# DavidXu-JJ/StreetUnveiler

Hardware: AMD Instinct MI355X
Metric: Msplats/s fwd+bwd @1920x1080, 3M Gaussians (higher is better)
Workload: dtype f32; 1 GPU; C3: 3M Gaussians, 1920x1080, fwd+bwd with depth/normal aux outputs (all 7 aux-map gradients live); gaussians=3000000, width=1920, height=1080, sh_degree=3, frames_per_rank=1, parallelism=single GPU, camera_rig=benchmark

## Files before the change

diff_surfel_rasterization/_C.py:

```python
from __future__ import annotations

import ctypes as C
import os

import torch

from streetunveiler_amd import _lib as L


_roctx = None


def _roctx_lib():
    global _roctx
    if _roctx is None:
        _roctx = False
        import os
        if os.environ.get("SURFEL_ROCTX") == "1":
            for name in ("libroctx64.so", "libroctx64.so.4", "/opt/rocm/lib/libroctx64.so"):
                try:
                    lib = C.CDLL(name)
                    lib.roctxRangePushA.argtypes = [C.c_char_p]; lib.roctxRangePushA.restype = C.c_int
                    lib.roctxRangePop.restype = C.c_int
                    _roctx = lib
                    break
                except OSError:
                    continue
    return _roctx


class _range:
    def __init__(self, name: str):
        self.name = name

    def __enter__(self):
        lib = _roctx_lib()
        self.on = bool(lib)
        if self.on:
            lib.roctxRangePushA(("surfel:" + self.name).encode())
        return self

    def __exit__(self, *exc):
        if self.on:
            _roctx.roctxRangePop()
        return False


def _ptr(t: torch.Tensor):
    return None if t is None or t.numel() == 0 else C.c_void_p(t.data_ptr())


def _f32c(t: torch.Tensor, name: str) -> torch.Tensor:
    if t is None:
        return None
    if not t.is_cuda:
        raise L.SurfelRasterError(f"{name} must be a CUDA (ROCm) tensor; the surfel rasterizer has no CPU path")
    if t.dtype != torch.float32:
        t = t.float()
    return t.contiguous()


def _stream(device):
    return C.c_void_p(torch.cuda.current_stream(device).cuda_stream)


_EXTRA_FLAGS = int(os.environ.get("SURFEL_EXTRA_FLAGS", "0"), 0)


def _frame(bg, scale_modifier, viewmatrix, projmatrix, tan_fovx, tan_fovy, H, W, degree, campos, prefiltered, debug, tile=None,
           quadrant_cull=True, blend_counters=None, ballot_ranking=False, row_mapped=None, forward_only=False, no_precomp_color_grad=False,
           binning_capacity=None, backward_kernel=None):
    keep = [_f32c(bg, "bg"), _f32c(viewmatrix, "viewmatrix"), _f32c(projmatrix, "projmatrix"), _f32c(campos, "campos"), blend_counters]
    if blend_counters is not None and (blend_counters.dtype != torch.int64 or blend_counters.numel() < 16 or not blend_counters.is_cuda):
        raise L.SurfelRasterError("blend_counters must be a CUDA (ROCm) int64 tensor with 16 entries")
    fr = L.SrFrame(int(H), int(W), float(tan_fovx), float(tan_fovy), float(scale_modifier), int(degree),
                   int(bool(prefiltered)), int(bool(debug)), _ptr(keep[0]), _ptr(keep[1]), _ptr(keep[2]), _ptr(keep[3]),
                   int(tile[0]) if tile else 0, int(tile[1]) if tile else 0, (0 if quadrant_cull else L.SR_FLAG_NO_QUADRANT_CULL) | (L.SR_FLAG_BALLOT_RANKING if ballot_ranking else 0) |
                   (0 if row_mapped is None else (L.SR_FLAG_ROW_MAPPED_FORWARD if row_mapped else L.SR_FLAG_QUADRANT_MAPPED_FORWARD)) |
                   (L.SR_FLAG_FORWARD_ONLY if forward_only else 0) | (L.SR_FLAG_NO_PRECOMP_COLOR_GRAD if no_precomp_color_grad else 0) |
                   (L.SR_FLAG_BINNING_CAPACITY if binning_capacity is not None else 0) |
                   ({None: 0, "one_wave": L.SR_FLAG_ONE_WAVE_BACKWARD, "coop": L.SR_FLAG_COOP_BACKWARD, "rows": L.SR_FLAG_ROW_BACKWARD}[backward_kernel]) | _EXTRA_FLAGS,
                   _ptr(blend_counters))
    return fr, keep


def _mask(mask, P, dev):
    if mask is None:
        return None
    if mask.numel() != P or mask.dtype not in (torch.bool, torch.uint8):
        raise L.SurfelRasterError("mask must be a bool tensor with one entry per Gaussian")
    if not mask.is_cuda:
        raise L.SurfelRasterError("mask must be a CUDA (ROCm) tensor")
    return mask.contiguous().view(torch.uint8)


def _channels(colors_precomp):
    if colors_precomp is None or (colors_precomp.numel() == 0 and not (colors_precomp.ndim == 2 and colors_precomp.shape[0] == 0 and colors_precomp.shape[1] in (3, 6))):
        return 3
    nc = int(colors_precomp.shape[-1])
    if colors_precomp.ndim != 2 or nc not in (3, 6):
        raise L.SurfelRasterError("colors_precomp must have dimensions (num_points, 3) or (num_points, 6)")
    return nc


def _gaussians(means3D, opacities, scales, rotations, sh, colors_precomp, transMat_precomp, activations=0, mask=None):
    P = int(means3D.shape[0])
    M = int(sh.shape[1]) if sh is not None and (sh.numel() or (P == 0 and sh.ndim == 3)) else 0
    NC = _channels(colors_precomp)
    if M and NC == 6:
        NC = 9
    elif M and colors_precomp is not None and colors_precomp.numel():
        raise L.SurfelRasterError("Please provide exactly one of either SHs or precomputed colors!")
    g = L.SrGaussians(P, M, NC, int(activations), _ptr(means3D), _ptr(opacities), _ptr(scales), _ptr(rotations), _ptr(sh),
                      _ptr(colors_precomp), _ptr(transMat_precomp), _ptr(mask))
    return g


def rasterize_gaussians(bg, means3D, colors_precomp, opacities, scales, rotations, scale_modifier, transMat_precomp,
                        viewmatrix, projmatrix, tan_fovx, tan_fovy, image_height, image_width, sh, degree, campos,
                        prefiltered, debug, activations=0, tile=None, mask=None, quadrant_cull=True, blend_counters=None,
                        ballot_ranking=False, row_mapped=None, forward_only=False, classes=None, n_classes=0, binning_capacity=None, backward_kernel=None):
    lib = L.load()
    if means3D.ndim != 2 or means3D.shape[1] != 3:
        raise L.SurfelRasterError("means3D must have dimensions (num_points, 3)")
    means3D = _f32c(means3D, "means3D"); opacities = _f32c(opacities, "opacities")
    colors_precomp = _f32c(colors_precomp, "colors_precomp"); scales = _f32c(scales, "scales")
    rotations = _f32c(rotations, "rotations"); transMat_precomp = _f32c(transMat_precomp, "transMat_precomp")
    sh = _f32c(sh, "sh")
    dev = means3D.device
    P, H, W = int(means3D.shape[0]), int(image_height), int(image_width)
    with torch.cuda.device(dev), _range("forward"):
        if binning_capacity is not None and (classes is not None or int(binning_capacity) < 0):
            raise L.SurfelRasterError("binning_capacity: a non-negative number of duplicates; not with the shared-plan class pass")
        fr, keep = _frame(bg, scale_modifier, viewmatrix, projmatrix, tan_fovx, tan_fovy, H, W, degree, campos, prefiltered, debug, tile,
                          quadrant_cull, blend_counters, ballot_ranking, row_mapped, forward_only, binning_capacity=binning_capacity,
                          backward_kernel=backward_kernel)
        mask = _mask(mask, P, dev)
        g = _gaussians(means3D, opacities, scales, rotations, sh, colors_precomp, transMat_precomp, activations, mask)
        if keep[0].numel() != g.color_channels:
            raise L.SurfelRasterError(f"bg must have {g.color_channels} entries, one per colour channel")
        color = torch.empty((g.color_channels, H, W), dtype=torch.float32, device=dev)
        allmap = torch.empty((7, H, W), dtype=torch.float32, device=dev)
        radii = torch.empty((P,), dtype=torch.int32, device=dev)
        geom = torch.empty((lib.sr_geom_bytes(P),), dtype=torch.uint8, device=dev)
        img = torch.empty((0 if forward_only else lib.sr_image_bytes(W, H),), dtype=torch.uint8, device=dev)
        stream = _stream(dev)
        D = C.c_uint32(0)
        L.check(lib.sr_forward_plan(C.byref(fr), C.byref(g), _ptr(geom), geom.numel(), _ptr(radii), C.byref(D), stream),
                "sr_forward_plan")
        num_rendered = int(D.value) if binning_capacity is None else (max(1, int(binning_capacity)) if P else 0)
        binning = torch.empty((lib.sr_binning_bytes(P, num_rendered, W, H),), dtype=torch.uint8, device=dev)
        L.check(lib.sr_forward_render(C.byref(fr), C.byref(g), _ptr(geom), geom.numel(), _ptr(binning), binning.numel(),
                                      _ptr(img), img.numel(), num_rendered, _ptr(color), _ptr(allmap), stream),
                "sr_forward_render")
        if classes is not None and int(n_classes) > 0:
            if classes.numel() != P:
                raise L.SurfelRasterError("classes must have one entry per Gaussian")
            if forward_only:
                raise L.SurfelRasterError("the shared-plan class pass is a training pass: not with forward_only")
            cls = classes.to(device=dev, dtype=torch.int32).contiguous()
            dist = torch.empty((int(n_classes), H, W), dtype=torch.float32, device=dev)
            cstate = torch.empty((lib.sr_class_shared_bytes(P, W, H, int(n_classes), num_rendered),), dtype=torch.uint8, device=dev)
            with _range("class_forward"):
                L.check(lib.sr_class_forward_shared(C.byref(fr), C.byref(g), int(n_classes), _ptr(cls), _ptr(geom), geom.numel(), _ptr(binning), binning.numel(),
                                                    _ptr(cstate), cstate.numel(), num_rendered, _ptr(dist), stream), "sr_class_forward_shared")
            del keep
            return num_rendered, color, allmap, radii, geom, binning, img, dist, cstate
    del keep
    return num_rendered, color, allmap, radii, geom, binning, img


def rasterize_gaussians_backward(bg, means3D, radii, colors_precomp, scales, rotations, scale_modifier, transMat_precomp,
                                 viewmatrix, projmatrix, tan_fovx, tan_fovy, dL_dcolor, dL_dallmap, sh, degree, campos,
                                 geomBuffer, num_rendered, binningBuffer, imgBuffer, debug, opacities=None, defer_sh=False,
                                 activations=0, tile=None, after_blend=None, class_state=None, dL_ddist=None, n_classes=0, want_precomp_color_grad=True,
                                 binning_capacity=None, backward_kernel=None):
    lib = L.load()
    means3D = _f32c(means3D, "means3D")
    colors_precomp = _f32c(colors_precomp, "colors_precomp"); scales = _f32c(scales, "scales")
    rotations = _f32c(rotations, "rotations"); transMat_precomp = _f32c(transMat_precomp, "transMat_precomp")
    sh = _f32c(sh, "sh")
    dL_dcolor = _f32c(dL_dcolor, "dL_dcolor"); dL_dallmap = _f32c(dL_dallmap, "dL_dallmap")
    dev = means3D.device
    P = int(means3D.shape[0])
    H, W = int(dL_dcolor.shape[1]), int(dL_dcolor.shape[2])
    M = int(sh.shape[1]) if sh is not None and sh.numel() else 0
    with torch.cuda.device(dev), _range("backward"):
        skip_cg = (not want_precomp_color_grad) and _channels(colors_precomp) == 6
        fr, keep = _frame(bg, scale_modifier, viewmatrix, projmatrix, tan_fovx, tan_fovy, H, W, degree, campos, False, debug, tile,
                          no_precomp_color_grad=skip_cg, binning_capacity=binning_capacity, backward_kernel=backward_kernel)
        g = _gaussians(means3D, means3D, scales, rotations, sh, colors_precomp, transMat_precomp, activations)
        e = lambda *shape: torch.empty(shape, dtype=torch.float32, device=dev)
        has = lambda t: t is not None and t.numel() > 0
        defer_sh = bool(defer_sh) and has(sh) and not has(colors_precomp)
        sizes = [("means3D", (P, 3)), ("sh", (P, M, 3) if has(sh) and not defer_sh else (0, 0, 3)), ("opacity", (P, 1)),
                 ("scales", (P, 2) if has(scales) else (0, 2)), ("rotations", (P, 4) if has(rotations) else (0, 4))]
        numel = lambda shp: int(torch.Size(shp).numel())
        flat = torch.empty(sum(numel(shp) for _, shp in sizes), dtype=torch.float32, device=dev)
        views, off = {}, 0
        for name, shp in sizes:
            n = numel(shp)
            views[name] = flat[off:off + n].view(shp)
            off += n
        dL_dmeans3D, dL_dsh, dL_dopacity, dL_dscales, dL_drotations = (views[k] for k in ("means3D", "sh", "opacity", "scales", "rotations"))
        dL_dmeans2D = e(P, 3)
        NC = g.color_channels
        if int(dL_dcolor.shape[0]) != NC or keep[0].numel() != NC:
            raise L.SurfelRasterError(f"dL_dcolor / bg must have {NC} channels")
        dL_dcolors = e(P, 6 if NC == 9 else NC) if (has(colors_precomp) and not skip_cg) or defer_sh else e(0, 3)
        dL_dtransMat = e(P, 9) if has(transMat_precomp) else e(0, 9)
        ws = torch.empty((lib.sr_backward_workspace_bytes(P, int(num_rendered), NC),), dtype=torch.uint8, device=dev)
        grads = L.SrGradients(_ptr(dL_dmeans2D), _ptr(dL_dcolors), _ptr(dL_dopacity), _ptr(dL_dmeans3D), _ptr(dL_dtransMat),
                              _ptr(dL_dsh), _ptr(dL_dscales), _ptr(dL_drotations))
        if class_state is not None:
            if defer_sh or after_blend is not None:
                raise L.SurfelRasterError("the shared-plan class pass (class_state) does not combine with the factored SH exchange "
                                          "(defer_sh / after_blend): exchange its gradients with the plain all-reduce")
            dL_ddist = _f32c(dL_ddist, "dL_ddist")
            L.check(lib.sr_backward_blend(C.byref(fr), C.byref(g), _ptr(geomBuffer), geomBuffer.numel(), _ptr(binningBuffer),
                                          binningBuffer.numel(), _ptr(imgBuffer), imgBuffer.numel(), int(num_rendered), _ptr(dL_dcolor),
                                          _ptr(dL_dallmap), _ptr(ws), ws.numel(), _stream(dev)), "sr_backward_blend")
            with _range("class_backward"):
                L.check(lib.sr_class_backward_shared(C.byref(fr), C.byref(g), int(n_classes), _ptr(geomBuffer), geomBuffer.numel(), _ptr(binningBuffer),
                                                     binningBuffer.numel(), _ptr(class_state), class_state.numel(), int(num_rendered), _ptr(dL_ddist),
                                                     _ptr(ws), ws.numel(), _stream(dev)), "sr_class_backward_shared")
            L.check(lib.sr_backward_geometry(C.byref(fr), C.byref(g), _ptr(radii), _ptr(geomBuffer), geomBuffer.numel(), _ptr(binningBuffer),
                                             binningBuffer.numel(), _ptr(imgBuffer), imgBuffer.numel(), int(num_rendered), _ptr(ws),
                                             ws.numel(), C.byref(grads), _stream(dev)), "sr_backward_geometry")
        elif after_blend is not None and defer_sh and NC == 3:
            L.check(lib.sr_backward_blend(C.byref(fr), C.byref(g), _ptr(geomBuffer), geomBuffer.numel(), _ptr(binningBuffer),
                                          binningBuffer.numel(), _ptr(imgBuffer), imgBuffer.numel(), int(num_rendered), _ptr(dL_dcolor),
                                          _ptr(dL_dallmap), _ptr(ws), ws.numel(), _stream(dev)), "sr_backward_blend")
            L.check(lib.sr_backward_colors(C.byref(fr), C.byref(g), _ptr(radii), _ptr(geomBuffer), geomBuffer.numel(), int(num_rendered),
                                           _ptr(ws), ws.numel(), _ptr(dL_dcolors), _stream(dev)), "sr_backward_colors")
            after_blend(dL_dcolors)
            grads.dL_dcolors = None
            L.check(lib.sr_backward_geometry(C.byref(fr), C.byref(g), _ptr(radii), _ptr(geomBuffer), geomBuffer.numel(), _ptr(binningBuffer),
                                             binningBuffer.numel(), _ptr(imgBuffer), imgBuffer.numel(), int(num_rendered), _ptr(ws),
                                             ws.numel(), C.byref(grads), _stream(dev)), "sr_backward_geometry")
        else:
            L.check(lib.sr_backward(C.byref(fr), C.byref(g), _ptr(radii), _ptr(geomBuffer), geomBuffer.numel(),
                                    _ptr(binningBuffer), binningBuffer.numel(), _ptr(imgBuffer), imgBuffer.numel(),
                                    int(num_rendered), _ptr(dL_dcolor), _ptr(dL_dallmap), _ptr(ws), ws.numel(),
                                    C.byref(grads), _stream(dev)), "sr_backward")
    del keep
    return dL_dmeans2D, dL_dcolors, dL_dopacity, dL_dmeans3D, dL_dtransMat, dL_dsh, dL_dscales, dL_drotations


def class_distortions(bg, means3D, classes, opacities, scales, rotations, scale_modifier, viewmatrix, projmatrix, tan_fovx, tan_fovy,
                      image_height, image_width, campos, n_classes, debug=False, activations=0, mask=None, tile=None):
    lib = L.load()
    if means3D.ndim != 2 or means3D.shape[1] != 3:
        raise L.SurfelRasterError("means3D must have dimensions (num_points, 3)")
    means3D = _f32c(means3D, "means3D"); opacities = _f32c(opacities, "opacities"); scales = _f32c(scales, "scales"); rotations = _f32c(rotations, "rotations")
    dev = means3D.device
    P, H, W = int(means3D.shape[0]), int(image_height), int(image_width)
    if classes.numel() != P:
        raise L.SurfelRasterError("classes must have one entry per Gaussian")
    cols = torch.zeros((P, 3), dtype=torch.float32, device=dev)
    cols[:, 0] = classes.to(device=dev, dtype=torch.float32).reshape(P)
    with torch.cuda.device(dev), _range("class_forward"):
        fr, keep = _frame(bg, scale_modifier, viewmatrix, projmatrix, tan_fovx, tan_fovy, H, W, 0, campos, False, debug, tile)
        mask = _mask(mask, P, dev)
        g = _gaussians(means3D, opacities, scales, rotations, None, cols, None, activations, mask)
        dist = torch.empty((int(n_classes), H, W), dtype=torch.float32, device=dev)
        radii = torch.empty((P,), dtype=torch.int32, device=dev)
        geom = torch.empty((lib.sr_geom_bytes(P),), dtype=torch.uint8, device=dev)
        cimg = torch.empty((lib.sr_class_image_bytes(W, H, int(n_classes)),), dtype=torch.uint8, device=dev)
        stream = _stream(dev)
        D = C.c_uint32(0)
        L.check(lib.sr_forward_plan(C.byref(fr), C.byref(g), _ptr(geom), geom.numel(), _ptr(radii), C.byref(D), stream), "sr_forward_plan")
        num_rendered = int(D.value)
        binning = torch.empty((lib.sr_binning_bytes(P, num_rendered, W, H),), dtype=torch.uint8, device=dev)
        L.check(lib.sr_class_forward_render(C.byref(fr), C.byref(g), int(n_classes), _ptr(geom), geom.numel(), _ptr(binning), binning.numel(),
                                            _ptr(cimg), cimg.numel(), num_rendered, _ptr(dist), stream), "sr_class_forward_render")
    del keep
    return num_rendered, dist, radii, cols, geom, binning, cimg


def class_distortions_backward(bg, means3D, radii, cols, scales, rotations, scale_modifier, viewmatrix, projmatrix, tan_fovx, tan_fovy,
                               dL_ddist, campos, n_classes, geom, num_rendered, binning, cimg, debug=False, activations=0, tile=None):
    lib = L.load()
    means3D = _f32c(means3D, "means3D"); scales = _f32c(scales, "scales"); rotations = _f32c(rotations, "rotations")
    dL_ddist = _f32c(dL_ddist, "dL_ddist")
    dev = means3D.device
    P = int(means3D.shape[0])
    H, W = int(dL_ddist.shape[1]), int(dL_ddist.shape[2])
    with torch.cuda.device(dev), _range("class_backward"):
        fr, keep = _frame(bg, scale_modifier, viewmatrix, projmatrix, tan_fovx, tan_fovy, H, W, 0, campos, False, debug, tile)
        g = _gaussians(means3D, means3D, scales, rotations, None, cols, None, activations)
        flat = torch.empty(P * 10, dtype=torch.float32, device=dev)
        dL_dmeans3D, dL_dopacity = flat[:3 * P].view(P, 3), flat[3 * P:4 * P].view(P, 1)
        dL_dscales, dL_drotations = flat[4 * P:6 * P].view(P, 2), flat[6 * P:].view(P, 4)
        dL_dmeans2D = torch.empty((P, 3), dtype=torch.float32, device=dev)
        ws = torch.empty((lib.sr_backward_workspace_bytes(P, int(num_rendered), 3),), dtype=torch.uint8, device=dev)
        grads = L.SrGradients(_ptr(dL_dmeans2D), None, _ptr(dL_dopacity), _ptr(dL_dmeans3D), None, None, _ptr(dL_dscales), _ptr(dL_drotations))
        L.check(lib.sr_class_backward(C.byref(fr), C.byref(g), int(n_classes), _ptr(radii), _ptr(geom), geom.numel(), _ptr(binning), binning.numel(),
                                      _ptr(cimg), cimg.numel(), int(num_rendered), _ptr(dL_ddist), _ptr(ws), ws.numel(), C.byref(grads),
                                      _stream(dev)), "sr_class_backward")
    del keep
    return dL_dmeans2D, dL_dopacity, dL_dmeans3D, dL_dscales, dL_drotations


def pair_decisions(bg, means3D, scale_modifier, viewmatrix, projmatrix, tan_fovx, tan_fovy, image_height, image_width, degree, campos,
                   geomBuffer, num_rendered, binningBuffer, tile=None):
    lib = L.load()
    means3D = _f32c(means3D, "means3D")
    dev = means3D.device
    tw, th = tile if tile else (16, 16)
    nq = (tw // 8) * (th // 8)
    valid = torch.zeros((max(int(num_rendered), 1), nq), dtype=torch.int64, device=dev)
    use3d = torch.zeros_like(valid)
    with torch.cuda.device(dev):
        fr, keep = _frame(bg, scale_modifier, viewmatrix, projmatrix, tan_fovx, tan_fovy, image_height, image_width, degree, campos, False, False, tile)
        g = L.SrGaussians(int(means3D.shape[0]), 0, 3, 0, _ptr(means3D), _ptr(means3D), None, None, None, _ptr(means3D), _ptr(means3D), None)
        L.check(lib.sr_debug_pair_decisions(C.byref(fr), C.byref(g), _ptr(geomBuffer), geomBuffer.numel(), _ptr(binningBuffer),
                                            binningBuffer.numel(), int(num_rendered), _ptr(valid), _ptr(use3d), _stream(dev)),
                "sr_debug_pair_decisions")
    del keep
    return valid[:int(num_rendered)], use3d[:int(num_rendered)]


def sh_gradient_expand(means3D, campos, dL_dcolors, sh_coeffs, degree):
    lib = L.load()
    means3D = _f32c(means3D, "means3D"); campos = _f32c(campos, "campos").reshape(-1, 3); dL_dcolors = _f32c(dL_dcolors, "dL_dcolors")
    P, V = int(means3D.shape[0]), int(campos.shape[0])
    if dL_dcolors.numel() != V * P * 3:
        raise L.SurfelRasterError(f"dL_dcolors must have {V} x {P} x 3 elements")
    out = torch.empty((P, int(sh_coeffs), 3), dtype=torch.float32, device=means3D.device)
    with torch.cuda.device(means3D.device):
        L.check(lib.sr_sh_gradient_expand(P, int(sh_coeffs), int(degree), V, _ptr(means3D), _ptr(campos), _ptr(dL_dcolors),
                                          _ptr(out), _stream(means3D.device)), "sr_sh_gradient_expand")
    return out


def mark_visible(means3D, viewmatrix, projmatrix):
    lib = L.load()
    means3D = _f32c(means3D, "means3D"); viewmatrix = _f32c(viewmatrix, "viewmatrix"); projmatrix = _f32c(projmatrix, "projmatrix")
    P = int(means3D.shape[0])
    present = torch.empty((P,), dtype=torch.bool, device=means3D.device)
    with torch.cuda.device(means3D.device):
        L.check(lib.sr_mark_visible(P, _ptr(means3D), _ptr(viewmatrix), _ptr(projmatrix), _ptr(present),
                                    _stream(means3D.device)), "sr_mark_visible")
    return present


def _view(buf: torch.Tensor, ptr, nbytes: int, dtype: torch.dtype) -> torch.Tensor:
    off = int(ptr) - buf.data_ptr()
    return buf[off:off + nbytes].view(dtype)


def forward_status(geom: torch.Tensor, P: int) -> torch.Tensor:
    v = L.SrGeomView()
    L.check(L.load().sr_geom_view(_ptr(geom), geom.numel(), int(P), C.byref(v)), "sr_geom_view")
    return _view(geom, v.frame_counts, 12, torch.int32)


def geom_view(geom: torch.Tensor, P: int):
    v = L.SrGeomView()
    L.check(L.load().sr_geom_view(_ptr(geom), geom.numel(), P, C.byref(v)), "sr_geom_view")
    return dict(splats=_view(geom, v.splats, P * 80, torch.float32).view(P, 20),
                depth_keys=_view(geom, v.depth_keys, P * 4, torch.int32), tiles_touched=_view(geom, v.tiles_touched, P * 4, torch.int32),
                clamped=_view(geom, v.clamped, P, torch.uint8), sorted_gid=_view(geom, v.sorted_gid, P * 4, torch.int32),
                frame_counts=_view(geom, v.frame_counts, 8, torch.int32))


def binning_view(binning: torch.Tensor, P: int, D: int, W: int, H: int, tile=(16, 16)):
    v = L.SrBinningView()
    L.check(L.load().sr_binning_view(_ptr(binning), binning.numel(), P, D, W, H, C.byref(v)), "sr_binning_view")
    tiles = ((W + tile[0] - 1) // tile[0]) * ((H + tile[1] - 1) // tile[1])
    ranges = _view(binning, v.ranges, tiles * 8, torch.int32).view(tiles, 2)
    counts = (ranges[:, 1] - ranges[:, 0]).long()
    tile_keys = torch.repeat_interleave(torch.arange(tiles, device=binning.device, dtype=torch.int32), counts)
    return dict(tile_keys=tile_keys, point_list=_view(binning, v.point_list, D * 4, torch.int32), ranges=ranges,
                tile_order=_view(binning, v.tile_order, tiles * 4, torch.int32))


def image_view(img: torch.Tensor, W: int, H: int):
    v = L.SrImageView()
    L.check(L.load().sr_image_view(_ptr(img), img.numel(), W, H, C.byref(v)), "sr_image_view")
    return dict(final_T=_view(img, v.final_T, 3 * H * W * 4, torch.float32).view(3, H, W),
                n_contrib=_view(img, v.n_contrib, 2 * H * W * 4, torch.int32).view(2, H, W))
```

streetunveiler_amd/csrc/api.hip:

```cpp
#include <cstdarg>
#include <cstdio>
#include <cstring>
#include <cmath>
#include <atomic>
#include <mutex>

#include "common.h"

namespace sr {
hipError_t launch_preprocess_forward(int P, const FrameDev& f, const SrGaussians& g, float4* recs, uint32_t* depth_keys,
                                     uint32_t* tiles_touched, uint2* rect, uint8_t* clamped, int32_t* radii, hipStream_t s);
hipError_t launch_preprocess_backward(int P, const FrameDev& f, const SrGaussians& g, const int32_t* radii,
                                      const uint8_t* clamped, const float4* recs, const float4* inst_grads, const uint8_t* written,
                                      const uint32_t* tiles_touched, const SrGradients& out, hipStream_t s);
hipError_t launch_mark_visible(int P, const float* means3D, const float* view, uint8_t* present, hipStream_t s);
hipError_t launch_sh_gradient_expand(int P, int M, int deg, int V, const float* means3D, const float* campos, const float* gc,
                                     float* dL_dsh, hipStream_t s);
size_t depth_sort_temp_bytes(int P);
size_t tile_scan_temp_bytes(int P);
size_t expand_x_hist_bytes(int P, int tiles_x);
size_t expand_y_hist_bytes(uint32_t D, int tiles_y);
hipError_t run_depth_sort(int P, const uint32_t* depth_keys, const uint2* rect, uint32_t* sorted_keys,
                          uint32_t* sorted_gid, uint2* rect_sorted, void* temp, size_t temp_bytes, int rank_mode, int tiles_x, int tiles_y,
                          const uint32_t* n_visible, hipStream_t s);
hipError_t run_tile_count_scan(int P, const uint32_t* tiles_touched, uint32_t* first, void* block_base, size_t base_bytes, uint32_t* total_host,
                               hipStream_t s);
hipError_t run_expand_columns(int P, int tiles_x, int n_tiles, const uint2* rect_sorted, const uint32_t* sorted_gid, uint2* columns,
                              uint32_t* n_columns, uint32_t* hist, uint32_t* row_total, uint32_t* tile_counts, int rank_mode, const uint32_t* n_visible,
                              hipStream_t s);
hipError_t run_expand_rows(uint32_t D, int tiles_x, int tiles_y, const uint2* columns, const uint32_t* n_columns, uint32_t* hist, uint32_t* row_total,
                           uint32_t* point_list, uint32_t* tile_counts, int rank_mode, hipStream_t s);
hipError_t run_tile_ranges_order(int n_tiles, const uint32_t* tile_counts, uint2* ranges, uint32_t* order, hipStream_t s);
hipError_t run_capacity_guard(uint32_t* counts, uint32_t capacity, hipStream_t s);
hipError_t launch_zero_bytes(void* p, size_t n, hipStream_t s);
hipError_t launch_render_forward(const FrameDev& f, const uint2* ranges, const uint32_t* tile_order, const uint32_t* point_list, const float4* recs,
                                 const float* extra, float* out_color, float* out_allmap, float* final_T, uint32_t* n_contrib, uint16_t* hit_mask, int flags,
                                 unsigned long long* counters, const uint32_t* frame_counts, hipStream_t s);
hipError_t launch_render_backward(const FrameDev& f, const uint2* ranges, const uint32_t* tile_order, const uint32_t* point_list, const float4* recs,
                                  const float* extra, const float* final_T, const uint32_t* n_contrib, const float* dL_dcolor,
                                  const float* dL_dallmap, const uint16_t* hit_mask, float4* inst_grads, uint8_t* written, bool precomp_color_grads, hipStream_t s, int coop_mode);
hipError_t launch_pair_decisions(const FrameDev& f, const uint2* ranges, const uint32_t* point_list, const float4* recs,
                                 unsigned long long* valid_bits, unsigned long long* use3d_bits, hipStream_t s);
hipError_t launch_class_partition(int P, int n_tiles, int n_classes, const float* class_cols, const int32_t* class_i32, const uint2* ranges,
                                  const uint32_t* point_list, uint8_t* ids, uint32_t* cls_list, uint2* cls_ranges, hipStream_t s);
hipError_t launch_class_forward(const FrameDev& f, int n_classes, const uint2* cls_ranges, const uint32_t* tile_order, const uint32_t* cls_list,
                                const float4* recs, float* out_dist, float* cls_state, uint32_t* cls_last, uint32_t* tile_total, uint16_t* hit_mask,
                                int cull, hipStream_t s);
hipError_t launch_class_backward(const FrameDev& f, int n_classes, const uint2* cls_ranges, const uint32_t* tile_order, const uint32_t* cls_list,
                                 const float4* recs, const float* cls_state, const uint32_t* cls_last, const uint32_t* tile_total,
                                 const float* dL_ddist, const uint16_t* hit_mask, float4* inst_grads, uint8_t* written, int shared_rec_quads, hipStream_t s);
hipError_t launch_color_gradients(int P, const FrameDev& f, const int32_t* radii, const uint8_t* clamped, const float4* recs, const float4* inst_grads,
                                  const uint8_t* written, const uint32_t* tiles_touched, bool mask_clamped, float* dL_dcolors, hipStream_t s);
size_t radix_sort_temp_bytes(uint32_t n);
hipError_t radix_sort_pairs(const uint32_t* keys_in, const uint32_t* vals_in, uint32_t* keys_out, uint32_t* vals_out, uint32_t n,
                            int total_bits, void* temp, size_t temp_bytes, hipStream_t s, const uint2* aux_src, uint2* aux_out, int rank_mode,
                            int rect_bx = 0, int rect_by = 0, const uint32_t* n_live = nullptr);
hipError_t launch_rank_selfcheck(uint32_t* result, hipStream_t s);
hipError_t lds_atomic_ranks(const uint32_t* digits, uint32_t* ranks, uint32_t n, int bins, hipStream_t s);
size_t knn_workspace_bytes(int nq, int nr);
hipError_t knn_mean_dist2(int nq, const float* query, int nr, const float* reference, int K, int take_sqrt, float* out, void* ws,
                          size_t ws_bytes, int rank_mode, hipStream_t s);
struct PostCam { int W, H; float fx, fy, depth_ratio; const float* view; };
hipError_t launch_postprocess_forward(const PostCam& cam, const float* allmap, float* rend_normal, float* surf_depth,
                                      float* surf_normal, float* surf_point, hipStream_t s);
hipError_t launch_postprocess_backward(const PostCam& cam, const float* allmap, const float* g_rend_normal, const float* g_surf_depth,
                                       const float* g_surf_normal, const float* g_surf_point, float* scratch6, float* g_allmap,
                                       hipStream_t s);
struct LossImages { int W, H, C; float lambda; const float* image; const float* gt; const float* sky; const float* alpha; };
bool image_loss_supported(int W, int H, int C);
size_t image_loss_partial_bytes();
hipError_t launch_image_loss_forward(const LossImages& a, void* workspace, float* out3, hipStream_t s);
hipError_t launch_image_loss_backward(const LossImages& a, const void* workspace, const float* g_loss, float* g_image, float* g_sky,
                                      float* g_alpha, hipStream_t s);
}

using namespace sr;

namespace {

thread_local char g_err[512] = "";
std::atomic<int> g_timing{0};
std::mutex g_ring_mu;

int fail(int code, const char* fmt, ...) {
    va_list ap;
    va_start(ap, fmt);
    vsnprintf(g_err, sizeof(g_err), fmt, ap);
    va_end(ap);
    return code;
}

#define SR_HIP(expr)                                                                                         \
    do {                                                                                                     \
        hipError_t _e = (expr);                                                                              \
        if (_e != hipSuccess) return fail(SR_ERR_HIP, "%s failed: %s (%s:%d)", #expr, hipGetErrorString(_e), \
                                          __FILE__, __LINE__);                                               \
    } while (0)

constexpr int kEvRing = 512;
struct EvRing {
    hipEvent_t ev[kEvRing][2];
    bool closed[kEvRing];
    int created = 0, used = 0;
};
EvRing g_ring[SR_STAGE_COUNT];

struct StageTimer {
    int stage; hipStream_t s; int slot = -1;
    StageTimer(int st, hipStream_t stream) : stage(st), s(stream) {
        const int mode = g_timing.load();
        if (!mode || (mode != 1 && !((mode >> 1) & (1 << stage)))) return;
        std::lock_guard<std::mutex> lk(g_ring_mu);
        EvRing& r = g_ring[stage];
        if (r.used >= kEvRing) return;
        if (r.used >= r.created) {
            if (hipEventCreate(&r.ev[r.created][0]) != hipSuccess || hipEventCreate(&r.ev[r.created][1]) != hipSuccess) return;
            ++r.created;
        }
        slot = r.used++;
        r.closed[slot] = false;
        (void)hipEventRecord(r.ev[slot][0], s);
    }
    ~StageTimer() {
        if (slot < 0) return;
        std::lock_guard<std::mutex> lk(g_ring_mu);
        if (hipEventRecord(g_ring[stage].ev[slot][1], s) == hipSuccess) g_ring[stage].closed[slot] = true;
    }
};

int debug_sync(const SrFrame* frame, hipStream_t s, const char* what) {
    if (!frame->debug) return SR_OK;
    hipError_t e = hipStreamSynchronize(s);
    if (e == hipSuccess) e = hipGetLastError();
    if (e != hipSuccess) return fail(SR_ERR_HIP, "[debug] after %s: %s", what, hipGetErrorString(e));
    return SR_OK;
}

uint32_t* pinned_words() {
    static thread_local uint32_t* pinned = nullptr;
    if (!pinned && hipHostMalloc(reinterpret_cast<void**>(&pinned), 64, hipHostMallocPortable | hipHostMallocMapped) != hipSuccess) { pinned = nullptr; (void)hipGetLastError(); }
    return pinned;
}

int stream_device(hipStream_t s, int* dev) {
    hipDevice_t d = 0;
    if (s && hipStreamGetDevice(s, &d) == hipSuccess) { *dev = (int)d; return SR_OK; }
    (void)hipGetLastError();
    SR_HIP(hipGetDevice(dev));
    return SR_OK;
}

constexpr int kMaxDevices = 64;
std::atomic<int> g_rank_mode[kMaxDevices];
int rank_mode(hipStream_t s, bool force_ballot, int* mode) {
    int dev = 0;
    { const int rc = stream_device(s, &dev); if (rc != SR_OK) return rc; }
    if (dev < 0 || dev >= kMaxDevices) return fail(SR_ERR_UNSUPPORTED, "device index %d beyond %d", dev, kMaxDevices);
    int m = g_rank_mode[dev].load(std::memory_order_acquire);
    if (m == kRankUnknown) {
        hipStreamCaptureStatus cap = hipStreamCaptureStatusNone;
        if (hipStreamIsCapturing(s, &cap) == hipSuccess && cap != hipStreamCaptureStatusNone)
            return fail(SR_ERR_UNSUPPORTED, "the stream is capturing and device %d has not run the rank self-check yet: call sr_rank_mode(stream) once before the capture", dev);
        (void)hipGetLastError();
        struct Scratch { uint32_t* p = nullptr; ~Scratch() { if (p) (void)hipFree(p); } } scratch;
        uint32_t* host = pinned_words();
        uint32_t* result = nullptr;
        const bool temp = !(host && hipHostGetDevicePointer(reinterpret_cast<void**>(&result), host + 8, 0) == hipSuccess && result);
        if (!temp) host[8] = 0;
        else { (void)hipGetLastError(); SR_HIP(hipMalloc(reinterpret_cast<void**>(&scratch.p), 4)); result = scratch.p; SR_HIP(hipMemsetAsync(result, 0, 4, s)); }
        SR_HIP(launch_rank_selfcheck(result, s));
        uint32_t r = 0;
        if (temp) { SR_HIP(hipMemcpyAsync(&r, result, 4, hipMemcpyDeviceToHost, s)); SR_HIP(hipStreamSynchronize(s)); }
        else { SR_HIP(hipStreamSynchronize(s)); r = *reinterpret_cast<volatile uint32_t*>(host + 8); }
        if (!(r & 0x100u)) return fail(SR_ERR_HIP, "the rank self-check kernel did not report back");
        m = (r & 1u) ? kRankAtomic : ((r & 2u) ? kRankBallot : kRankNone);
        g_rank_mode[dev].store(m, std::memory_order_release);
    }
    if (m == kRankNone) return fail(SR_ERR_UNSUPPORTED, "neither LDS-atomic nor ballot ranking passes the self-check on device %d", dev);
    *mode = force_ballot ? (int)kRankBallot : m;
    return SR_OK;
}

constexpr int kMaxTilesPerAxis = SR_MAX_TILES_PER_AXIS;
struct GeomLayout {
    size_t recs, depth_keys, tiles_touched, rect, clamped, sorted_keys, sorted_gid, rect_sorted, first, sh_jac, block_base, base_bytes,
        n_scan_blocks, temp, temp_bytes, total;
};
GeomLayout geom_layout(int P) {
    GeomLayout L{};
    const size_t n = (size_t)(P > 0 ? P : 1);
    size_t off = 0;
    auto take = [&](size_t bytes) { size_t o = off; off = align_up(off + bytes, 256); return o; };
    L.recs = take(n * kRecFloats * 4);
    L.depth_keys = take(n * 4);
    L.tiles_touched = take(n * 4);
    L.rect = take(n * 8);
    L.clamped = take(n);
    L.sorted_keys = take(n * 4);
    L.sorted_gid = take(n * 4);
    L.rect_sorted = take(n * 8);
    L.first = take(n * 4);
    L.sh_jac = take(n * 36);
    L.base_bytes = tile_scan_temp_bytes(P);
    L.block_base = take(L.base_bytes);
    L.n_scan_blocks = (n + 2047) / 2048;
    static thread_local int memo_P = -1;
    static thread_local size_t memo_bytes = 0;
    if (memo_P != P) {
        memo_bytes = depth_sort_temp_bytes(P);
        const size_t hx = align_up(expand_x_hist_bytes(P, kMaxTilesPerAxis), 256);
        if (hx > memo_bytes) memo_bytes = hx;
        memo_P = P;
    }
    L.temp_bytes = memo_bytes;
    L.temp = take(L.temp_bytes);
    L.total = off;
    return L;
}

struct BinLayout {
    size_t columns, point_list, hit_mask, ranges, order, tile_counts, row_total, n_columns, hist, hist_bytes, total;
};
BinLayout bin_layout(uint32_t D, int W, int H) {
    BinLayout L{};
    const size_t n = (size_t)(D > 0 ? D : 1);
    const int tiles = ((W + 7) / 8) * ((H + 7) / 8);
    size_t off = 0;
    auto take = [&](size_t bytes) { size_t o = off; off = align_up(off + bytes, 256); return o; };
    L.columns = take(n * 8);
    L.point_list = take(n * 4);
    L.hit_mask = take(n * 2);
    L.ranges = take((size_t)(tiles > 0 ? tiles : 1) * 8);
    L.order = take((size_t)(tiles > 0 ? tiles : 1) * 4);
    L.tile_counts = take((size_t)(tiles > 0 ? tiles : 1) * 4);
    L.row_total = take((size_t)kMaxTilesPerAxis * 4);
    L.n_columns = take(4);
    L.hist_bytes = expand_y_hist_bytes(D, (H + 7) / 8);
    L.hist = take(L.hist_bytes);
    L.total = off;
    return L;
}

struct ImgLayout { size_t final_T, n_contrib, total; };
ImgLayout img_layout(int W, int H) {
    ImgLayout L{};
    const size_t hw = (size_t)(W > 0 ? W : 1) * (size_t)(H > 0 ? H : 1);
    L.final_T = 0;
    L.n_contrib = align_up(hw * 3 * 4, 256);
    L.total = align_up(L.n_contrib + hw * 2 * 4, 256);
    return L;
}

int check_common(const SrFrame* frame, const SrGaussians* g) {
    if (!frame || !g) return fail(SR_ERR_INVALID_ARGUMENT, "frame / gaussians is NULL");
    if (frame->image_width <= 0 || frame->image_height <= 0) return fail(SR_ERR_INVALID_ARGUMENT, "bad image size %dx%d", frame->image_width, frame->image_height);
    if (g->P < 0) return fail(SR_ERR_INVALID_ARGUMENT, "P < 0");
    {
        const int tw = frame->tile_width > 0 ? frame->tile_width : kTile, th = frame->tile_height > 0 ? frame->tile_height : kTile;
        const bool known = (tw == 16 && th == 16) || (tw == 8 && th == 8) || (tw == 16 && th == 8) || (tw == 32 && th == 8) || (tw == 32 && th == 16);
        if (!known) return fail(SR_ERR_UNSUPPORTED, "tile shape %dx%d not in {8x8, 16x8, 16x16, 32x8, 32x16}", tw, th);
    }
    if (!frame->bg || !frame->viewmatrix || !frame->projmatrix || !frame->campos) return fail(SR_ERR_INVALID_ARGUMENT, "bg / viewmatrix / projmatrix / campos must be non-NULL device pointers");
    if (g->P > 0) {
        if (!g->means3D || !g->opacities) return fail(SR_ERR_INVALID_ARGUMENT, "means3D / opacities is NULL");
        if (g->color_channels == 9) {
            if (!g->shs || !g->colors_precomp) return fail(SR_ERR_INVALID_ARGUMENT, "9 colour channels need SHs AND a [P,6] precomputed colour array");
        } else if ((g->shs != nullptr) == (g->colors_precomp != nullptr)) return fail(SR_ERR_INVALID_ARGUMENT, "Please provide exactly one of either SHs or precomputed colors!");
        if (g->color_channels != 0 && g->color_channels != 3 && g->color_channels != 6 && g->color_channels != 9) return fail(SR_ERR_UNSUPPORTED, "color_channels %d not in {3, 6, 9}", g->color_channels);
        if (g->activations & ~(SR_ACT_EXP_SCALES | SR_ACT_SIGMOID_OPACITY | SR_ACT_NORMALIZE_ROTATIONS)) return fail(SR_ERR_UNSUPPORTED, "unknown activation bits 0x%x", g->activations);
        if (g->color_channels == 6 && g->shs) return fail(SR_ERR_INVALID_ARGUMENT, "6 colour channels need precomputed colors, not SHs");
        const bool sr_pair = g->scales != nullptr && g->rotations != nullptr;
        if ((g->scales != nullptr) != (g->rotations != nullptr) || sr_pair == (g->transMat_precomp != nullptr))
            return fail(SR_ERR_INVALID_ARGUMENT, "Please provide exactly one of either scale/rotation pair or precomputed transMat!");
        if (g->shs) {
            if (frame->sh_degree < 0 || frame->sh_degree > 3) return fail(SR_ERR_UNSUPPORTED, "sh_degree %d not in 0..3", frame->sh_degree);
            if (g->sh_coeffs < (frame->sh_degree + 1) * (frame->sh_degree + 1)) return fail(SR_ERR_INVALID_ARGUMENT, "shs has %d coefficients, degree %d needs %d", g->sh_coeffs, frame->sh_degree, (frame->sh_degree + 1) * (frame->sh_degree + 1));
        }
    }
    return SR_OK;
}

int check_backward_frame(const SrFrame* frame) {
#if SR_BACKWARD_WH_FROM_FOCAL
    if (!(frame->tanfovx > 0.f) || !(frame->tanfovy > 0.f) || !std::isfinite(frame->tanfovx) || !std::isfinite(frame->tanfovy))
        return fail(SR_ERR_INVALID_ARGUMENT, "tanfovx / tanfovy must be finite and > 0 for a backward call (got %g, %g)", (double)frame->tanfovx, (double)frame->tanfovy);
#else
    (void)frame;
#endif
    return SR_OK;
}

int check_blend_pair_flags(const SrFrame* frame) {
    const uint32_t pair = frame->flags & (SR_FLAG_ONE_WAVE_BACKWARD | SR_FLAG_COOP_BACKWARD | SR_FLAG_ROW_BACKWARD);
    if (pair & (pair - 1))
        return fail(SR_ERR_INVALID_ARGUMENT, "SR_FLAG_ONE_WAVE_BACKWARD, SR_FLAG_COOP_BACKWARD and SR_FLAG_ROW_BACKWARD exclude each other (flags 0x%x)", pair);
    return SR_OK;
}

FrameDev make_frame(const SrFrame* frame, const SrGaussians* g) {
    FrameDev f{};
    f.W = frame->image_width; f.H = frame->image_height;
    f.bw_W = f.W; f.bw_H = f.H;
#if SR_BACKWARD_WH_FROM_FOCAL
    if (frame->tanfovx > 0.f && frame->tanfovy > 0.f && std::isfinite(frame->tanfovx) && std::isfinite(frame->tanfovy)) {
        const float focal_x = (float)f.W / (2.0f * frame->tanfovx), focal_y = (float)f.H / (2.0f * frame->tanfovy);
        f.bw_W = (int)(focal_x * frame->tanfovx * 2); f.bw_H = (int)(focal_y * frame->tanfovy * 2);
    }
#endif
    f.tile_w = frame->tile_width > 0 ? frame->tile_width : kTile; f.tile_h = frame->tile_height > 0 ? frame->tile_height : kTile;
    f.inv_tile_w = 1.f / (float)f.tile_w; f.inv_tile_h = 1.f / (float)f.tile_h;
    f.tiles_x = (f.W + f.tile_w - 1) / f.tile_w; f.tiles_y = (f.H + f.tile_h - 1) / f.tile_h;
    f.sh_degree = frame->sh_degree; f.sh_coeffs = g->sh_coeffs;
    f.colors = g->color_channels == 6 ? 6 : (g->color_channels == 9 ? 9 : 3);
    f.activations = g->activations;
    f.scale_modifier = frame->scale_modifier;
    f.bg = frame->bg; f.view = frame->viewmatrix; f.proj = frame->projmatrix; f.campos = frame->campos;
    f.overflow = nullptr;
    return f;
}

template <class T> T* at(void* base, size_t off) { return reinterpret_cast<T*>(static_cast<char*>(base) + off); }

}

extern "C" {

int sr_abi_version(void) { return SR_ABI_VERSION; }
uint32_t sr_build_switches(void) { return SR_SWITCH_BITS; }
const char* sr_last_error(void) { return g_err; }

size_t sr_geom_bytes(int32_t P) { return geom_layout(P).total; }
size_t sr_binning_bytes(int32_t P, uint32_t num_rendered, int32_t W, int32_t H) { (void)P; return bin_layout(num_rendered, W, H).total; }
size_t sr_image_bytes(int32_t W, int32_t H) { return img_layout(W, H).total; }
static size_t record_bytes(int color_channels) { return (size_t)(color_channels == 9 ? kGradFloats + 4 : kGradFloats) * 4; }

size_t sr_backward_workspace_bytes(int32_t P, uint32_t num_rendered, int32_t color_channels) {
    (void)P;
    const size_t n = (size_t)(num_rendered > 0 ? num_rendered : 1);
    return align_up(n * record_bytes(color_channels), 256) + align_up(n, 256);
}

int sr_geom_view(void* geom, size_t geom_bytes, int32_t P, SrGeomView* out) {
    if (!geom || !out) return fail(SR_ERR_INVALID_ARGUMENT, "NULL argument");
    const GeomLayout L = geom_layout(P);
    if (geom_bytes < L.total) return fail(SR_ERR_BUFFER_TOO_SMALL, "geom buffer %zu < %zu", geom_bytes, L.total);
    out->splats = at<float>(geom, L.recs); out->depth_keys = at<uint32_t>(geom, L.depth_keys);
    out->tiles_touched = at<uint32_t>(geom, L.tiles_touched); out->clamped = at<uint8_t>(geom, L.clamped);
    out->sorted_gid = at<uint32_t>(geom, L.sorted_gid);
    out->frame_counts = at<uint32_t>(geom, L.block_base) + L.n_scan_blocks;
    return SR_OK;
}

int sr_binning_view(void* binning, size_t binning_bytes, int32_t P, uint32_t D, int32_t W, int32_t H, SrBinningView* out) {
    (void)P;
    if (!binning || !out) return fail(SR_ERR_INVALID_ARGUMENT, "NULL argument");
    const BinLayout L = bin_layout(D, W, H);
    if (binning_bytes < L.total) return fail(SR_ERR_BUFFER_TOO_SMALL, "binning buffer %zu < %zu", binning_bytes, L.total);
    out->point_list = at<uint32_t>(binning, L.point_list);
    out->ranges = at<uint32_t>(binning, L.ranges); out->tile_order = at<uint32_t>(binning, L.order);
    return SR_OK;
}

int sr_image_view(void* image, size_t image_bytes, int32_t W, int32_t H, SrImageView* out) {
    if (!image || !out) return fail(SR_ERR_INVALID_ARGUMENT, "NULL argument");
    const ImgLayout L = img_layout(W, H);
    if (image_bytes < L.total) return fail(SR_ERR_BUFFER_TOO_SMALL, "image buffer %zu < %zu", image_bytes, L.total);
    out->final_T = at<float>(image, L.final_T); out->n_contrib = at<uint32_t>(image, L.n_contrib);
    return SR_OK;
}

int sr_forward_plan(const SrFrame* frame, const SrGaussians* g, void* geom, size_t geom_bytes, int32_t* radii,
                    uint32_t* num_rendered_host, void* stream) {
    if (int rc = check_common(frame, g)) return rc;
    if (!num_rendered_host) return fail(SR_ERR_INVALID_ARGUMENT, "num_rendered_host is NULL");
    *num_rendered_host = 0;
    const int P = g->P;
    if (P == 0) return SR_OK;
    if (!geom || !radii) return fail(SR_ERR_INVALID_ARGUMENT, "geom / radii is NULL");
    const GeomLayout L = geom_layout(P);
    if (geom_bytes < L.total) return fail(SR_ERR_BUFFER_TOO_SMALL, "geom buffer %zu < %zu", geom_bytes, L.total);
    hipStream_t s = static_cast<hipStream_t>(stream);
    FrameDev f = make_frame(frame, g);
    f.sh_jac = (frame->flags & SR_FLAG_FORWARD_ONLY) ? nullptr : at<float>(geom, L.sh_jac);
    {
        StageTimer t(SR_STAGE_PREPROCESS, s);
        SR_HIP(launch_preprocess_forward(P, f, *g, at<float4>(geom, L.recs), at<uint32_t>(geom, L.depth_keys),
                                         at<uint32_t>(geom, L.tiles_touched), at<uint2>(geom, L.rect), at<uint8_t>(geom, L.clamped), radii, s));
    }
    if (int rc = debug_sync(frame, s, "preprocess_forward")) return rc;
    int sort_mode = kRankUnknown;
    if (int rc = rank_mode(s, (frame->flags & SR_FLAG_BALLOT_RANKING) != 0, &sort_mode)) return rc;
    const int depth_sort_mode = sort_mode | ((frame->flags & SR_FLAG_ONE_SWEEP_SORT) ? 0x100 : 0);
    if (frame->flags & SR_FLAG_BINNING_CAPACITY) {
        {
            StageTimer t(SR_STAGE_SCAN, s);
            SR_HIP(run_tile_count_scan(P, at<uint32_t>(geom, L.tiles_touched), at<uint32_t>(geom, L.first), at<void>(geom, L.block_base), L.base_bytes, nullptr, s));
        }
        if (int rc = debug_sync(frame, s, "emission_scan")) return rc;
        {
            StageTimer t(SR_STAGE_DEPTH_SORT, s);
            SR_HIP(run_depth_sort(P, at<uint32_t>(geom, L.depth_keys), at<uint2>(geom, L.rect), at<uint32_t>(geom, L.sorted_keys),
                                  at<uint32_t>(geom, L.sorted_gid), at<uint2>(geom, L.rect_sorted), at<void>(geom, L.temp), L.temp_bytes, depth_sort_mode,
                                  f.tiles_x, f.tiles_y, at<uint32_t>(geom, L.block_base) + L.n_scan_blocks + 1, s));
        }
        *num_rendered_host = 0xFFFFFFFFu;
        return debug_sync(frame, s, "depth_sort");
    }
    uint32_t* pinned = pinned_words();
    uint32_t* pinned_dev = nullptr;
    if (pinned && (hipHostGetDevicePointer(reinterpret_cast<void**>(&pinned_dev), pinned, 0) != hipSuccess)) pinned_dev = nullptr;
    {
        StageTimer t(SR_STAGE_SCAN, s);
        SR_HIP(run_tile_count_scan(P, at<uint32_t>(geom, L.tiles_touched), at<uint32_t>(geom, L.first), at<void>(geom, L.block_base),
                                   L.base_bytes, pinned_dev, s));
    }
    if (int rc = debug_sync(frame, s, "emission_scan")) return rc;
    static thread_local hipEvent_t copied_ev[kMaxDevices] = {};
    int dev = 0;
    SR_HIP(hipGetDevice(&dev));
    hipEvent_t copied = nullptr;
    if (dev >= 0 && dev < kMaxDevices) {
        if (!copied_ev[dev] && hipEventCreateWithFlags(&copied_ev[dev], hipEventDisableTiming) != hipSuccess) copied_ev[dev] = nullptr;
        copied = copied_ev[dev];
    }
    if (!pinned_dev) {
        uint32_t* dst = pinned ? pinned : num_rendered_host;
        SR_HIP(hipMemcpyAsync(dst, at<uint32_t>(geom, L.block_base) + L.n_scan_blocks, 4, hipMemcpyDeviceToHost, s));
    }
    if (copied && pinned && hipEventRecord(copied, s) != hipSuccess) copied = nullptr;
    {
        StageTimer t(SR_STAGE_DEPTH_SORT, s);
        SR_HIP(run_depth_sort(P, at<uint32_t>(geom, L.depth_keys), at<uint2>(geom, L.rect), at<uint32_t>(geom, L.sorted_keys),
                              at<uint32_t>(geom, L.sorted_gid), at<uint2>(geom, L.rect_sorted), at<void>(geom, L.temp), L.temp_bytes, depth_sort_mode,
                              f.tiles_x, f.tiles_y, at<uint32_t>(geom, L.block_base) + L.n_scan_blocks + 1, s));
    }
    if (int rc = debug_sync(frame, s, "depth_sort")) return rc;
    if (copied && pinned) SR_HIP(hipEventSynchronize(copied));
    else SR_HIP(hipStreamSynchronize(s));
    if (pinned) *num_rendered_host = *reinterpret_cast<volatile uint32_t*>(pinned);
    return SR_OK;
}

namespace {
int bin_duplicates(const SrFrame* frame, const SrGaussians* g, const FrameDev& f, void* geom, size_t geom_bytes, void* binning, const BinLayout& B,
                   uint32_t D, hipStream_t s, float4** recs_out) {
    const int P = g->P;
    const int n_tiles = f.tiles_x * f.tiles_y;
    *recs_out = nullptr;
    if (P > 0 && D > 0) {
        if (!geom) return fail(SR_ERR_INVALID_ARGUMENT, "geom is NULL");
        const GeomLayout L = geom_layout(P);
        if (geom_bytes < L.total) return fail(SR_ERR_BUFFER_TOO_SMALL, "geom buffer %zu < %zu", geom_bytes, L.total);
        float4* recs = at<float4>(geom, L.recs);
        *recs_out = recs;
        if (f.tiles_x > kMaxTilesPerAxis || f.tiles_y > kMaxTilesPerAxis)
            return fail(SR_ERR_INVALID_ARGUMENT, "%d x %d tiles: at most %d per axis (use a larger tile)", f.tiles_x, f.tiles_y, kMaxTilesPerAxis);
        if (L.temp_bytes < expand_x_hist_bytes(P, f.tiles_x)) return fail(SR_ERR_BUFFER_TOO_SMALL, "geom scratch too small for the column histogram");
        int sort_mode = kRankUnknown;
        if (int rc = rank_mode(s, (frame->flags & SR_FLAG_BALLOT_RANKING) != 0, &sort_mode)) return rc;
        if (frame->flags & SR_FLAG_BINNING_CAPACITY)
            SR_HIP(run_capacity_guard(at<uint32_t>(geom, L.block_base) + L.n_scan_blocks, D, s));
        {
            StageTimer t(SR_STAGE_EXPAND_X, s);
            SR_HIP(run_expand_columns(P, f.tiles_x, n_tiles, at<uint2>(geom, L.rect_sorted), at<uint32_t>(geom, L.sorted_gid), at<uint2>(binning, B.columns),
                                      at<uint32_t>(binning, B.n_columns), at<uint32_t>(geom, L.temp), at<uint32_t>(binning, B.row_total),
                                      at<uint32_t>(binning, B.tile_counts), sort_mode, at<uint32_t>(geom, L.block_base) + L.n_scan_blocks + 1, s));
        }
        if (int rc = debug_sync(frame, s, "expand_columns")) return rc;
        {
            StageTimer t(SR_STAGE_EXPAND_Y, s);
            SR_HIP(run_expand_rows(D, f.tiles_x, f.tiles_y, at<uint2>(binning, B.columns), at<uint32_t>(binning, B.n_columns),
                                   at<uint32_t>(binning, B.hist), at<uint32_t>(binning, B.row_total), at<uint32_t>(binning, B.point_list),
                                   at<uint32_t>(binning, B.tile_counts), sort_mode, s));
        }
        if (int rc = debug_sync(frame, s, "expand_rows")) return rc;
    } else {
        SR_HIP(launch_zero_bytes(at<uint32_t>(binning, B.tile_counts), sizeof(uint32_t) * (size_t)n_tiles, s));
    }
    {
        StageTimer t(SR_STAGE_RANGES, s);
        SR_HIP(run_tile_ranges_order(n_tiles, at<uint32_t>(binning, B.tile_counts), at<uint2>(binning, B.ranges), at<uint32_t>(binning, B.order), s));
    }
    return debug_sync(frame, s, "tile_ranges");
}

struct ClassLayout { size_t state, last, tile_total, ranges, total; };
ClassLayout class_layout(int W, int H, int n_classes) {
    ClassLayout L{};
    const size_t hw = (size_t)(W > 0 ? W : 1) * (size_t)(H > 0 ? H : 1), n = (size_t)(n_classes > 0 ? n_classes : 1);
    const size_t tiles = (size_t)((W + 7) / 8) * (size_t)((H + 7) / 8);
    L.state = 0;
    L.last = align_up(n * 3 * hw * 4, 256);
    L.tile_total = L.last + align_up(n * hw * 4, 256);
    L.ranges = L.tile_total + align_up((tiles > 0 ? tiles : 1) * n * 4, 256);
    L.total = L.ranges + align_up((tiles > 0 ? tiles : 1) * n * 8, 256);
    return L;
}

int check_class_pass(const SrFrame* frame, const SrGaussians* g, int n_classes) {
    if (int rc = check_common(frame, g)) return rc;
    if (frame->flags & SR_FLAG_BINNING_CAPACITY) return fail(SR_ERR_UNSUPPORTED, "SR_FLAG_BINNING_CAPACITY serves the operator (sr_forward_* / sr_backward*), not the per-class pass");
    if (n_classes < 1 || n_classes > 6) return fail(SR_ERR_UNSUPPORTED, "n_classes %d not in 1..6", n_classes);
    const int tw = frame->tile_width > 0 ? frame->tile_width : kTile, th = frame->tile_height > 0 ? frame->tile_height : kTile;
    (void)tw; (void)th;
    if (g->P > 0 && (g->shs || !g->colors_precomp || (g->color_channels != 0 && g->color_channels != 3)))
        return fail(SR_ERR_INVALID_ARGUMENT, "the per-class distortion pass takes the class ids in colors_precomp[P,3] (column 0), no SHs");
    return SR_OK;
}
}

int sr_forward_render(const SrFrame* frame, const SrGaussians* g, void* geom, size_t geom_bytes, void* binning,
                      size_t binning_bytes, void* image, size_t image_bytes, uint32_t D, float* out_color,
                      float* out_allmap, void* stream) {
    if (int rc = check_common(frame, g)) return rc;
    if (int rc = check_blend_pair_flags(frame)) return rc;
    const bool fwd_only = (frame->flags & SR_FLAG_FORWARD_ONLY) != 0;
    if (!binning || (!image && !fwd_only) || !out_color || !out_allmap) return fail(SR_ERR_INVALID_ARGUMENT, "binning / image / out_color / out_allmap is NULL");
    const int W = frame->image_width, H = frame->image_height;
    const BinLayout B = bin_layout(D, W, H);
    const ImgLayout I = img_layout(W, H);
    if (binning_bytes < B.total) return fail(SR_ERR_BUFFER_TOO_SMALL, "binning buffer %zu < %zu", binning_bytes, B.total);
    if (!fwd_only && image_bytes < I.total) return fail(SR_ERR_BUFFER_TOO_SMALL, "image buffer %zu < %zu", image_bytes, I.total);
    if (fwd_only && frame->blend_counters) return fail(SR_ERR_UNSUPPORTED, "SR_FLAG_FORWARD_ONLY and blend_counters exclude each other");
    hipStream_t s = static_cast<hipStream_t>(stream);
    const FrameDev f = make_frame(frame, g);
    if (frame->blend_counters && !(f.tile_w == 16 && f.tile_h == 16 && (f.colors == 3 || f.colors == 6)))
        return fail(SR_ERR_UNSUPPORTED, "blend_counters: the counting variant of the forward blend exists for the 16x16 tile with 3 or 6 colour channels only");
    float4* recs = nullptr;
    if (int rc = bin_duplicates(frame, g, f, geom, geom_bytes, binning, B, D, s, &recs)) return rc;
    {
        StageTimer t(SR_STAGE_BLEND_FWD, s);
        const bool rows = (frame->flags & SR_FLAG_ROW_MAPPED_FORWARD) != 0, quads = (frame->flags & SR_FLAG_QUADRANT_MAPPED_FORWARD) != 0;
        if (rows && quads) return fail(SR_ERR_INVALID_ARGUMENT, "SR_FLAG_ROW_MAPPED_FORWARD and SR_FLAG_QUADRANT_MAPPED_FORWARD exclude each other");
        if (rows && (!(f.tile_w == 16 && f.tile_h == 16 && f.colors == 3) || frame->blend_counters || (frame->flags & SR_FLAG_NO_QUADRANT_CULL)))
            return fail(SR_ERR_UNSUPPORTED, "SR_FLAG_ROW_MAPPED_FORWARD: 16x16 tile, three colour channels, no counters, culling on");
        const bool cells = (frame->flags & SR_FLAG_ROW_BACKWARD) != 0;
        if (cells && (!(f.tile_w == 16 && f.tile_h == 16 && f.colors == 3) || frame->blend_counters || (frame->flags & SR_FLAG_NO_QUADRANT_CULL) || quads || fwd_only))
            return fail(SR_ERR_UNSUPPORTED, "SR_FLAG_ROW_BACKWARD: 16x16 tile, three colour channels, no counters, culling on, the row-mapped forward, a backward to follow");
        const int flags = ((frame->flags & SR_FLAG_NO_QUADRANT_CULL) ? 0 : 1) | (frame->blend_counters ? 2 : 0) | (rows ? 4 : 0) | (quads ? 8 : 0) |
                          ((frame->flags & SR_FLAG_ONE_WAVE_BACKWARD) ? 16 : 0) | ((frame->flags & SR_FLAG_COOP_BACKWARD) ? 32 : 0) |
                          (cells ? 64 : 0);
        const GeomLayout GL = geom_layout(g->P);
        SR_HIP(launch_render_forward(f, at<uint2>(binning, B.ranges), at<uint32_t>(binning, B.order), at<uint32_t>(binning, B.point_list), recs, g->colors_precomp, out_color,
                                     out_allmap, fwd_only ? nullptr : at<float>(image, I.final_T), fwd_only ? nullptr : at<uint32_t>(image, I.n_contrib),
                                     fwd_only ? nullptr : at<uint16_t>(binning, B.hit_mask), flags,
                                     reinterpret_cast<unsigned long long*>(frame->blend_counters), at<uint32_t>(geom, GL.block_base) + GL.n_scan_blocks, s));
    }
    return debug_sync(frame, s, "render_forward");
}

size_t sr_class_image_bytes(int32_t W, int32_t H, int32_t n_classes) { return class_layout(W, H, n_classes).total; }

int sr_class_forward_render(const SrFrame* frame, const SrGaussians* g, int32_t n_classes, void* geom, size_t geom_bytes, void* binning,
                            size_t binning_bytes, void* class_image, size_t class_image_bytes, uint32_t D, float* out_dist, void* stream) {
    if (int rc = check_class_pass(frame, g, n_classes)) return rc;
    if (!binning || !class_image || !out_dist) return fail(SR_ERR_INVALID_ARGUMENT, "binning / class_image / out_dist is NULL");
    if (g->P > 0 && !geom) return fail(SR_ERR_INVALID_ARGUMENT, "geom is NULL (the class ids of the P Gaussians are staged in it, even when no duplicate was emitted)");
    const int W = frame->image_width, H = frame->image_height;
    const BinLayout B = bin_layout(D, W, H);
    const ClassLayout C = class_layout(W, H, n_classes);
    if (binning_bytes < B.total) return fail(SR_ERR_BUFFER_TOO_SMALL, "binning buffer %zu < %zu", binning_bytes, B.total);
    if (class_image_bytes < C.total) return fail(SR_ERR_BUFFER_TOO_SMALL, "class image buffer %zu < %zu", class_image_bytes, C.total);
    hipStream_t s = static_cast<hipStream_t>(stream);
    const FrameDev f = make_frame(frame, g);
    float4* recs = nullptr;
    if (int rc = bin_duplicates(frame, g, f, geom, geom_bytes, binning, B, D, s, &recs)) return rc;
    {
        StageTimer t(SR_STAGE_CLASS_PARTITION, s);
        const GeomLayout GL = geom_layout(g->P);
        SR_HIP(launch_class_partition(g->P, f.tiles_x * f.tiles_y, n_classes, g->colors_precomp, nullptr, at<uint2>(binning, B.ranges), at<uint32_t>(binning, B.point_list),
                                      g->P > 0 && geom ? at<uint8_t>(geom, GL.sh_jac) : nullptr, at<uint32_t>(binning, B.columns), at<uint2>(class_image, C.ranges), s));
    }
    if (int rc = debug_sync(frame, s, "class_partition")) return rc;
    {
        StageTimer t(SR_STAGE_CLASS_FWD, s);
        SR_HIP(launch_class_forward(f, n_classes, at<uint2>(class_image, C.ranges), at<uint32_t>(binning, B.order), at<uint32_t>(binning, B.columns), recs, out_dist,
                                    at<float>(class_image, C.state), at<uint32_t>(class_image, C.last), at<uint32_t>(class_image, C.tile_total),
                                    at<uint16_t>(binning, B.hit_mask), (frame->flags & SR_FLAG_NO_QUADRANT_CULL) ? 0 : 1, s));
    }
    return debug_sync(frame, s, "class_forward");
}

int sr_class_backward(const SrFrame* frame, const SrGaussians* g, int32_t n_classes, const int32_t* radii, void* geom, size_t geom_bytes,
                      void* binning, size_t binning_bytes, void* class_image, size_t class_image_bytes, uint32_t D, const float* dL_ddist,
                      void* workspace, size_t workspace_bytes, const SrGradients* grads, void* stream) {
    if (int rc = check_class_pass(frame, g, n_classes)) return rc;
    if (int rc = check_backward_frame(frame)) return rc;
    if (!grads) return fail(SR_ERR_INVALID_ARGUMENT, "grads is NULL");
    const int P = g->P;
    if (P == 0) return SR_OK;
    if (!radii || !geom || !binning || !class_image || !dL_ddist || !workspace) return fail(SR_ERR_INVALID_ARGUMENT, "NULL buffer argument");
    const int W = frame->image_width, H = frame->image_height;
    const GeomLayout L = geom_layout(P);
    const BinLayout B = bin_layout(D, W, H);
    const ClassLayout C = class_layout(W, H, n_classes);
    if (geom_bytes < L.total || binning_bytes < B.total || class_image_bytes < C.total) return fail(SR_ERR_BUFFER_TOO_SMALL, "state buffer too small");
    if (workspace_bytes < sr_backward_workspace_bytes(P, D, 3)) return fail(SR_ERR_BUFFER_TOO_SMALL, "workspace %zu < %zu", workspace_bytes, sr_backward_workspace_bytes(P, D, 3));
    hipStream_t s = static_cast<hipStream_t>(stream);
    FrameDev f = make_frame(frame, g);
    f.first = at<uint32_t>(geom, L.first); f.first_base = at<uint32_t>(geom, L.block_base); f.sh_jac = at<float>(geom, L.sh_jac);
    float4* inst_grads = static_cast<float4*>(workspace);
    uint8_t* written = static_cast<uint8_t*>(workspace) + align_up((size_t)(D > 0 ? D : 1) * record_bytes(3), 256);
    {
        StageTimer t(SR_STAGE_CLASS_BWD, s);
        if (D > 0) SR_HIP(launch_zero_bytes(written, D, s));
        if (D > 0)
            SR_HIP(launch_class_backward(f, n_classes, at<uint2>(class_image, C.ranges), at<uint32_t>(binning, B.order), at<uint32_t>(binning, B.columns), at<float4>(geom, L.recs),
                                         at<float>(class_image, C.state), at<uint32_t>(class_image, C.last), at<uint32_t>(class_image, C.tile_total), dL_ddist,
                                         at<uint16_t>(binning, B.hit_mask), inst_grads, written, 0, s));
    }
    if (int rc = debug_sync(frame, s, "class_backward")) return rc;
    {
        StageTimer t(SR_STAGE_PREPROCESS_BWD, s);
        SR_HIP(launch_preprocess_backward(P, f, *g, radii, at<uint8_t>(geom, L.clamped), at<float4>(geom, L.recs), inst_grads, written,
                                          at<uint32_t>(geom, L.tiles_touched), *grads, s));
    }
    return debug_sync(frame, s, "preprocess_backward");
}

namespace {
struct ClassSharedLayout { ClassLayout C; size_t ids, hit, total; };
ClassSharedLayout class_shared_layout(int P, int W, int H, int n_classes, uint32_t D) {
    ClassSharedLayout L{};
    L.C = class_layout(W, H, n_classes);
    L.ids = L.C.total;
    L.hit = L.ids + align_up((size_t)(P > 0 ? P : 1), 256);
    L.total = L.hit + align_up((size_t)(D > 0 ? D : 1) * 2, 256);
    return L;
}
}

size_t sr_class_shared_bytes(int32_t P, int32_t W, int32_t H, int32_t n_classes, uint32_t D) { return class_shared_layout(P, W, H, n_classes, D).total; }

int sr_class_forward_shared(const SrFrame* frame, const SrGaussians* g, int32_t n_classes, const int32_t* classes, void* geom, size_t geom_bytes,
                            void* binning, size_t binning_bytes, void* class_state, size_t class_state_bytes, uint32_t D, float* out_dist, void* stream) {
    if (int rc = check_common(frame, g)) return rc;
    if (frame->flags & SR_FLAG_BINNING_CAPACITY) return fail(SR_ERR_UNSUPPORTED, "SR_FLAG_BINNING_CAPACITY serves the operator (sr_forward_* / sr_backward*), not the per-class pass");
    if (n_classes < 1 || n_classes > 6) return fail(SR_ERR_UNSUPPORTED, "n_classes %d not in 1..6", n_classes);
    if (!binning || !class_state || !out_dist || (g->P > 0 && !classes)) return fail(SR_ERR_INVALID_ARGUMENT, "binning / class_state / out_dist / classes is NULL");
    if (g->transMat_precomp) return fail(SR_ERR_UNSUPPORTED, "the per-class pass takes scales and rotations, not a precomputed transMat");
    const int W = frame->image_width, H = frame->image_height, P = g->P;
    const BinLayout B = bin_layout(D, W, H);
    const ClassSharedLayout S = class_shared_layout(P, W, H, n_classes, D);
    if (binning_bytes < B.total) return fail(SR_ERR_BUFFER_TOO_SMALL, "binning buffer %zu < %zu", binning_bytes, B.total);
    if (class_state_bytes < S.total) return fail(SR_ERR_BUFFER_TOO_SMALL, "class state buffer %zu < %zu", class_state_bytes, S.total);
    float4* recs = nullptr;
    if (P > 0 && D > 0) {
        if (!geom) return fail(SR_ERR_INVALID_ARGUMENT, "geom is NULL");
        const GeomLayout L = geom_layout(P);
        if (geom_bytes < L.total) return fail(SR_ERR_BUFFER_TOO_SMALL, "geom buffer %zu < %zu", geom_bytes, L.total);
        recs = at<float4>(geom, L.recs);
    }
    hipStream_t s = static_cast<hipStream_t>(stream);
    const FrameDev f = make_frame(frame, g);
    {
        StageTimer t(SR_STAGE_CLASS_PARTITION, s);
        SR_HIP(launch_class_partition(P, f.tiles_x * f.tiles_y, n_classes, nullptr, classes, at<uint2>(binning, B.ranges), at<uint32_t>(binning, B.point_list),
                                      at<uint8_t>(class_state, S.ids), at<uint32_t>(binning, B.columns), at<uint2>(class_state, S.C.ranges), s));
    }
    if (int rc = debug_sync(frame, s, "class_partition")) return rc;
    {
        StageTimer t(SR_STAGE_CLASS_FWD, s);
        SR_HIP(launch_class_forward(f, n_classes, at<uint2>(class_state, S.C.ranges), at<uint32_t>(binning, B.order), at<uint32_t>(binning, B.columns), recs, out_dist,
                                    at<float>(class_state, S.C.state), at<uint32_t>(class_state, S.C.last), at<uint32_t>(class_state, S.C.tile_total),
                                    at<uint16_t>(class_state, S.hit), (frame->flags & SR_FLAG_NO_QUADRANT_CULL) ? 0 : 1, s));
    }
    return debug_sync(frame, s, "class_forward");
}

int sr_class_backward_shared(const SrFrame* frame, const SrGaussians* g, int32_t n_classes, void* geom, size_t geom_bytes, void* binning,
                             size_t binning_bytes, void* class_state, size_t class_state_bytes, uint32_t D, const float* dL_ddist, void* workspace,
                             size_t workspace_bytes, void* stream) {
    if (int rc = check_common(frame, g)) return rc;
    if (frame->flags & SR_FLAG_BINNING_CAPACITY) return fail(SR_ERR_UNSUPPORTED, "SR_FLAG_BINNING_CAPACITY serves the operator (sr_forward_* / sr_backward*), not the per-class pass");
    if (int rc = check_backward_frame(frame)) return rc;
    if (n_classes < 1 || n_classes > 6) return fail(SR_ERR_UNSUPPORTED, "n_classes %d not in 1..6", n_classes);
    const int P = g->P;
    if (P == 0 || D == 0) return SR_OK;
    if (!geom || !binning || !class_state || !dL_ddist || !workspace) return fail(SR_ERR_INVALID_ARGUMENT, "NULL buffer argument");
    const int W = frame->image_width, H = frame->image_height;
    const GeomLayout L = geom_layout(P);
    const BinLayout B = bin_layout(D, W, H);
    const ClassSharedLayout S = class_shared_layout(P, W, H, n_classes, D);
    if (geom_bytes < L.total || binning_bytes < B.total || class_state_bytes < S.total) return fail(SR_ERR_BUFFER_TOO_SMALL, "state buffer too small");
    if (workspace_bytes < sr_backward_workspace_bytes(P, D, g->color_channels)) return fail(SR_ERR_BUFFER_TOO_SMALL, "workspace %zu < %zu", workspace_bytes, sr_backward_workspace_bytes(P, D, g->color_channels));
    hipStream_t s = static_cast<hipStream_t>(stream);
    FrameDev f = make_frame(frame, g);
    f.first = at<uint32_t>(geom, L.first); f.first_base = at<uint32_t>(geom, L.block_base);
    float4* inst_grads = static_cast<float4*>(workspace);
    uint8_t* written = static_cast<uint8_t*>(workspace) + align_up((size_t)D * record_bytes(g->color_channels), 256);
    {
        StageTimer t(SR_STAGE_CLASS_BWD, s);
        SR_HIP(launch_class_backward(f, n_classes, at<uint2>(class_state, S.C.ranges), at<uint32_t>(binning, B.order), at<uint32_t>(binning, B.columns), at<float4>(geom, L.recs),
                                     at<float>(class_state, S.C.state), at<uint32_t>(class_state, S.C.last), at<uint32_t>(class_state, S.C.tile_total), dL_ddist,
                                     at<uint16_t>(class_state, S.hit), inst_grads, written, (int)(record_bytes(g->color_channels) / 16), s));
    }
    return debug_sync(frame, s, "class_backward_shared");
}

namespace {
struct BackwardCtx {
    int P; GeomLayout L; BinLayout B; ImgLayout I; FrameDev f; float4* inst_grads; uint8_t* written; hipStream_t s;
};
int backward_ctx(const SrFrame* frame, const SrGaussians* g, void* geom, size_t geom_bytes, void* binning, size_t binning_bytes,
                 void* image, size_t image_bytes, uint32_t D, void* workspace, size_t workspace_bytes, void* stream, BackwardCtx* c) {
    if (int rc = check_common(frame, g)) return rc;
    if (int rc = check_backward_frame(frame)) return rc;
    if (int rc = check_blend_pair_flags(frame)) return rc;
    const FrameDev shape = make_frame(frame, g);
    if ((frame->flags & SR_FLAG_ROW_BACKWARD) && (!(shape.tile_w == 16 && shape.tile_h == 16 && shape.colors == 3) || (frame->flags & SR_FLAG_NO_QUADRANT_CULL)))
        return fail(SR_ERR_UNSUPPORTED, "SR_FLAG_ROW_BACKWARD: 16x16 tile, three colour channels, culling on (as in the forward of the frame)");
    c->P = g->P;
    if (c->P == 0) return SR_OK;
    if (!geom || !binning || !image || !workspace) return fail(SR_ERR_INVALID_ARGUMENT, "NULL buffer argument");
    const int W = frame->image_width, H = frame->image_height;
    c->L = geom_layout(c->P); c->B = bin_layout(D, W, H); c->I = img_layout(W, H);
    if (geom_bytes < c->L.total) return fail(SR_ERR_BUFFER_TOO_SMALL, "geom buffer %zu < %zu", geom_bytes, c->L.total);
    if (binning_bytes < c->B.total) return fail(SR_ERR_BUFFER_TOO_SMALL, "binning buffer %zu < %zu", binning_bytes, c->B.total);
    if (image_bytes < c->I.total) return fail(SR_ERR_BUFFER_TOO_SMALL, "image buffer %zu < %zu", image_bytes, c->I.total);
    if (workspace_bytes < sr_backward_workspace_bytes(c->P, D, g->color_channels)) return fail(SR_ERR_BUFFER_TOO_SMALL, "workspace %zu < %zu", workspace_bytes, sr_backward_workspace_bytes(c->P, D, g->color_channels));
    c->s = static_cast<hipStream_t>(stream);
    c->f = make_frame(frame, g);
    c->f.first = at<uint32_t>(geom, c->L.first); c->f.first_base = at<uint32_t>(geom, c->L.block_base); c->f.sh_jac = at<float>(geom, c->L.sh_jac);
    if (frame->flags & SR_FLAG_BINNING_CAPACITY) c->f.overflow = at<uint32_t>(geom, c->L.block_base) + c->L.n_scan_blocks + 2;
    c->inst_grads = static_cast<float4*>(workspace);
    c->written = static_cast<uint8_t*>(workspace) + align_up((size_t)(D > 0 ? D : 1) * record_bytes(g->color_channels), 256);
    return SR_OK;
}
}

int sr_backward_blend(const SrFrame* frame, const SrGaussians* g, void* geom, size_t geom_bytes, void* binning, size_t binning_bytes,
                      void* image, size_t image_bytes, uint32_t D, const float* dL_dcolor, const float* dL_dallmap, void* workspace,
                      size_t workspace_bytes, void* stream) {
    BackwardCtx c;
    if (int rc = backward_ctx(frame, g, geom, geom_bytes, binning, binning_bytes, image, image_bytes, D, workspace, workspace_bytes, stream, &c)) return rc;
    if (c.P == 0) return SR_OK;
    if (!dL_dcolor || !dL_dallmap) return fail(SR_ERR_INVALID_ARGUMENT, "dL_dcolor / dL_dallmap is NULL");
    {
        StageTimer t(SR_STAGE_BLEND_BWD, c.s);
        if (D > 0) SR_HIP(launch_zero_bytes(c.written, D, c.s));
        if (D > 0)
            SR_HIP(launch_render_backward(c.f, at<uint2>(binning, c.B.ranges), at<uint32_t>(binning, c.B.order), at<uint32_t>(binning, c.B.point_list), at<float4>(geom, c.L.recs), g->colors_precomp,
                                          at<float>(image, c.I.final_T), at<uint32_t>(image, c.I.n_contrib), dL_dcolor, dL_dallmap, at<uint16_t>(binning, c.B.hit_mask), c.inst_grads, c.written,
                                          !(frame->flags & SR_FLAG_NO_PRECOMP_COLOR_GRAD), c.s,
                                          (frame->flags & SR_FLAG_ROW_BACKWARD) ? 3
                                          : ((frame->flags & SR_FLAG_ONE_WAVE_BACKWARD) ? 1 : ((frame->flags & SR_FLAG_COOP_BACKWARD) ? 2 : 0))));
    }
    return debug_sync(frame, c.s, "render_backward");
}

int sr_backward_colors(const SrFrame* frame, const SrGaussians* g, const int32_t* radii, void* geom, size_t geom_bytes, uint32_t D,
                       void* workspace, size_t workspace_bytes, float* dL_dcolors, void* stream) {
    if (int rc = check_common(frame, g)) return rc;
    if (int rc = check_backward_frame(frame)) return rc;
    const int P = g->P;
    if (P == 0) return SR_OK;
    if (g->color_channels == 6 || g->color_channels == 9) return fail(SR_ERR_UNSUPPORTED, "sr_backward_colors serves the 3-channel pass");
    if (!radii || !geom || !workspace || !dL_dcolors) return fail(SR_ERR_INVALID_ARGUMENT, "NULL buffer argument");
    const GeomLayout L = geom_layout(P);
    if (geom_bytes < L.total) return fail(SR_ERR_BUFFER_TOO_SMALL, "geom buffer %zu < %zu", geom_bytes, L.total);
    if (workspace_bytes < sr_backward_workspace_bytes(P, D, g->color_channels)) return fail(SR_ERR_BUFFER_TOO_SMALL, "workspace too small");
    hipStream_t s = static_cast<hipStream_t>(stream);
    FrameDev f = make_frame(frame, g);
    f.first = at<uint32_t>(geom, L.first); f.first_base = at<uint32_t>(geom, L.block_base); f.sh_jac = at<float>(geom, L.sh_jac);
    if (frame->flags & SR_FLAG_BINNING_CAPACITY) f.overflow = at<uint32_t>(geom, L.block_base) + L.n_scan_blocks + 2;
    const uint8_t* written = static_cast<uint8_t*>(workspace) + align_up((size_t)(D > 0 ? D : 1) * record_bytes(g->color_channels), 256);
    StageTimer t(SR_STAGE_PREPROCESS_BWD, s);
    SR_HIP(launch_color_gradients(P, f, radii, at<uint8_t>(geom, L.clamped), at<float4>(geom, L.recs), static_cast<const float4*>(workspace), written,
                                  at<uint32_t>(geom, L.tiles_touched), g->shs != nullptr, dL_dcolors, s));
    return debug_sync(frame, s, "color_gradients");
}

int sr_backward_geometry(const SrFrame* frame, const SrGaussians* g, const int32_t* radii, void* geom, size_t geom_bytes,
                         void* binning, size_t binning_bytes, void* image, size_t image_bytes, uint32_t D, void* workspace,
                         size_t workspace_bytes, const SrGradients* grads, void* stream) {
    if (!grads) return fail(SR_ERR_INVALID_ARGUMENT, "grads is NULL");
    BackwardCtx c;
    if (int rc = backward_ctx(frame, g, geom, geom_bytes, binning, binning_bytes, image, image_bytes, D, workspace, workspace_bytes, stream, &c)) return rc;
    if (c.P == 0) return SR_OK;
    if (!radii) return fail(SR_ERR_INVALID_ARGUMENT, "radii is NULL");
    {
        StageTimer t(SR_STAGE_PREPROCESS_BWD, c.s);
        SR_HIP(launch_preprocess_backward(c.P, c.f, *g, radii, at<uint8_t>(geom, c.L.clamped), at<float4>(geom, c.L.recs), c.inst_grads, c.written,
                                          at<uint32_t>(geom, c.L.tiles_touched), *grads, c.s));
    }
    return debug_sync(frame, c.s, "preprocess_backward");
}

int sr_backward(const SrFrame* frame, const SrGaussians* g, const int32_t* radii, void* geom, size_t geom_bytes,
                void* binning, size_t binning_bytes, void* image, size_t image_bytes, uint32_t D, const float* dL_dcolor,
                const float* dL_dallmap, void* workspace, size_t workspace_bytes, const SrGradients* grads, void* stream) {
    if (!grads) return fail(SR_ERR_INVALID_ARGUMENT, "grads is NULL");
    if (int rc = sr_backward_blend(frame, g, geom, geom_bytes, binning, binning_bytes, image, image_bytes, D, dL_dcolor, dL_dallmap, workspace, workspace_bytes, stream)) return rc;
    return sr_backward_geometry(frame, g, radii, geom, geom_bytes, binning, binning_bytes, image, image_bytes, D, workspace, workspace_bytes, grads, stream);
}

int sr_debug_pair_decisions(const SrFrame* frame, const SrGaussians* g, void* geom, size_t geom_bytes, void* binning, size_t binning_bytes,
                            uint32_t D, uint64_t* valid_bits, uint64_t* use3d_bits, void* stream) {
    if (int rc = check_common(frame, g)) return rc;
    if (g->P == 0 || D == 0) return SR_OK;
    if (!geom || !binning || !valid_bits || !use3d_bits) return fail(SR_ERR_INVALID_ARGUMENT, "NULL buffer argument");
    const GeomLayout L = geom_layout(g->P);
    const BinLayout B = bin_layout(D, frame->image_width, frame->image_height);
    if (geom_bytes < L.total || binning_bytes < B.total) return fail(SR_ERR_BUFFER_TOO_SMALL, "state buffer too small");
    const FrameDev f = make_frame(frame, g);
    SR_HIP(launch_pair_decisions(f, at<uint2>(binning, B.ranges), at<uint32_t>(binning, B.point_list), at<float4>(geom, L.recs),
                                 reinterpret_cast<unsigned long long*>(valid_bits), reinterpret_cast<unsigned long long*>(use3d_bits), static_cast<hipStream_t>(stream)));
    return SR_OK;
}

int sr_sh_gradient_expand(int32_t P, int32_t sh_coeffs, int32_t sh_degree, int32_t n_views, const float* means3D,
                          const float* campos, const float* dL_dcolors, float* dL_dsh, void* stream) {
    if (P < 0 || n_views < 1) return fail(SR_ERR_INVALID_ARGUMENT, "P < 0 or n_views < 1");
    if (sh_degree < 0 || sh_degree > 3) return fail(SR_ERR_UNSUPPORTED, "sh_degree %d not in 0..3", sh_degree);
    if (sh_coeffs < (sh_degree + 1) * (sh_degree + 1)) return fail(SR_ERR_INVALID_ARGUMENT, "shs has %d coefficients, degree %d needs %d", sh_coeffs, sh_degree, (sh_degree + 1) * (sh_degree + 1));
    if (P == 0) return SR_OK;
    if (!means3D || !campos || !dL_dcolors || !dL_dsh) return fail(SR_ERR_INVALID_ARGUMENT, "NULL argument");
    SR_HIP(launch_sh_gradient_expand(P, sh_coeffs, sh_degree, n_views, means3D, campos, dL_dcolors, dL_dsh, static_cast<hipStream_t>(stream)));
    return SR_OK;
}

size_t sr_knn_workspace_bytes(int32_t n_query, int32_t n_reference) {
    return knn_workspace_bytes(n_query > 0 ? n_query : 0, n_reference > 0 ? n_reference : 0);
}

int sr_knn_mean_dist2(int32_t n_query, const float* query, int32_t n_reference, const float* reference, int32_t K,
                      int32_t take_sqrt, float* out, void* workspace, size_t workspace_bytes, void* stream) {
    if (K != 3 && K != 10) return fail(SR_ERR_UNSUPPORTED, "K = %d, supported: 3 and 10", K);
    if (n_reference < 0 || (query && n_query < 0)) return fail(SR_ERR_INVALID_ARGUMENT, "negative point count");
    const int nq = query ? n_query : 0;
    if ((query ? nq : n_reference) == 0) return SR_OK;
    if (n_reference == 0) return fail(SR_ERR_INVALID_ARGUMENT, "empty reference cloud");
    if (!reference || !out || !workspace) return fail(SR_ERR_INVALID_ARGUMENT, "NULL argument");
    if (workspace_bytes < knn_workspace_bytes(nq, n_reference)) return fail(SR_ERR_BUFFER_TOO_SMALL, "workspace %zu < %zu", workspace_bytes, knn_workspace_bytes(nq, n_reference));
    int sort_mode = kRankUnknown;
    if (int rc = rank_mode(static_cast<hipStream_t>(stream), false, &sort_mode)) return rc;
    SR_HIP(knn_mean_dist2(nq, query, n_reference, reference, K, take_sqrt, out, workspace, workspace_bytes, sort_mode, static_cast<hipStream_t>(stream)));
    return SR_OK;
}

int sr_mark_visible(int32_t P, const float* means3D, const float* viewmatrix, const float* projmatrix, uint8_t* present,
                    void* stream) {
    (void)projmatrix;
    if (P < 0) return fail(SR_ERR_INVALID_ARGUMENT, "P < 0");
    if (P == 0) return SR_OK;
    if (!means3D || !viewmatrix || !present) return fail(SR_ERR_INVALID_ARGUMENT, "NULL argument");
    SR_HIP(launch_mark_visible(P, means3D, viewmatrix, present, static_cast<hipStream_t>(stream)));
    return SR_OK;
}

static int post_cam(int32_t W, int32_t H, float fovx, float fovy, float depth_ratio, const float* viewmatrix, PostCam* cam) {
    if (W <= 0 || H <= 0 || !viewmatrix) return fail(SR_ERR_INVALID_ARGUMENT, "bad image size / NULL viewmatrix");
    cam->W = W; cam->H = H;
    cam->fx = (float)W / (2.f * tanf(fovx * 0.5f)); cam->fy = (float)H / (2.f * tanf(fovy * 0.5f));
    cam->depth_ratio = depth_ratio; cam->view = viewmatrix;
    return SR_OK;
}

int sr_postprocess_forward(int32_t W, int32_t H, float fovx, float fovy, float depth_ratio, const float* viewmatrix,
                           const float* allmap, float* rend_normal, float* surf_depth, float* surf_normal, float* surf_point,
                           void* stream) {
    PostCam cam;
    if (int rc = post_cam(W, H, fovx, fovy, depth_ratio, viewmatrix, &cam)) return rc;
    if (!allmap || !rend_normal || !surf_depth || !surf_normal || !surf_point) return fail(SR_ERR_INVALID_ARGUMENT, "NULL argument");
    SR_HIP(launch_postprocess_forward(cam, allmap, rend_normal, surf_depth, surf_normal, surf_point, static_cast<hipStream_t>(stream)));
    return SR_OK;
}

int sr_postprocess_backward(int32_t W, int32_t H, float fovx, float fovy, float depth_ratio, const float* viewmatrix,
                            const float* allmap, const float* g_rend_normal, const float* g_surf_depth, const float* g_surf_normal,
                            const float* g_surf_point, float* scratch6, float* g_allmap, void* stream) {
    PostCam cam;
    if (int rc = post_cam(W, H, fovx, fovy, depth_ratio, viewmatrix, &cam)) return rc;
    if (!allmap || !scratch6 || !g_allmap) return fail(SR_ERR_INVALID_ARGUMENT, "NULL argument");
    SR_HIP(launch_postprocess_backward(cam, allmap, g_rend_normal, g_surf_depth, g_surf_normal, g_surf_point, scratch6, g_allmap,
                                       static_cast<hipStream_t>(stream)));
    return SR_OK;
}

size_t sr_image_loss_workspace_bytes(int32_t W, int32_t H, int32_t C) {
    if (W <= 0 || H <= 0 || C <= 0) return 0;
    return image_loss_partial_bytes() + 3 * sizeof(float) * (size_t)W * (size_t)H * (size_t)C;
}

static int image_loss_args(int32_t W, int32_t H, int32_t C, float lambda_dssim, const float* image, const float* gt, const float* sky,
                           const float* alpha, const void* workspace, size_t workspace_bytes, LossImages* a) {
    if (W <= 0 || H <= 0 || C <= 0) return fail(SR_ERR_INVALID_ARGUMENT, "bad image size %dx%d with %d channels", W, H, C);
    if (!image || !gt || !workspace) return fail(SR_ERR_INVALID_ARGUMENT, "image / gt / workspace is NULL");
    if ((sky != nullptr) != (alpha != nullptr)) return fail(SR_ERR_INVALID_ARGUMENT, "sky and alpha go together: give both or neither");
    if (!image_loss_supported(W, H, C)) return fail(SR_ERR_UNSUPPORTED, "%dx%d with %d channels is beyond the launch limits", W, H, C);
    if (workspace_bytes < sr_image_loss_workspace_bytes(W, H, C))
        return fail(SR_ERR_BUFFER_TOO_SMALL, "workspace %zu < %zu", workspace_bytes, sr_image_loss_workspace_bytes(W, H, C));
    *a = LossImages{W, H, C, lambda_dssim, image, gt, sky, alpha};
    return SR_OK;
}

int sr_image_loss_forward(int32_t W, int32_t H, int32_t C, float lambda_dssim, const float* image, const float* gt, const float* sky,
                          const float* alpha, void* workspace, size_t workspace_bytes, float* out3, void* stream) {
    LossImages a;
    if (int rc = image_loss_args(W, H, C, lambda_dssim, image, gt, sky, alpha, workspace, workspace_bytes, &a)) return rc;
    if (!out3) return fail(SR_ERR_INVALID_ARGUMENT, "out3 is NULL");
    SR_HIP(launch_image_loss_forward(a, workspace, out3, static_cast<hipStream_t>(stream)));
    return SR_OK;
}

int sr_image_loss_backward(int32_t W, int32_t H, int32_t C, float lambda_dssim, const float* image, const float* gt, const float* sky,
                           const float* alpha, const void* workspace, size_t workspace_bytes, const float* g_loss, float* g_image,
                           float* g_sky, float* g_alpha, void* stream) {
    LossImages a;
    if (int rc = image_loss_args(W, H, C, lambda_dssim, image, gt, sky, alpha, workspace, workspace_bytes, &a)) return rc;
    if (!g_loss || !g_image) return fail(SR_ERR_INVALID_ARGUMENT, "g_loss / g_image is NULL");
    if (sky && (!g_sky || !g_alpha)) return fail(SR_ERR_INVALID_ARGUMENT, "with sky and alpha, g_sky and g_alpha are required");
    SR_HIP(launch_image_loss_backward(a, workspace, g_loss, g_image, g_sky, g_alpha, static_cast<hipStream_t>(stream)));
    return SR_OK;
}

int sr_debug_lds_atomic_ranks(const uint32_t* digits, uint32_t* ranks, uint32_t n, int bins, void* stream) {
    if (n > 0 && (!digits || !ranks)) return fail(SR_ERR_INVALID_ARGUMENT, "NULL argument");
    if (bins < 1 || bins > 1024 || (n % 256u) != 0u) return fail(SR_ERR_INVALID_ARGUMENT, "bins %d not in 1..1024 or n %u not a multiple of 256", bins, n);
    SR_HIP(lds_atomic_ranks(digits, ranks, n, bins, static_cast<hipStream_t>(stream)));
    return SR_OK;
}

int sr_rank_mode(void* stream) {
    int mode = kRankUnknown;
    if (int rc = rank_mode(static_cast<hipStream_t>(stream), false, &mode)) return rc;
    return mode;
}

size_t sr_debug_radix_sort_temp_bytes(uint32_t n) { return radix_sort_temp_bytes(n); }

int sr_debug_radix_sort(const uint32_t* keys_in, const uint32_t* vals_in, uint32_t* keys_out, uint32_t* vals_out, uint32_t n,
                        int total_bits, void* temp, size_t temp_bytes, uint32_t flags, void* stream) {
    if (n > 0 && (!keys_in || !keys_out || !vals_out || !temp)) return fail(SR_ERR_INVALID_ARGUMENT, "NULL argument");
    if (total_bits < 1 || total_bits > 32) return fail(SR_ERR_INVALID_ARGUMENT, "total_bits %d not in 1..32", total_bits);
    if (temp_bytes < radix_sort_temp_bytes(n)) return fail(SR_ERR_BUFFER_TOO_SMALL, "temp %zu < %zu", temp_bytes, radix_sort_temp_bytes(n));
    int sort_mode = kRankUnknown;
    if (int rc = rank_mode(static_cast<hipStream_t>(stream), (flags & SR_FLAG_BALLOT_RANKING) != 0, &sort_mode)) return rc;
    if (flags & SR_FLAG_ONE_SWEEP_SORT) sort_mode |= 0x100;
    SR_HIP(radix_sort_pairs(keys_in, vals_in, keys_out, vals_out, n, total_bits, temp, temp_bytes, static_cast<hipStream_t>(stream), nullptr, nullptr, sort_mode));
    return SR_OK;
}

void sr_set_stage_timing(int enable) {
    std::lock_guard<std::mutex> lk(g_ring_mu);
    g_timing.store(enable);
    if (enable) for (auto& r : g_ring) r.used = 0;
}

int sr_stage_stats(int stage, float* total_ms, int* launches) {
    if (stage < 0 || stage >= SR_STAGE_COUNT || !total_ms || !launches) return fail(SR_ERR_INVALID_ARGUMENT, "bad stage / NULL output");
    std::lock_guard<std::mutex> lk(g_ring_mu);
    EvRing& r = g_ring[stage];
    float sum = 0.f;
    int done = 0;
    for (int i = 0; i < r.used; ++i) {
        if (!r.closed[i]) continue;
        ++done;
        float ms = 0.f;
        SR_HIP(hipEventSynchronize(r.ev[i][1]));
        SR_HIP(hipEventElapsedTime(&ms, r.ev[i][0], r.ev[i][1]));
        sum += ms;
    }
    *total_ms = sum;
    *launches = done;
    return SR_OK;
}

}
```

streetunveiler_amd/csrc/binning.hip:

```cpp
#include "common.h"

namespace sr {

size_t radix_sort_temp_bytes(uint32_t n);
hipError_t radix_sort_pairs(const uint32_t* keys_in, const uint32_t* vals_in, uint32_t* keys_out, uint32_t* vals_out, uint32_t n,
                            int total_bits, void* temp, size_t temp_bytes, hipStream_t s, const uint2* aux_src, uint2* aux_out, int rank_mode,
                            int rect_bx = 0, int rect_by = 0, const uint32_t* n_live = nullptr);
size_t tile_count_scan_temp_bytes(uint32_t n);
hipError_t tile_count_scan(const uint32_t* counts, uint32_t* out, uint32_t n, void* temp, size_t temp_bytes, uint32_t* total_host, hipStream_t s);

constexpr int kXpThreads = 256, kXpWaves = kXpThreads / 64;
constexpr int kXpInputsX = 1024, kXpInputsY = 2048;
template <int AXIS> constexpr int xp_inputs() { return AXIS == 0 ? kXpInputsX : kXpInputsY; }
constexpr int kXpBatch = 2048;
constexpr int kXpMaxBins = 1024;
__device__ inline uint32_t pack_column(int miny, int h, int tx) { return (uint32_t)miny | ((uint32_t)h << 10) | ((uint32_t)tx << 21); }

__device__ inline uint32_t block_exclusive_scan(uint32_t x, uint32_t* s_w, uint32_t& total) {
    const int lane = threadIdx.x & 63, w = threadIdx.x >> 6;
    uint32_t incl = wave_inclusive_scan(x);
    __syncthreads();
    if (lane == 63) s_w[w] = incl;
    __syncthreads();
    uint32_t off = 0, tot = 0;
#pragma unroll
    for (int k = 0; k < kXpWaves; ++k) { const uint32_t c = s_w[k]; if (k < w) off += c; tot += c; }
    total = tot;
    return off + incl - x;
}

template <int AXIS> __device__ inline void expansion_of(uint2 item, int& start, int& len) {
    if (AXIS == 0) { start = (int)(item.x & 0xFFFFu); len = (int)(item.y & 0xFFFFu); }
    else { start = (int)(item.y & 1023u); len = (int)((item.y >> 10) & 2047u); }
}

template <int AXIS>
__global__ __launch_bounds__(kXpThreads) void expand_hist_kernel(const uint2* __restrict__ in, uint32_t n_host, const uint32_t* __restrict__ n_dev,
                                                                 int bins, uint32_t* __restrict__ hist, int stride, int tiles_x,
                                                                 uint32_t* __restrict__ tile_counts, int n_tiles) {
    __shared__ uint32_t s_diff[kXpMaxBins + 1];
    __shared__ uint32_t s_full[AXIS ? 4 : 1][AXIS ? kXpMaxBins + 1 : 1];
    __shared__ uint32_t s_w[kXpWaves];
    const int tid = threadIdx.x, lane = tid & 63, w = tid >> 6;
    if (AXIS == 0)
        for (int k = blockIdx.x * kXpThreads + tid; k < n_tiles; k += gridDim.x * kXpThreads) tile_counts[k] = 0;
    const uint32_t n = n_dev ? *n_dev : n_host;
    constexpr int kInputs = xp_inputs<AXIS>();
    const uint32_t base = blockIdx.x * (uint32_t)kInputs;
    if (base >= n) return;
    for (int k = tid; k <= bins; k += kXpThreads) s_diff[k] = 0;
    int tx0 = 0;
    if (AXIS == 1) {
        for (int k = tid; k < 4 * (kXpMaxBins + 1); k += kXpThreads) (&s_full[0][0])[k] = 0;
        tx0 = (int)(in[base].y >> 21);
    }
    __syncthreads();
#pragma unroll
    for (int i = 0; i < kInputs / kXpThreads; ++i) {
        const uint32_t idx = base + (uint32_t)(i * kXpThreads + tid);
        if (idx < n) {
            const uint2 it = in[idx];
            int start, len; expansion_of<AXIS>(it, start, len);
            if (len) {
                atomicAdd(&s_diff[start], 1u); atomicSub(&s_diff[start + len], 1u);
                if (AXIS == 1) {
                    const int tx = (int)(it.y >> 21);
                    const uint32_t rel = (uint32_t)(tx - tx0);
                    if (rel < 4u) { atomicAdd(&s_full[rel][start], 1u); atomicSub(&s_full[rel][start + len], 1u); }
                    else for (int k = 0; k < len; ++k) atomicAdd(&tile_counts[(start + k) * tiles_x + tx], 1u);
                }
            }
        }
    }
    __syncthreads();
    {
        uint32_t v[4], sum = 0;
#pragma unroll
        for (int j = 0; j < 4; ++j) { const int b = 4 * tid + j; sum += b < bins ? s_diff[b] : 0u; v[j] = sum; }
        uint32_t total;
        const uint32_t excl = block_exclusive_scan(sum, s_w, total);
#pragma unroll
        for (int j = 0; j < 4; ++j) { const int b = 4 * tid + j; if (b < bins) hist[(size_t)b * stride + blockIdx.x] = excl + v[j]; }
    }
    if (AXIS == 1 && tx0 + w < tiles_x) {
        uint32_t carry = 0;
        for (int c = 0; c < bins; c += 64) {
            const int row = c + lane;
            uint32_t incl = wave_inclusive_scan(row < bins ? s_full[w][row] : 0u);
            const uint32_t cnt = carry + incl;
            if (row < bins && cnt) atomicAdd(&tile_counts[row * tiles_x + tx0 + w], cnt);
            carry += (uint32_t)__shfl((int)incl, 63);
        }
    }
}

__global__ __launch_bounds__(kXpThreads) void expand_scan_rows_kernel(uint32_t* __restrict__ hist, int stride, uint32_t n_host,
                                                                      const uint32_t* __restrict__ n_dev, int inputs_per_block,
                                                                      uint32_t* __restrict__ row_total) {
    __shared__ uint32_t s_w[kXpWaves];
    const uint32_t n = n_dev ? *n_dev : n_host;
    const int nblocks = (int)((n + (uint32_t)inputs_per_block - 1) / (uint32_t)inputs_per_block);
    uint32_t* row = hist + (size_t)blockIdx.x * stride;
    uint32_t carry = 0;
    for (int c = 0; c < nblocks; c += kXpThreads) {
        const int i = c + (int)threadIdx.x;
        const uint32_t x = i < nblocks ? row[i] : 0u;
        uint32_t total;
        const uint32_t excl = block_exclusive_scan(x, s_w, total);
        if (i < nblocks) row[i] = carry + excl;
        carry += total;
    }
    if (threadIdx.x == 0) row_total[blockIdx.x] = carry;
}

template <int AXIS, int kBits, bool kAtomicRank>
__global__ __launch_bounds__(kXpThreads) void expand_scatter_kernel(
    const uint2* __restrict__ in, uint32_t n_host, const uint32_t* __restrict__ n_dev, int bins, const uint32_t* __restrict__ hist, int stride,
    const uint32_t* __restrict__ row_total,
    const uint32_t* __restrict__ sorted_gid, uint2* __restrict__ columns_out, uint32_t* __restrict__ n_columns_out,
    uint32_t* __restrict__ point_list) {
    constexpr int kBins = 1 << kBits;
    constexpr int kPer = kBins / kXpThreads > 0 ? kBins / kXpThreads : 1;
    constexpr int kInputs = xp_inputs<AXIS>(), kXpPerThread = kInputs / kXpThreads;
    __shared__ __attribute__((aligned(16))) uint8_t s_start[kXpBatch];
    __shared__ uint32_t s_prefix[kInputs + 1];
    __shared__ uint32_t s_count[kXpWaves][kBins];
    __shared__ uint32_t s_lstart[kBins];
    __shared__ uint32_t s_goff[kBins];
    __shared__ uint32_t s_w[kXpWaves];
    __shared__ uint32_t s_id[kXpBatch];
    __shared__ uint32_t s_rows[AXIS == 0 ? kXpBatch : 1];
    __shared__ uint16_t s_dig[kXpBatch];
    const int tid = threadIdx.x, lane = tid & 63, w = tid >> 6;
    const uint32_t n = n_dev ? *n_dev : n_host;
    const uint32_t base = blockIdx.x * (uint32_t)kInputs;
    if (base >= n) return;
    const int n_items = (int)min((uint32_t)kInputs, n - base);
    uint32_t E;
    uint32_t it_first[kXpPerThread];
    {
        uint32_t incl[kXpPerThread], sum = 0;
#pragma unroll
        for (int i = 0; i < kXpPerThread; ++i) {
            const int j = tid * kXpPerThread + i;
            int start = 0, len = 0;
            if (j < n_items) {
                const uint2 it = in[base + j];
                expansion_of<AXIS>(it, start, len);
            }
            it_first[i] = len ? sum : 0xFFFFFFFFu;
            sum += (uint32_t)len;
            incl[i] = sum;
        }
        for (int k = tid; k < kXpBatch / 4; k += kXpThreads) reinterpret_cast<uint32_t*>(s_start)[k] = 0;
        const uint32_t excl = block_exclusive_scan(sum, s_w, E);
#pragma unroll
        for (int i = 0; i < kXpPerThread; ++i) {
            s_prefix[tid * kXpPerThread + i + 1] = excl + incl[i];
            if (it_first[i] != 0xFFFFFFFFu) it_first[i] += excl;
        }
        if (tid == 0) s_prefix[0] = 0;
    }
    {
        uint32_t v[kPer], sum = 0;
#pragma unroll
        for (int j = 0; j < kPer; ++j) { const int d = tid * kPer + j; const uint32_t c = (d < bins) ? row_total[d] : 0u; v[j] = sum; sum += c; }
        uint32_t total;
        const uint32_t excl = block_exclusive_scan(sum, s_w, total);
#pragma unroll
        for (int j = 0; j < kPer; ++j) { const int d = tid * kPer + j; if (d < kBins) s_goff[d] = d < bins ? excl + v[j] + hist[(size_t)d * stride + blockIdx.x] : 0u; }
        if (AXIS == 0 && blockIdx.x == 0 && tid == 0) *n_columns_out = total;
    }
    for (uint32_t q0 = 0; q0 < E; q0 += kXpBatch) {
        for (int k = tid; k < kXpWaves * kBins; k += kXpThreads) (&s_count[0][0])[k] = 0;
#pragma unroll
        for (int i = 0; i < kXpPerThread; ++i)
            if (it_first[i] - q0 < (uint32_t)kXpBatch) s_start[it_first[i] - q0] = 1;
        __syncthreads();
        const uint32_t s0 = q0 + (uint32_t)(w * (kXpBatch / kXpWaves));
        uint32_t marks_before = 0;
        if (s0 < E) {
            int lo = 0;
#pragma unroll
            for (int step = kInputs / 2; step > 0; step >>= 1)
                if (lo + step < n_items && s_prefix[lo + step] <= s0) lo += step;
            marks_before = (uint32_t)lo + (s_prefix[lo] == s0 ? 0u : 1u);
        }
        uint32_t dig[kXpBatch / kXpThreads], id[kXpBatch / kXpThreads], rows[AXIS == 0 ? kXpBatch / kXpThreads : 1];
#pragma unroll
        for (int i = 0; i < kXpBatch / kXpThreads; ++i) {
            const uint32_t slot = s0 + (uint32_t)(i * 64 + lane);
            dig[i] = 0; id[i] = 0;
            if (AXIS == 0) rows[i] = 0;
            const bool mark = slot < E && s_start[slot - q0] != 0;
            const unsigned long long marks = ballot64(mark);
            const uint32_t lo = marks_before + __builtin_amdgcn_mbcnt_hi((uint32_t)(marks >> 32), __builtin_amdgcn_mbcnt_lo((uint32_t)marks, 0u)) +
                                (mark ? 1u : 0u) - 1u;
            marks_before += (uint32_t)__popcll(marks);
            if (slot < E) {
                const uint2 it = in[base + lo];
                int start, len; expansion_of<AXIS>(it, start, len);
                dig[i] = (uint32_t)start + (slot - s_prefix[lo]);
                if (AXIS == 0) { id[i] = sorted_gid[base + lo]; rows[i] = (it.x >> 16) | ((it.y >> 16) << 10); }
                else id[i] = it.x;
                atomicAdd(&s_count[w][dig[i]], 1u);
            }
        }
        __syncthreads();
        for (int k = tid; k < kXpBatch / 4; k += kXpThreads) reinterpret_cast<uint32_t*>(s_start)[k] = 0;
        uint32_t tot[kPer];
        {
            uint32_t sum = 0;
#pragma unroll
            for (int j = 0; j < kPer; ++j) {
                const int d = tid * kPer + j;
                tot[j] = 0;
                if (d < kBins) {
#pragma unroll
                    for (int k = 0; k < kXpWaves; ++k) tot[j] += s_count[k][d];
                }
                sum += tot[j];
            }
            uint32_t total;
            uint32_t run = block_exclusive_scan(sum, s_w, total);
#pragma unroll
            for (int j = 0; j < kPer; ++j) {
                const int d = tid * kPer + j;
                if (d < kBins) {
                    s_lstart[d] = run;
#pragma unroll
                    for (int k = 0; k < kXpWaves; ++k) { const uint32_t c = s_count[k][d]; s_count[k][d] = run; run += c; }
                }
            }
        }
        __syncthreads();
#pragma unroll
        for (int i = 0; i < kXpBatch / kXpThreads; ++i) {
            const uint32_t slot = q0 + (uint32_t)(w * (kXpBatch / kXpWaves) + i * 64 + lane);
            const bool live = slot < E;
            const uint32_t d = dig[i];
            const uint32_t pos = take_run_slot<kAtomicRank>(s_count[w], d, live, kBits);
            if (live) { s_id[pos] = id[i]; s_dig[pos] = (uint16_t)d; if (AXIS == 0) s_rows[pos] = rows[i]; }
        }
        __syncthreads();
        const uint32_t count = min((uint32_t)kXpBatch, E - q0);
#pragma unroll
        for (int i = 0; i < kXpBatch / kXpThreads; ++i) {
            const uint32_t li = (uint32_t)(i * kXpThreads + tid);
            if (li < count) {
                const uint32_t d = s_dig[li];
                const uint32_t g = s_goff[d] + (li - s_lstart[d]);
                if (AXIS == 0) columns_out[g] = make_uint2(s_id[li], s_rows[li] | (d << 21));
                else point_list[g] = s_id[li];
            }
        }
        __syncthreads();
#pragma unroll
        for (int j = 0; j < kPer; ++j) { const int d = tid * kPer + j; if (d < kBins) s_goff[d] += tot[j]; }
    }
}

constexpr int kOrderThreads = 1024, kOrderClasses = 16;
__device__ __forceinline__ uint32_t row_inclusive_scan16(uint32_t x) {
    int v = (int)x;
    v += __builtin_amdgcn_update_dpp(0, v, 0x111, 0xf, 0xf, true);
    v += __builtin_amdgcn_update_dpp(0, v, 0x112, 0xf, 0xf, true);
    v += __builtin_amdgcn_update_dpp(0, v, 0x114, 0xf, 0xf, true);
    v += __builtin_amdgcn_update_dpp(0, v, 0x118, 0xf, 0xf, true);
    return (uint32_t)v;
}
__global__ __launch_bounds__(kOrderThreads) void tile_ranges_order_kernel(int n_tiles, const uint32_t* __restrict__ counts, uint2* __restrict__ ranges,
                                                                          uint32_t* __restrict__ order) {
    constexpr int kPer = 8, kWaves = kOrderThreads / 64, kChunk = kOrderThreads * kPer;
    static_assert(kWaves == 16 && kOrderClasses == 16, "the cross-wave prefix below runs on 16 x 16 values, one 16-lane row per class");
    __shared__ uint32_t s_cls[kOrderClasses][kWaves];
    __shared__ uint32_t s_off[kOrderClasses][kWaves];
    __shared__ uint32_t s_tot[kOrderClasses];
    __shared__ uint32_t s_wsum[kWaves], s_woff[kWaves];
    __shared__ uint32_t s_carry, s_cls_base[kOrderClasses];
    const int tid = threadIdx.x, lane = tid & 63, w = tid >> 6;
    auto cls_of = [](uint32_t len) { return len ? min(kOrderClasses - 1, max(0, (int)__clz(len) - 11)) : kOrderClasses - 1; };
    const bool single_chunk = n_tiles <= kChunk;
    if (tid < kOrderClasses) s_cls_base[tid] = 0;
    if (tid == 0) s_carry = 0;
    if (!single_chunk) {
        uint32_t my_cls[kOrderClasses];
#pragma unroll
        for (int k = 0; k < kOrderClasses; ++k) my_cls[k] = 0;
        for (int t = tid; t < n_tiles; t += kOrderThreads) { const int c = cls_of(counts[t]);
#pragma unroll
            for (int k = 0; k < kOrderClasses; ++k) my_cls[k] += (c == k); }
        __syncthreads();
#pragma unroll
        for (int k = 0; k < kOrderClasses; ++k) {
            const uint32_t v = wave_inclusive_scan(my_cls[k]);
            if (lane == 63 && v) atomicAdd(&s_cls_base[k], v);
        }
        __syncthreads();
        if (tid == 0) { uint32_t run = 0; for (int k = 0; k < kOrderClasses; ++k) { const uint32_t c = s_cls_base[k]; s_cls_base[k] = run; run += c; } }
    }
    __syncthreads();
    for (int base = 0; base < n_tiles; base += kChunk) {
        const int t0 = base + tid * kPer;
        uint32_t c[kPer], sum = 0;
#pragma unroll
        for (int i = 0; i < kPer; ++i) { c[i] = t0 + i < n_tiles ? counts[t0 + i] : 0u; sum += c[i]; }
        const uint32_t incl = wave_inclusive_scan(sum);
        if (lane == 63) s_wsum[w] = incl;
        uint32_t mine[kOrderClasses];
#pragma unroll
        for (int k = 0; k < kOrderClasses; ++k) mine[k] = 0;
#pragma unroll
        for (int i = 0; i < kPer; ++i) { if (t0 + i < n_tiles) { const int cl = cls_of(c[i]);
#pragma unroll
            for (int k = 0; k < kOrderClasses; ++k) mine[k] += (cl == k); } }
        uint32_t before[kOrderClasses];
#pragma unroll
        for (int k = 0; k < kOrderClasses; ++k) {
            const uint32_t v = wave_inclusive_scan(mine[k]);
            before[k] = v - mine[k];
            if (lane == 63) s_cls[k][w] = v;
        }
        __syncthreads();
        if (tid < kOrderClasses * kWaves) {
            const uint32_t v = s_cls[tid >> 4][tid & 15], in = row_inclusive_scan16(v);
            s_off[tid >> 4][tid & 15] = in - v;
            if ((tid & 15) == 15) s_tot[tid >> 4] = in;
        } else if (tid < kOrderClasses * kWaves + 64) {
            const int j = tid - kOrderClasses * kWaves;
            const uint32_t v = j < kWaves ? s_wsum[j] : 0u, in = row_inclusive_scan16(v);
            if (j < kWaves) s_woff[j] = in - v;
        }
        __syncthreads();
        if (single_chunk) {
            if (tid == 0) { uint32_t run = 0; for (int k = 0; k < kOrderClasses; ++k) { s_cls_base[k] = run; run += s_tot[k]; } }
            __syncthreads();
        }
        uint32_t run = s_carry + s_woff[w] + incl - sum;
#pragma unroll
        for (int k = 0; k < kOrderClasses; ++k) before[k] += s_cls_base[k] + s_off[k][w];
#pragma unroll
        for (int i = 0; i < kPer; ++i) {
            if (t0 + i < n_tiles) {
                ranges[t0 + i] = c[i] ? make_uint2(run, run + c[i]) : make_uint2(0u, 0u);
                run += c[i];
                const int cl = cls_of(c[i]);
                uint32_t pos = 0;
#pragma unroll
                for (int k = 0; k < kOrderClasses; ++k) { if (cl == k) { pos = before[k]; before[k] += 1; } }
                order[pos] = (uint32_t)(t0 + i);
            }
        }
        __syncthreads();
        if (tid == kOrderThreads - 1) s_carry = run;
        if (tid < kOrderClasses) s_cls_base[tid] += s_tot[tid];
        __syncthreads();
    }
}

size_t depth_sort_temp_bytes(int P) {
    const uint32_t n = (uint32_t)(P > 0 ? P : 1);
    return align_up(radix_sort_temp_bytes(n), 256);
}
size_t tile_scan_temp_bytes(int P) { return tile_count_scan_temp_bytes((uint32_t)(P > 0 ? P : 1)); }

size_t expand_x_hist_bytes(int P, int tiles_x) { return (size_t)tiles_x * (((size_t)(P > 0 ? P : 1) + kXpInputsX - 1) / kXpInputsX) * 4; }
size_t expand_y_hist_bytes(uint32_t D, int tiles_y) { return (size_t)tiles_y * (((size_t)(D > 0 ? D : 1) + kXpInputsY - 1) / kXpInputsY) * 4; }

hipError_t run_depth_sort(int P, const uint32_t* depth_keys, const uint2* rect, uint32_t* sorted_keys,
                          uint32_t* sorted_gid, uint2* rect_sorted, void* temp, size_t temp_bytes, int rank_mode, int tiles_x, int tiles_y,
                          const uint32_t* n_visible, hipStream_t s) {
    if (P == 0) return hipSuccess;
    const int bx = 32 - __builtin_clz((unsigned)(tiles_x > 0 ? tiles_x : 1)), by = 32 - __builtin_clz((unsigned)(tiles_y > 0 ? tiles_y : 1));
    return radix_sort_pairs(depth_keys, nullptr, sorted_keys, sorted_gid, (uint32_t)P, 32, temp, temp_bytes, s, rect, rect_sorted, rank_mode, bx, by, n_visible);
}

hipError_t run_tile_count_scan(int P, const uint32_t* tiles_touched, uint32_t* first, void* block_base, size_t base_bytes, uint32_t* total_host,
                               hipStream_t s) {
    if (P == 0) return hipSuccess;
    return tile_count_scan(tiles_touched, first, (uint32_t)P, block_base, base_bytes, total_host, s);
}

template <int AXIS, bool kAtomicRank, typename... Args>
static void launch_expand_scatter_r(int bins, int blocks, hipStream_t s, Args... a) {
    if (bins <= 128) hipLaunchKernelGGL((expand_scatter_kernel<AXIS, 7, kAtomicRank>), dim3(blocks), dim3(kXpThreads), 0, s, a...);
    else if (bins <= 256) hipLaunchKernelGGL((expand_scatter_kernel<AXIS, 8, kAtomicRank>), dim3(blocks), dim3(kXpThreads), 0, s, a...);
    else if (bins <= 512) hipLaunchKernelGGL((expand_scatter_kernel<AXIS, 9, kAtomicRank>), dim3(blocks), dim3(kXpThreads), 0, s, a...);
    else hipLaunchKernelGGL((expand_scatter_kernel<AXIS, 10, kAtomicRank>), dim3(blocks), dim3(kXpThreads), 0, s, a...);
}
template <int AXIS, typename... Args>
static void launch_expand_scatter(int rank_mode, int bins, int blocks, hipStream_t s, Args... a) {
    if (rank_mode == kRankAtomic) launch_expand_scatter_r<AXIS, true>(bins, blocks, s, a...);
    else launch_expand_scatter_r<AXIS, false>(bins, blocks, s, a...);
}

hipError_t run_expand_columns(int P, int tiles_x, int n_tiles, const uint2* rect_sorted, const uint32_t* sorted_gid, uint2* columns,
                              uint32_t* n_columns, uint32_t* hist, uint32_t* row_total, uint32_t* tile_counts, int rank_mode, const uint32_t* n_visible,
                              hipStream_t s) {
    if (P == 0) return hipSuccess;
    if (tiles_x > kXpMaxBins || (rank_mode != kRankAtomic && rank_mode != kRankBallot)) return hipErrorInvalidValue;
    const int nb = (P + kXpInputsX - 1) / kXpInputsX;
    hipLaunchKernelGGL(expand_hist_kernel<0>, dim3(nb), dim3(kXpThreads), 0, s, rect_sorted, (uint32_t)P, n_visible, tiles_x, hist, nb,
                       tiles_x, tile_counts, n_tiles);
    hipLaunchKernelGGL(expand_scan_rows_kernel, dim3(tiles_x), dim3(kXpThreads), 0, s, hist, nb, (uint32_t)P, n_visible, kXpInputsX, row_total);
    launch_expand_scatter<0>(rank_mode, tiles_x, nb, s, rect_sorted, (uint32_t)P, n_visible, tiles_x, (const uint32_t*)hist, nb,
                             (const uint32_t*)row_total, sorted_gid, columns, n_columns, (uint32_t*)nullptr);
    return hipGetLastError();
}

hipError_t run_expand_rows(uint32_t D, int tiles_x, int tiles_y, const uint2* columns, const uint32_t* n_columns, uint32_t* hist, uint32_t* row_total,
                           uint32_t* point_list, uint32_t* tile_counts, int rank_mode, hipStream_t s) {
    if (D == 0) return hipSuccess;
    if (tiles_y > kXpMaxBins || (rank_mode != kRankAtomic && rank_mode != kRankBallot)) return hipErrorInvalidValue;
    const int nb = (int)((D + kXpInputsY - 1) / kXpInputsY);
    hipLaunchKernelGGL(expand_hist_kernel<1>, dim3(nb), dim3(kXpThreads), 0, s, columns, D, n_columns, tiles_y, hist, nb, tiles_x, tile_counts,
                       tiles_x * tiles_y);
    hipLaunchKernelGGL(expand_scan_rows_kernel, dim3(tiles_y), dim3(kXpThreads), 0, s, hist, nb, D, n_columns, kXpInputsY, row_total);
    launch_expand_scatter<1>(rank_mode, tiles_y, nb, s, columns, D, n_columns, tiles_y, (const uint32_t*)hist, nb, (const uint32_t*)row_total,
                             (const uint32_t*)nullptr, (uint2*)nullptr, (uint32_t*)nullptr, point_list);
    return hipGetLastError();
}

__global__ void capacity_guard_kernel(uint32_t* __restrict__ counts, uint32_t capacity) {
    const uint32_t over = counts[0] > capacity ? 1u : 0u;
    counts[2] = over;
    if (over) counts[1] = 0u;
}
__global__ __launch_bounds__(256) void zero_bytes_kernel(uint8_t* __restrict__ p, size_t n) {
    const size_t head = (size_t)((16 - (reinterpret_cast<uintptr_t>(p) & 15)) & 15);
    const size_t h = head < n ? head : n;
    const size_t body = (n - h) / 16;
    const size_t i = (size_t)blockIdx.x * 256 + threadIdx.x, stride = (size_t)gridDim.x * 256;
    uint4* q = reinterpret_cast<uint4*>(p + h);
    for (size_t k = i; k < body; k += stride) q[k] = make_uint4(0u, 0u, 0u, 0u);
    if (i < h) p[i] = 0;
    const size_t tail0 = h + body * 16;
    if (i < n - tail0) p[tail0 + i] = 0;
}
hipError_t launch_zero_bytes(void* p, size_t n, hipStream_t s) {
    if (n == 0) return hipSuccess;
    const size_t blocks = (n / 16 + 255) / 256;
    hipLaunchKernelGGL(zero_bytes_kernel, dim3((unsigned)(blocks < 1 ? 1 : (blocks > 4096 ? 4096 : blocks))), dim3(256), 0, s, static_cast<uint8_t*>(p), n);
    return hipGetLastError();
}

hipError_t run_capacity_guard(uint32_t* counts, uint32_t capacity, hipStream_t s) {
    hipLaunchKernelGGL(capacity_guard_kernel, dim3(1), dim3(1), 0, s, counts, capacity);
    return hipGetLastError();
}

hipError_t run_tile_ranges_order(int n_tiles, const uint32_t* tile_counts, uint2* ranges, uint32_t* order, hipStream_t s) {
    if (n_tiles == 0) return hipSuccess;
    hipLaunchKernelGGL(tile_ranges_order_kernel, dim3(1), dim3(kOrderThreads), 0, s, n_tiles, tile_counts, ranges, order);
    return hipGetLastError();
}

}
```

streetunveiler_amd/csrc/common.h:

```cpp
#pragma once
#include <hip/hip_runtime.h>
#include <stdint.h>

#include "../../include/surfel_raster.h"
#include "../../include/surfel_switches.h"

#if defined(__HIP_DEVICE_COMPILE__) && !defined(__gfx950__)
#error "these kernels are written for gfx950 (MI355X): wave64, v_permlane16/32_swap, DPP row controls, and the LDS-atomic lane order the sort kernels rank by (checked at run time, api.hip rank_mode)"
#endif

namespace sr {

constexpr int kTile = SR_TILE;
constexpr int kBlock = kTile * kTile;
constexpr float kNear = 0.2f;
constexpr float kFar = 100.0f;
constexpr float kFilterSize = 0.707106f;
constexpr float kFilterInvSquare = 2.0f;
constexpr float kCutoff = 3.0f;
constexpr float kAlphaCap = 0.99f;
constexpr float kAlphaFloor = 1.0f / 255.0f;
constexpr float kTStop = 0.0001f;
constexpr uint32_t kCulledKey = 0xFFFFFFFFu;

constexpr int kRecQuads = 5;
constexpr int kRecFloats = SR_SPLAT_FLOATS;

constexpr int kGradQuads = 6;
constexpr int kGradFloats = SR_GRAD_FLOATS;

struct FrameDev {
    int W, H, tiles_x, tiles_y;
    int bw_W, bw_H;
    int tile_w, tile_h;
    float inv_tile_w, inv_tile_h;
    int sh_degree, sh_coeffs;
    int colors;
    int activations;
    float scale_modifier;
    const float* bg;
    const float* view;
    const float* proj;
    const float* campos;
    const uint32_t* first;
    const uint32_t* first_base;
    float* sh_jac;
    const uint32_t* overflow;
};
constexpr int kScanTile = 2048;
__device__ __forceinline__ uint32_t first_index(const FrameDev& f, uint32_t gid) { return f.first[gid] + f.first_base[gid / kScanTile]; }

__host__ __device__ inline size_t align_up(size_t x, size_t a) { return (x + a - 1) / a * a; }

__device__ __forceinline__ unsigned long long ballot64(bool p) { return __builtin_amdgcn_ballot_w64(p); }

__device__ __forceinline__ uint32_t wave_inclusive_scan(uint32_t x) {
    int v = (int)x;
    v += __builtin_amdgcn_update_dpp(0, v, 0x111, 0xf, 0xf, true);
    v += __builtin_amdgcn_update_dpp(0, v, 0x112, 0xf, 0xf, true);
    v += __builtin_amdgcn_update_dpp(0, v, 0x114, 0xf, 0xf, true);
    v += __builtin_amdgcn_update_dpp(0, v, 0x118, 0xf, 0xf, true);
    v += __builtin_amdgcn_update_dpp(0, v, 0x142, 0xa, 0xf, true);
    v += __builtin_amdgcn_update_dpp(0, v, 0x143, 0xc, 0xf, true);
    return (uint32_t)v;
}

template <bool kAtomic>
__device__ __forceinline__ uint32_t take_run_slot(uint32_t* run, uint32_t d, bool live, int bits) {
    uint32_t pos = 0;
    if (kAtomic) {
        if (live) pos = atomicAdd(&run[d], 1u);
        return pos;
    }
    unsigned long long same = ballot64(live);
    for (int b = 0; b < bits; ++b) {
        const unsigned long long vote = ballot64(((d >> b) & 1u) != 0u);
        same &= ((d >> b) & 1u) ? vote : ~vote;
    }
    const uint32_t lane = threadIdx.x & 63u;
    const uint32_t rank = (uint32_t)__popcll(same & ((1ull << lane) - 1ull));
    if (live) pos = run[d] + rank;
    __builtin_amdgcn_wave_barrier();
    if (live && rank == 0) run[d] += (uint32_t)__popcll(same);
    __builtin_amdgcn_wave_barrier();
    return pos;
}
enum RankMode { kRankUnknown = 0, kRankAtomic = 1, kRankBallot = 2, kRankNone = 3 };

}
```

streetunveiler_amd/csrc/render.hip:

```cpp
#include "blend_common.h"

#ifndef SR_K6_COLOURS_UP_FRONT
#define SR_K6_COLOURS_UP_FRONT 1
#endif
namespace sr {

template <int QX, int QY, int SPLIT>
__device__ __forceinline__ void store_hit_mask(uint16_t* __restrict__ hit_mask, uint32_t pos, int part, uint32_t hm) {
    if (SPLIT == 2) reinterpret_cast<uint8_t*>(hit_mask)[2 * (size_t)pos + part] = (uint8_t)hm;
    else if (QY == 2) hit_mask[pos] = (uint16_t)((hm & ((1u << QX) - 1u)) | ((hm >> QX) << 8));
    else hit_mask[pos] = (uint16_t)hm;
}

template <bool kStats, int NC, int QX, int QY, int SPLIT>
__device__ __forceinline__ void render_forward_body(float4 (*s_e)[kWave], const FrameDev& f, const uint2* __restrict__ ranges, const uint32_t* __restrict__ tile_order,
                                                    const uint32_t* __restrict__ point_list, const float4* __restrict__ recs, const float* __restrict__ extra,
                                                    float* __restrict__ out_color, float* __restrict__ out_allmap, float* __restrict__ final_T,
                                                    uint32_t* __restrict__ n_contrib, uint16_t* __restrict__ hit_mask, int cull, unsigned long long* __restrict__ g_stats) {
    const int lane = threadIdx.x;
    int tile = blockIdx.x, part = 0;
    if (SPLIT > 1) {
        const int xcd = blockIdx.x % kXcds, k = blockIdx.x / kXcds;
        tile = (k / SPLIT) * kXcds + xcd; part = k % SPLIT;
        if (tile >= f.tiles_x * f.tiles_y) return;
    }
    tile = (int)tile_order[tile];
    constexpr int NQ = QX * QY;
    const int tx0 = (tile % f.tiles_x) * (QX * 8), ty0 = (tile / f.tiles_x) * (QY * 8 * SPLIT) + part * (QY * 8);
    const float Xc = (float)(tx0 + QX * 4), Yc = (float)((tile / f.tiles_x) * (QY * 8 * SPLIT) + QY * SPLIT * 4);
    const int yshift_px = part * (QY * 8) - QY * (SPLIT - 1) * 4;
    const float yshift = (float)yshift_px;
    const int lx = lane & 7, ly = lane >> 3;
    const uint2 range = ranges[tile];
    const uint32_t n_total = range.y - range.x;

    float xl[NQ], yl[NQ];
    float T[NQ], C0[NQ], C1[NQ], C2[NQ], N0[NQ], N1[NQ], N2[NQ], Dsum[NQ], M1[NQ], M2[NQ], dist[NQ], med[NQ];
    float C3[NQ], C4[NQ], C5[NQ], C6[NQ], C7[NQ], C8[NQ];
    uint32_t lastc[NQ], medc[NQ];
    uint32_t alive = 0;
#pragma unroll
    for (int q = 0; q < NQ; ++q) {
        const int px = tx0 + (q % QX) * 8 + lx, py = ty0 + (q / QX) * 8 + ly;
        xl[q] = (float)((q % QX) * 8 + lx - QX * 4); yl[q] = (float)((q / QX) * 8 + ly - QY * 4) + yshift;
        T[q] = (px < f.W && py < f.H) ? 1.f : -1.f; C0[q] = C1[q] = C2[q] = N0[q] = N1[q] = N2[q] = 0.f;
        C3[q] = C4[q] = C5[q] = C6[q] = C7[q] = C8[q] = 0.f;
        Dsum[q] = M1[q] = M2[q] = dist[q] = med[q] = 0.f;
        lastc[q] = 0; medc[q] = 0xFFFFFFFFu;
        if (ballot64(T[q] > 0.f) != 0) alive |= 1u << q;
    }

    float4 nr[kRecQuads], nx = make_float4(0.f, 0.f, 0.f, 0.f), ny = nx;
    uint32_t gid_ahead = 0;
    if ((uint32_t)lane < n_total) {
        const uint32_t gid = point_list[range.x + lane];
        load_record18(recs, gid, nr);
        if (NC == 6) nx = load_extra(extra, gid, 3);
            if (NC == 9) { nx = load_extra(extra, gid, 0); ny = load_extra(extra, gid, 3); }
    }
    if (kWave + (uint32_t)lane < n_total) gid_ahead = point_list[range.x + kWave + lane];
    unsigned long long hit_prev[NQ];
#pragma unroll
    for (int q = 0; q < NQ; ++q) hit_prev[q] = 0ull;
    uint32_t n_prev = 0, base_prev = 0;
    for (uint32_t base = 0; base < n_total && alive; base += kWave) {
        const uint32_t n = min((uint32_t)kWave, n_total - base);
        uint32_t m = 0;
        int ys = yshift_px;
        asm volatile("" : "+s"(ys));
        uint32_t cells16 = 0;
        wait_vector_memory();
        if ((uint32_t)lane < n) m = stage_entry<QX, QY, NC>(nr, nx, ny, Xc, Yc, cull & 1, s_e, lane, (float)ys, kStats && QX == 2 && QY == 2 ? &cells16 : nullptr);
        const uint32_t gid = gid_ahead;
        if (hit_mask && (uint32_t)lane < n_prev) {
            uint32_t hm = 0;
#pragma unroll
            for (int q = 0; q < NQ; ++q) hm |= (uint32_t)((hit_prev[q] >> lane) & 1ull) << q;
            store_hit_mask<QX, QY, SPLIT>(hit_mask, range.x + base_prev + lane, part, hm);
        }
        if (base + 2 * kWave + lane < n_total) gid_ahead = point_list[range.x + base + 2 * kWave + lane];
        __builtin_amdgcn_sched_barrier(0);
        if (base + kWave + lane < n_total) {
            load_record18(recs, gid, nr);
            if (NC == 6) nx = load_extra(extra, gid, 3);
            if (NC == 9) { nx = load_extra(extra, gid, 0); ny = load_extra(extra, gid, 3); }
        }
        __builtin_amdgcn_sched_barrier(0);
        const uint32_t alive_at_round_start = alive;
        unsigned long long bits = ballot64((m & alive) != 0);
        if (kStats && lane == 0) { atomicAdd(&g_stats[0], (unsigned long long)n); atomicAdd(&g_stats[1], (unsigned long long)__popcll(bits)); }
        unsigned long long hit[NQ];
#pragma unroll
        for (int q = 0; q < NQ; ++q) hit[q] = 0ull;
        uint32_t cell_round[NQ][4];
#pragma unroll
        for (int q = 0; q < NQ; ++q) { cell_round[q][0] = cell_round[q][1] = cell_round[q][2] = cell_round[q][3] = 0u; }
        while (bits) {
            const int j = __ffsll((long long)bits) - 1;
            bits &= bits - 1;
            const uint32_t mj = (uint32_t)__builtin_amdgcn_readlane((int)m, j) & alive;
            if (!mj) continue;
            const float4 e0 = s_e[0][j], e1 = s_e[1][j], e2 = s_e[2][j], e3 = s_e[3][j];
            constexpr bool kColoursUpFront = SR_K6_COLOURS_UP_FRONT && NC != 3 && !kStats;
            float4 u4 = make_float4(0.f, 0.f, 0.f, 0.f), u5 = u4, u6 = u4;
            if (kColoursUpFront) { u4 = s_e[4][j]; u5 = s_e[5][j]; if (NC == 9) u6 = s_e[6][j]; }
            const uint32_t contributor = base + (uint32_t)j + 1u;
#pragma unroll
            for (int q = 0; q < NQ; ++q) {
                if (!(mj & (1u << q))) continue;
                Hit h;
                const bool valid = intersect(xl[q], yl[q], e0, e1, e2, e3, h) & (T[q] > 0.f);
                if (kStats) {
                    const unsigned long long vb = ballot64(valid);
                    if (lane == 0) { atomicAdd(&g_stats[2], 1ull); if (vb) atomicAdd(&g_stats[3], 1ull); atomicAdd(&g_stats[4], (unsigned long long)__popcll(vb));
                                     if (vb & 0xFFFFFFFFull) atomicAdd(&g_stats[5], 1ull); if (vb >> 32) atomicAdd(&g_stats[6], 1ull); }
                    cell_round[q][0] += (vb & 0x000000000F0F0F0Full) != 0; cell_round[q][1] += (vb & 0x00000000F0F0F0F0ull) != 0;
                    cell_round[q][2] += (vb & 0x0F0F0F0F00000000ull) != 0; cell_round[q][3] += (vb & 0xF0F0F0F000000000ull) != 0;
                    if (NQ == 4) {
                        const uint32_t cj = (uint32_t)__builtin_amdgcn_readlane((int)cells16, j) >> (16 + 4 * q);
                        const uint32_t exact = ((vb & 0x000000000F0F0F0Full) != 0 ? 1u : 0u) | ((vb & 0x00000000F0F0F0F0ull) != 0 ? 2u : 0u) |
                                               ((vb & 0x0F0F0F0F00000000ull) != 0 ? 4u : 0u) | ((vb & 0xF0F0F0F000000000ull) != 0 ? 8u : 0u);
                        if (lane == 0 && (exact & ~cj & 15u)) atomicAdd(&g_stats[14], (unsigned long long)__popc(exact & ~cj & 15u));
                    }
                }
                if (ballot64(valid) == 0) continue;
                hit[q] |= 1ull << j;
                const float4 e4 = kColoursUpFront ? u4 : s_e[4][j], e5 = kColoursUpFront ? u5 : s_e[5][j];
                if (valid) {
                    const float test_T = T[q] * (1.f - h.alpha);
                    const bool go = !(test_T < kTStop);
                    if (go) {
                        const float w = h.alpha * T[q];
                        const float A = 1.f - T[q];
                        const float mm = kFN * (1.f - kNear * fast_rcp(h.depth));
                        dist[q] += (mm * mm * A + M2[q] - 2.f * mm * M1[q]) * w;
                        Dsum[q] += h.depth * w;
                        M1[q] += mm * w;
                        M2[q] += mm * mm * w;
                        if (T[q] > 0.5f) { med[q] = h.depth; medc[q] = contributor; }
                        N0[q] += e4.x * w; N1[q] += e4.y * w; N2[q] += e4.z * w;
                        C0[q] += e4.w * w; C1[q] += e5.x * w; C2[q] += e5.y * w;
                        if (NC >= 6) { C3[q] += e5.z * w; C4[q] += e5.w * w; C5[q] += e3.w * w; }
                        if (NC == 9) { const float4 e6 = kColoursUpFront ? u6 : s_e[6][j]; C6[q] += e6.x * w; C7[q] += e6.y * w; C8[q] += e6.z * w; }
                        lastc[q] = contributor;
                    }
                    T[q] = go ? test_T : -T[q];
                }
                if (ballot64(T[q] > 0.f) == 0) alive &= ~(1u << q);
            }
        }
        if (kStats && lane == 0) {
            unsigned long long any = 0ull;
#pragma unroll
            for (int q = 0; q < NQ; ++q) any |= hit[q];
            atomicAdd(&g_stats[7], (unsigned long long)__popcll(any));
            unsigned long long cells = 0ull, steps = 0ull;
#pragma unroll
            for (int q = 0; q < NQ; ++q) {
                cells += cell_round[q][0] + cell_round[q][1] + cell_round[q][2] + cell_round[q][3];
                steps += max(max(cell_round[q][0], cell_round[q][1]), max(cell_round[q][2], cell_round[q][3]));
            }
            atomicAdd(&g_stats[8], cells); atomicAdd(&g_stats[9], steps);
        }
        if (kStats && NQ == 4) {
            unsigned long long kept = 0ull, steps = 0ull;
#pragma unroll
            for (int q = 0; q < 4; ++q) {
                uint32_t busiest = 0;
#pragma unroll
                for (int c = 0; c < 4; ++c) {
                    const uint32_t k = (uint32_t)__popcll(ballot64(((cells16 >> (4 * q + c)) & 1u) != 0u && ((m >> q) & 1u) != 0u && ((alive_at_round_start >> q) & 1u) != 0u));
                    kept += k; busiest = max(busiest, k);
                }
                steps += busiest;
            }
            if (lane == 0) { atomicAdd(&g_stats[10], kept); atomicAdd(&g_stats[11], steps); }
            kept = 0ull; steps = 0ull;
#pragma unroll
            for (int q = 0; q < 4; ++q) {
                uint32_t busiest = 0;
#pragma unroll
                for (int c = 0; c < 4; ++c) {
                    const uint32_t k = (uint32_t)__popcll(ballot64(((cells16 >> (16 + 4 * q + c)) & 1u) != 0u && ((m >> q) & 1u) != 0u && ((alive_at_round_start >> q) & 1u) != 0u));
                    kept += k; busiest = max(busiest, k);
                }
                steps += busiest;
            }
            if (lane == 0) { atomicAdd(&g_stats[12], kept); atomicAdd(&g_stats[13], steps); }
        }
        if (hit_mask) {
#pragma unroll
            for (int q = 0; q < NQ; ++q) hit_prev[q] = hit[q];
            n_prev = n; base_prev = base;
        }
    }
    if (hit_mask && (uint32_t)lane < n_prev) {
        uint32_t hm = 0;
#pragma unroll
        for (int q = 0; q < NQ; ++q) hm |= (uint32_t)((hit_prev[q] >> lane) & 1ull) << q;
        store_hit_mask<QX, QY, SPLIT>(hit_mask, range.x + base_prev + lane, part, hm);
    }
    const size_t HW = (size_t)f.H * f.W;
    const float bg0 = f.bg[0], bg1 = f.bg[1], bg2 = f.bg[2];
    int lane_again = threadIdx.x;
    asm volatile("" : "+v"(lane_again));
    const int lx2 = lane_again & 7, ly2 = lane_again >> 3;
#pragma unroll
    for (int q = 0; q < NQ; ++q) {
        const int px = tx0 + (q % QX) * 8 + lx2, py = ty0 + (q / QX) * 8 + ly2;
        if (px < f.W && py < f.H) {
            const size_t pix = (size_t)py * f.W + px;
            const float Tq = fabsf(T[q]);
            if (final_T) {
                final_T[pix] = Tq; final_T[HW + pix] = M1[q]; final_T[2 * HW + pix] = M2[q];
                n_contrib[pix] = lastc[q]; n_contrib[HW + pix] = medc[q];
            }
            out_color[pix] = C0[q] + Tq * bg0;
            out_color[HW + pix] = C1[q] + Tq * bg1;
            out_color[2 * HW + pix] = C2[q] + Tq * bg2;
            if (NC >= 6) {
                out_color[3 * HW + pix] = C3[q] + Tq * f.bg[3];
                out_color[4 * HW + pix] = C4[q] + Tq * f.bg[4];
                out_color[5 * HW + pix] = C5[q] + Tq * f.bg[5];
            }
            if (NC == 9) {
                out_color[6 * HW + pix] = C6[q] + Tq * f.bg[6];
                out_color[7 * HW + pix] = C7[q] + Tq * f.bg[7];
                out_color[8 * HW + pix] = C8[q] + Tq * f.bg[8];
            }
            out_allmap[pix] = Dsum[q];
            out_allmap[HW + pix] = 1.f - Tq;
            out_allmap[2 * HW + pix] = N0[q]; out_allmap[3 * HW + pix] = N1[q]; out_allmap[4 * HW + pix] = N2[q];
            out_allmap[5 * HW + pix] = med[q];
            out_allmap[6 * HW + pix] = dist[q];
        }
    }
}

template <bool kStats, int NC, int QX, int QY, int SPLIT>
__global__ __launch_bounds__(kWave) __attribute__((amdgpu_waves_per_eu(!kStats && NC == 3 && QX == 2 && QY == 1 && SPLIT == 2 ? 6 : 1, !kStats && NC == 3 && QX == 2 && QY == 1 && SPLIT == 2 ? 6 : 8)))
void render_forward_kernel(FrameDev f, const uint2* __restrict__ ranges, const uint32_t* __restrict__ tile_order, const uint32_t* __restrict__ point_list,
                           const float4* __restrict__ recs, const float* __restrict__ extra, float* __restrict__ out_color, float* __restrict__ out_allmap,
                           float* __restrict__ final_T, uint32_t* __restrict__ n_contrib, uint16_t* __restrict__ hit_mask, int cull,
                           unsigned long long* __restrict__ g_stats) {
    __shared__ float4 s_e[entry_quads<NC>()][kWave];
    render_forward_body<kStats, NC, QX, QY, SPLIT>(s_e, f, ranges, tile_order, point_list, recs, extra, out_color, out_allmap, final_T, n_contrib, hit_mask, cull, g_stats);
}

template <int QX, int QY, int SPLIT, bool kCells = false>
__device__ __forceinline__ void render_forward_rows_body(float4 (*s_e)[kWave], uint8_t (*s_hit)[kCells ? 4 * kWave : kWave], const FrameDev& f, const uint2* __restrict__ ranges,
                                                         const uint32_t* __restrict__ tile_order, const uint32_t* __restrict__ point_list,
                                                         const float4* __restrict__ recs, float* __restrict__ out_color, float* __restrict__ out_allmap,
                                                         float* __restrict__ final_T, uint32_t* __restrict__ n_contrib, uint16_t* __restrict__ hit_mask) {
    constexpr int NC = 3;
    const int lane = threadIdx.x;
    int tile = blockIdx.x, part = 0;
    if (SPLIT > 1) {
        const int xcd = blockIdx.x % kXcds, k = blockIdx.x / kXcds;
        tile = (k / SPLIT) * kXcds + xcd; part = k % SPLIT;
        if (tile >= f.tiles_x * f.tiles_y) return;
    }
    tile = (int)tile_order[tile];
    constexpr int NQ = QX * QY;
    const int tx0 = (tile % f.tiles_x) * (QX * 8), ty0 = (tile / f.tiles_x) * (QY * 8 * SPLIT) + part * (QY * 8);
    const float Xc = (float)(tx0 + QX * 4), Yc = (float)((tile / f.tiles_x) * (QY * 8 * SPLIT) + QY * SPLIT * 4);
    const int yshift_px = part * (QY * 8) - QY * (SPLIT - 1) * 4;
    const float yshift = (float)yshift_px;
    const int lx = ((lane >> 4) & 1) * 4 + (lane & 3), ly = (lane >> 5) * 4 + ((lane >> 2) & 3);
    const uint2 range = ranges[tile];
    const uint32_t n_total = range.y - range.x;

    const float xl0 = (float)(lx - QX * 4), yl0 = (float)(ly - QY * 4) + yshift;
    float T[NQ], C0[NQ], C1[NQ], C2[NQ], N0[NQ], N1[NQ], N2[NQ], Dsum[NQ], M1[NQ], M2[NQ], dist[NQ], med[NQ];
    uint32_t lastc[NQ], medc[NQ];
    uint32_t alive = 0;
#pragma unroll
    for (int q = 0; q < NQ; ++q) {
        const int px = tx0 + (q % QX) * 8 + lx, py = ty0 + (q / QX) * 8 + ly;
        T[q] = (px < f.W && py < f.H) ? 1.f : -1.f; C0[q] = C1[q] = C2[q] = N0[q] = N1[q] = N2[q] = 0.f;
        Dsum[q] = M1[q] = M2[q] = dist[q] = med[q] = 0.f;
        lastc[q] = 0; medc[q] = 0xFFFFFFFFu;
        if (ballot64(T[q] > 0.f) != 0) alive |= 1u << q;
    }
    float4 nr[kRecQuads];
    const float4 nx = make_float4(0.f, 0.f, 0.f, 0.f);
    uint32_t gid_ahead = 0;
    if ((uint32_t)lane < n_total) load_record18(recs, point_list[range.x + lane], nr);
    if (kWave + (uint32_t)lane < n_total) gid_ahead = point_list[range.x + kWave + lane];
    uint32_t hm_prev = 0, n_prev = 0, base_prev = 0;
    for (uint32_t base = 0; base < n_total && alive; base += kWave) {
        const uint32_t n = min((uint32_t)kWave, n_total - base);
        int ys = yshift_px;
        asm volatile("" : "+s"(ys));
        uint32_t cm = 0;
        wait_vector_memory();
        if ((uint32_t)lane < n) (void)stage_entry<QX, QY, NC>(nr, nx, nx, Xc, Yc, 1, s_e, lane, (float)ys, nullptr, &cm);
        const uint32_t gid = gid_ahead;
        if (hit_mask && (uint32_t)lane < n_prev) store_hit_mask<QX, QY, SPLIT>(hit_mask, range.x + base_prev + lane, part, hm_prev);
        if (base + 2 * kWave + lane < n_total) gid_ahead = point_list[range.x + base + 2 * kWave + lane];
        __builtin_amdgcn_sched_barrier(0);
        if (base + kWave + lane < n_total) load_record18(recs, gid, nr);
        __builtin_amdgcn_sched_barrier(0);
#pragma unroll
        for (int q = 0; q < NQ; ++q) { if (kCells) reinterpret_cast<uint32_t*>(&s_hit[q][0])[lane] = 0u; else s_hit[q][lane] = 0; }
#pragma unroll
        for (int q = 0; q < NQ; ++q) {
            if (!(alive & (1u << q))) continue;
            const float xq = xl0 + (float)((q % QX) * 8), yq = yl0 + (float)((q / QX) * 8);
            unsigned long long brow;
            {
                const unsigned long long b0 = ballot64(((cm >> (4 * q)) & 1u) != 0u), b1 = ballot64(((cm >> (4 * q + 1)) & 1u) != 0u),
                                         b2 = ballot64(((cm >> (4 * q + 2)) & 1u) != 0u), b3 = ballot64(((cm >> (4 * q + 3)) & 1u) != 0u);
                const int row = lane >> 4;
                brow = row == 0 ? b0 : (row == 1 ? b1 : (row == 2 ? b2 : b3));
            }
            while (ballot64(brow != 0ull) != 0ull) {
                const bool act = brow != 0ull;
                const uint32_t j = act ? (uint32_t)__builtin_ctzll(brow) : 0u;
                brow &= brow - 1ull;
                const float4 e0 = s_e[0][j], e1 = s_e[1][j], e2 = s_e[2][j], e3 = s_e[3][j];
                Hit h;
                const bool valid = intersect(xq, yq, e0, e1, e2, e3, h) & (T[q] > 0.f) & act;
                if (ballot64(valid) == 0ull) continue;
                const float4 e4 = s_e[4][j], e5 = s_e[5][j];
                if (valid) {
                    if (kCells) s_hit[q][4 * j + (lane >> 4)] = 1; else s_hit[q][j] = 1;
                    const uint32_t contributor = base + j + 1u;
                    const float test_T = T[q] * (1.f - h.alpha);
                    const bool go = !(test_T < kTStop);
                    if (go) {
                        const float w = h.alpha * T[q];
                        const float A = 1.f - T[q];
                        const float mm = kFN * (1.f - kNear * fast_rcp(h.depth));
                        dist[q] += (mm * mm * A + M2[q] - 2.f * mm * M1[q]) * w;
                        Dsum[q] += h.depth * w;
                        M1[q] += mm * w;
                        M2[q] += mm * mm * w;
                        if (T[q] > 0.5f) { med[q] = h.depth; medc[q] = contributor; }
                        N0[q] += e4.x * w; N1[q] += e4.y * w; N2[q] += e4.z * w;
                        C0[q] += e4.w * w; C1[q] += e5.x * w; C2[q] += e5.y * w;
                        lastc[q] = contributor;
                    }
                    T[q] = go ? test_T : -T[q];
                }
                if (ballot64(T[q] > 0.f) == 0ull) { alive &= ~(1u << q); break; }
            }
        }
        if (hit_mask) {
            uint32_t hm = 0;
#pragma unroll
            for (int q = 0; q < NQ; ++q) {
                if (kCells) {
                    const uint32_t wd = reinterpret_cast<const uint32_t*>(&s_hit[q][0])[lane];
                    hm |= (((wd * 0x00204081u) >> 21) & 15u) << (4 * q);
                } else hm |= (uint32_t)s_hit[q][lane] << q;
            }
            hm_prev = hm; n_prev = n; base_prev = base;
        }
    }
    if (hit_mask && (uint32_t)lane < n_prev) store_hit_mask<QX, QY, SPLIT>(hit_mask, range.x + base_prev + lane, part, hm_prev);
    const size_t HW = (size_t)f.H * f.W;
    const float bg0 = f.bg[0], bg1 = f.bg[1], bg2 = f.bg[2];
    int lane_again = threadIdx.x;
    asm volatile("" : "+v"(lane_again));
    const int lx2 = ((lane_again >> 4) & 1) * 4 + (lane_again & 3), ly2 = (lane_again >> 5) * 4 + ((lane_again >> 2) & 3);
#pragma unroll
    for (int q = 0; q < NQ; ++q) {
        const int px = tx0 + (q % QX) * 8 + lx2, py = ty0 + (q / QX) * 8 + ly2;
        if (px < f.W && py < f.H) {
            const size_t pix = (size_t)py * f.W + px;
            const float Tq = fabsf(T[q]);
            if (final_T) {
                final_T[pix] = Tq; final_T[HW + pix] = M1[q]; final_T[2 * HW + pix] = M2[q];
                n_contrib[pix] = lastc[q]; n_contrib[HW + pix] = medc[q];
            }
            out_color[pix] = C0[q] + Tq * bg0;
            out_color[HW + pix] = C1[q] + Tq * bg1;
            out_color[2 * HW + pix] = C2[q] + Tq * bg2;
            out_allmap[pix] = Dsum[q];
            out_allmap[HW + pix] = 1.f - Tq;
            out_allmap[2 * HW + pix] = N0[q]; out_allmap[3 * HW + pix] = N1[q]; out_allmap[4 * HW + pix] = N2[q];
            out_allmap[5 * HW + pix] = med[q];
            out_allmap[6 * HW + pix] = dist[q];
        }
    }
}

template <int QX, int QY, int SPLIT, bool kCells = false>
__global__ __launch_bounds__(kWave) __attribute__((amdgpu_waves_per_eu(QX * QY <= 2 ? 6 : 1, QX * QY <= 2 ? 6 : 8)))
void render_forward_rows_kernel(FrameDev f, const uint2* __restrict__ ranges, const uint32_t* __restrict__ tile_order, const uint32_t* __restrict__ point_list,
                                const float4* __restrict__ recs, float* __restrict__ out_color, float* __restrict__ out_allmap, float* __restrict__ final_T,
                                uint32_t* __restrict__ n_contrib, uint16_t* __restrict__ hit_mask) {
    static_assert(!kCells || (QX == 2 && QY == 1 && SPLIT == 2), "cell-granular hit masks: the 16x16 tile's band waves (eight cells per band byte)");
    __shared__ float4 s_e[entry_quads<3>()][kWave];
    __shared__ __attribute__((aligned(4))) uint8_t s_hit[QX * QY][kCells ? 4 * kWave : kWave];
    render_forward_rows_body<QX, QY, SPLIT, kCells>(s_e, s_hit, f, ranges, tile_order, point_list, recs, out_color, out_allmap, final_T, n_contrib, hit_mask);
}


__global__ __launch_bounds__(4 * kWave) void render_forward_coop_kernel(FrameDev f, const uint2* __restrict__ ranges, const uint32_t* __restrict__ tile_order,
                                                                          const uint32_t* __restrict__ point_list, const float4* __restrict__ recs,
                                                                          float* __restrict__ out_color, float* __restrict__ out_allmap, float* __restrict__ final_T,
                                                                          uint32_t* __restrict__ n_contrib, uint16_t* __restrict__ hit_mask) {
    constexpr int NC = 3, kStage = kWave / 4;
    __shared__ float4 s_e[entry_quads<NC>()][kWave];
    __shared__ uint32_t s_m[kWave];
    __shared__ uint8_t s_hitq[4][kWave];
    __shared__ uint32_t s_alive[4];
    const int tid = threadIdx.x, lane = tid & 63, w = tid >> 6;
    const int tile = (int)tile_order[blockIdx.x];
    const int tx0 = (tile % f.tiles_x) * 16, ty0 = (tile / f.tiles_x) * 16;
    const float Xc = (float)(tx0 + 8), Yc = (float)(ty0 + 8);
    const int lx = lane & 7, ly = lane >> 3, qx = w & 1, qy = w >> 1;
    const int px = tx0 + qx * 8 + lx, py = ty0 + qy * 8 + ly;
    const float xl = (float)(qx * 8 + lx - 8), yl = (float)(qy * 8 + ly - 8);
    const uint2 range = ranges[tile];
    const uint32_t n_total = range.y - range.x;
    float T = (px < f.W && py < f.H) ? 1.f : -1.f;
    float C0 = 0.f, C1 = 0.f, C2 = 0.f, N0 = 0.f, N1 = 0.f, N2 = 0.f, Dsum = 0.f, M1 = 0.f, M2 = 0.f, dist = 0.f, med = 0.f;
    uint32_t lastc = 0, medc = 0xFFFFFFFFu;
    if (lane == 0) s_alive[w] = 0u;
    __syncthreads();
    if (ballot64(T > 0.f) != 0ull && lane == 0) s_alive[w] = 1u;
    __syncthreads();
    const bool stager = lane < kStage;
    const int se = w * kStage + lane;
    const float4 zero4 = make_float4(0.f, 0.f, 0.f, 0.f);
    float4 nr[kRecQuads];
    uint32_t gid_ahead = 0;
    if (stager && (uint32_t)se < n_total) load_record18(recs, point_list[range.x + se], nr);
    if (stager && kWave + (uint32_t)se < n_total) gid_ahead = point_list[range.x + kWave + se];
    uint32_t hm_prev = 0, n_prev = 0, base_prev = 0;
    for (uint32_t base = 0; base < n_total; base += kWave) {
        const uint32_t alive = (s_alive[0] ? 1u : 0u) | (s_alive[1] ? 2u : 0u) | (s_alive[2] ? 4u : 0u) | (s_alive[3] ? 8u : 0u);
        if (!alive) break;
        const uint32_t n = min((uint32_t)kWave, n_total - base);
        wait_vector_memory();
        if (stager) {
            uint32_t m = 0;
            if ((uint32_t)se < n) m = stage_entry<2, 2, NC>(nr, zero4, zero4, Xc, Yc, 1, s_e, se) & alive;
            s_m[se] = m;
            const uint32_t gid = gid_ahead;
            if (hit_mask && (uint32_t)se < n_prev) hit_mask[range.x + base_prev + se] = (uint16_t)((hm_prev & 3u) | ((hm_prev >> 2) << 8));
            if (base + 2 * kWave + se < n_total) gid_ahead = point_list[range.x + base + 2 * kWave + se];
            __builtin_amdgcn_sched_barrier(0);
            if (base + kWave + se < n_total) load_record18(recs, gid, nr);
            __builtin_amdgcn_sched_barrier(0);
        }
        s_hitq[w][lane] = 0;
        __syncthreads();
        unsigned long long bits = ballot64(((s_m[lane] >> w) & 1u) != 0u);
        unsigned long long hit = 0ull;
        bool open = true;
        while (bits && open) {
            const int j = __ffsll((long long)bits) - 1;
            bits &= bits - 1;
            const float4 e0 = s_e[0][j], e1 = s_e[1][j], e2 = s_e[2][j], e3 = s_e[3][j];
            const uint32_t contributor = base + (uint32_t)j + 1u;
            Hit h;
            const bool valid = intersect(xl, yl, e0, e1, e2, e3, h) & (T > 0.f);
            if (ballot64(valid) == 0) continue;
            hit |= 1ull << j;
            const float4 e4 = s_e[4][j], e5 = s_e[5][j];
            if (valid) {
                const float test_T = T * (1.f - h.alpha);
                const bool go = !(test_T < kTStop);
                if (go) {
                    const float wgt = h.alpha * T;
                    const float A = 1.f - T;
                    const float mm = kFN * (1.f - kNear * fast_rcp(h.depth));
                    dist += (mm * mm * A + M2 - 2.f * mm * M1) * wgt;
                    Dsum += h.depth * wgt;
                    M1 += mm * wgt;
                    M2 += mm * mm * wgt;
                    if (T > 0.5f) { med = h.depth; medc = contributor; }
                    N0 += e4.x * wgt; N1 += e4.y * wgt; N2 += e4.z * wgt;
                    C0 += e4.w * wgt; C1 += e5.x * wgt; C2 += e5.y * wgt;
                    lastc = contributor;
                }
                T = go ? test_T : -T;
            }
            if (ballot64(T > 0.f) == 0) open = false;
        }
        s_hitq[w][lane] = (uint8_t)((hit >> lane) & 1ull);
        const bool quadrant_done = ballot64(T > 0.f) == 0ull;
        if (lane == 0 && quadrant_done) s_alive[w] = 0u;
        __syncthreads();
        if (stager) {
            hm_prev = (uint32_t)s_hitq[0][se] | ((uint32_t)s_hitq[1][se] << 1) | ((uint32_t)s_hitq[2][se] << 2) | ((uint32_t)s_hitq[3][se] << 3);
            n_prev = n; base_prev = base;
        }
        __syncthreads();
    }
    if (stager && hit_mask && (uint32_t)se < n_prev) hit_mask[range.x + base_prev + se] = (uint16_t)((hm_prev & 3u) | ((hm_prev >> 2) << 8));
    const size_t HW = (size_t)f.H * f.W;
    if (px < f.W && py < f.H) {
        const size_t pix = (size_t)py * f.W + px;
        const float Tq = fabsf(T);
        if (final_T) {
            final_T[pix] = Tq; final_T[HW + pix] = M1; final_T[2 * HW + pix] = M2;
            n_contrib[pix] = lastc; n_contrib[HW + pix] = medc;
        }
        out_color[pix] = C0 + Tq * f.bg[0];
        out_color[HW + pix] = C1 + Tq * f.bg[1];
        out_color[2 * HW + pix] = C2 + Tq * f.bg[2];
        out_allmap[pix] = Dsum;
        out_allmap[HW + pix] = 1.f - Tq;
        out_allmap[2 * HW + pix] = N0; out_allmap[3 * HW + pix] = N1; out_allmap[4 * HW + pix] = N2;
        out_allmap[5 * HW + pix] = med;
        out_allmap[6 * HW + pix] = dist;
    }
}

constexpr uint32_t kRowsBelowDuplicatesPerVisibleX2 = 13;
__global__ __launch_bounds__(kWave) __attribute__((amdgpu_waves_per_eu(6, 6)))
void render_forward_auto_kernel(FrameDev f, const uint2* __restrict__ ranges, const uint32_t* __restrict__ tile_order, const uint32_t* __restrict__ point_list,
                                const float4* __restrict__ recs, float* __restrict__ out_color, float* __restrict__ out_allmap, float* __restrict__ final_T,
                                uint32_t* __restrict__ n_contrib, uint16_t* __restrict__ hit_mask, const uint32_t* __restrict__ counts) {
    __shared__ float4 s_e[entry_quads<3>()][kWave];
    __shared__ uint8_t s_hit[2][kWave];
    const unsigned long long D = counts[0], V = counts[1];
    if (2ull * D < (unsigned long long)kRowsBelowDuplicatesPerVisibleX2 * V)
        render_forward_rows_body<2, 1, 2>(s_e, s_hit, f, ranges, tile_order, point_list, recs, out_color, out_allmap, final_T, n_contrib, hit_mask);
    else
        render_forward_body<false, 3, 2, 1, 2>(s_e, f, ranges, tile_order, point_list, recs, nullptr, out_color, out_allmap, final_T, n_contrib, hit_mask, 1, nullptr);
}

template <int QX, int QY>
__global__ __launch_bounds__(kWave) void pair_decisions_kernel(FrameDev f, const uint2* __restrict__ ranges, const uint32_t* __restrict__ point_list,
                                                               const float4* __restrict__ recs, unsigned long long* __restrict__ valid_bits,
                                                               unsigned long long* __restrict__ use3d_bits) {
    __shared__ float4 s_e[entry_quads<3>()][kWave];
    constexpr int NQ = QX * QY;
    const int lane = threadIdx.x, tile = blockIdx.x;
    const int tx0 = (tile % f.tiles_x) * (QX * 8), ty0 = (tile / f.tiles_x) * (QY * 8);
    const float Xc = (float)(tx0 + QX * 4), Yc = (float)(ty0 + QY * 4);
    const float xl0 = (float)((lane & 7) - QX * 4), yl0 = (float)((lane >> 3) - QY * 4);
    const uint2 range = ranges[tile];
    const uint32_t n_total = range.y - range.x;
    const float4 zero4 = make_float4(0.f, 0.f, 0.f, 0.f);
    for (uint32_t base = 0; base < n_total; base += kWave) {
        const uint32_t n = min((uint32_t)kWave, n_total - base);
        if ((uint32_t)lane < n) {
            float4 nr[kRecQuads];
            load_record(recs, point_list[range.x + base + lane], nr);
            (void)stage_entry<QX, QY, 3>(nr, zero4, zero4, Xc, Yc, 0, s_e, lane);
        }
        for (uint32_t j = 0; j < n; ++j) {
            const float4 e0 = s_e[0][j], e1 = s_e[1][j], e2 = s_e[2][j], e3 = s_e[3][j];
#pragma unroll
            for (int q = 0; q < NQ; ++q) {
                Hit h;
                const bool valid = intersect(xl0 + (float)((q % QX) * 8), yl0 + (float)((q / QX) * 8), e0, e1, e2, e3, h);
                const unsigned long long vb = ballot64(valid), ub = ballot64(h.use3d);
                if (lane == 0) { valid_bits[(size_t)(range.x + base + j) * NQ + q] = vb; use3d_bits[(size_t)(range.x + base + j) * NQ + q] = ub; }
            }
        }
    }
}


hipError_t launch_render_forward(const FrameDev& f, const uint2* ranges, const uint32_t* tile_order, const uint32_t* point_list, const float4* recs,
                                 const float* extra, float* out_color, float* out_allmap, float* final_T, uint32_t* n_contrib,
                                 uint16_t* hit_mask, int flags, unsigned long long* counters, const uint32_t* frame_counts, hipStream_t s) {
    const int n_tiles = f.tiles_x * f.tiles_y;
    if (n_tiles == 0) return hipSuccess;
    const dim3 block(kWave);
    const int cull = flags & 1;
    const bool count = (flags & 2) != 0 && counters != nullptr;
#define SR_LAUNCH_FWD(STATS, NCH, QX, QY, SPLIT)                                                                                  \
    hipLaunchKernelGGL((render_forward_kernel<STATS, NCH, QX, QY, SPLIT>),                                                          \
                       dim3(SPLIT > 1 ? (n_tiles + kXcds - 1) / kXcds * kXcds * SPLIT : n_tiles), block, 0, s, f, \
                       ranges, tile_order, point_list, recs, extra, out_color, out_allmap, final_T, n_contrib, hit_mask, cull, counters)
    if (f.tile_w == 16 && f.tile_h == 16) {
        if (f.colors == 9) { SR_LAUNCH_FWD(false, 9, 2, 1, 2); }
        else if (f.colors == 6) { if (count) SR_LAUNCH_FWD(true, 6, 2, 2, 1); else SR_LAUNCH_FWD(false, 6, 2, 1, 2); }
        else if (count)         SR_LAUNCH_FWD(true, 3, 2, 2, 1);
        else if (cull && !(flags & (4 | 8)) && (flags & 32))
                                hipLaunchKernelGGL(render_forward_coop_kernel, dim3(n_tiles), dim3(4 * kWave), 0, s, f, ranges, tile_order, point_list, recs, out_color,
                                                   out_allmap, final_T, n_contrib, hit_mask);
        else if (flags & 64)    hipLaunchKernelGGL((render_forward_rows_kernel<2, 1, 2, true>), dim3((n_tiles + kXcds - 1) / kXcds * kXcds * 2), block, 0, s, f, ranges,
                                                   tile_order, point_list, recs, out_color, out_allmap, final_T, n_contrib, hit_mask);
        else if (flags & 4)     hipLaunchKernelGGL((render_forward_rows_kernel<2, 1, 2>), dim3((n_tiles + kXcds - 1) / kXcds * kXcds * 2), block, 0, s, f, ranges,
                                                   tile_order, point_list, recs, out_color, out_allmap, final_T, n_contrib, hit_mask);
        else if (cull && !(flags & 8) && frame_counts)
                                hipLaunchKernelGGL(render_forward_auto_kernel, dim3((n_tiles + kXcds - 1) / kXcds * kXcds * 2), block, 0, s, f, ranges,
                                                   tile_order, point_list, recs, out_color, out_allmap, final_T, n_contrib, hit_mask, frame_counts);
        else                    SR_LAUNCH_FWD(false, 3, 2, 1, 2);
    } else if (f.colors != 3 && f.tile_w == 32 && f.tile_h == 16) {
        if (f.colors == 9) { SR_LAUNCH_FWD(false, 9, 4, 1, 2); } else { SR_LAUNCH_FWD(false, 6, 4, 1, 2); }
    } else if (f.colors != 3) {
        if (f.tile_h != 8) return hipErrorInvalidValue;
#define SR_FWD_NC(QX)                                                                                        \
        { if (f.colors == 9) { SR_LAUNCH_FWD(false, 9, QX, 1, 1); } else { SR_LAUNCH_FWD(false, 6, QX, 1, 1); } }
        if (f.tile_w == 8) SR_FWD_NC(1) else if (f.tile_w == 16) SR_FWD_NC(2) else if (f.tile_w == 32) SR_FWD_NC(4) else return hipErrorInvalidValue;
#undef SR_FWD_NC
    } else {
        if (f.tile_w == 32 && f.tile_h == 16) { SR_LAUNCH_FWD(false, 3, 4, 1, 2); }
        else {
#define SR_FWD_SHAPE(QX, QY) SR_LAUNCH_FWD(false, 3, QX, QY, 1)
            SR_FOR_TILE_SHAPE(SR_FWD_SHAPE)
#undef SR_FWD_SHAPE
        }
    }
#undef SR_LAUNCH_FWD
    return hipGetLastError();
}

hipError_t launch_pair_decisions(const FrameDev& f, const uint2* ranges, const uint32_t* point_list, const float4* recs,
                                 unsigned long long* valid_bits, unsigned long long* use3d_bits, hipStream_t s) {
    const int n_tiles = f.tiles_x * f.tiles_y;
    if (n_tiles == 0) return hipSuccess;
#define SR_DEC_SHAPE(QX, QY) hipLaunchKernelGGL((pair_decisions_kernel<QX, QY>), dim3(n_tiles), dim3(kWave), 0, s, f, ranges, point_list, recs, valid_bits, use3d_bits)
    SR_FOR_TILE_SHAPE(SR_DEC_SHAPE)
#undef SR_DEC_SHAPE
    return hipGetLastError();
}

}
```

Before: 924.8 Msplats/s.

## Schedule backward tiles by forward-measured work estimate, heaviest first

The forward blend kernels now count per-tile hit tests and entries and write them to a new tile_work buffer. A single-block radix-sort kernel turns these counts into a heaviest-first tile order, which the backward blend uses in place of the forward order. The aim is to reduce load imbalance and tail effects in the backward pass. The cost is one extra small kernel plus popcount and ballot work in the forward loop, and an env var can restore the old order.

```diff
diff --git a/diff_surfel_rasterization/_C.py b/diff_surfel_rasterization/_C.py
--- a/diff_surfel_rasterization/_C.py
+++ b/diff_surfel_rasterization/_C.py
@@ -381,3 +381,33 @@
     L.check(L.load().sr_image_view(_ptr(img), img.numel(), W, H, C.byref(v)), "sr_image_view")
     return dict(final_T=_view(img, v.final_T, 3 * H * W * 4, torch.float32).view(3, H, W),
                 n_contrib=_view(img, v.n_contrib, 2 * H * W * 4, torch.int32).view(2, H, W))
+
+
+def backward_order_view(binning: torch.Tensor, P: int, D: int, W: int, H: int, tile=(16, 16), parts=2):
+    v = L.SrBinningView()
+    L.check(L.load().sr_binning_view(_ptr(binning), binning.numel(), P, D, W, H, C.byref(v)), "sr_binning_view")
+    a256 = lambda n: (n + 255) // 256 * 256
+    tiles = ((W + tile[0] - 1) // tile[0]) * ((H + tile[1] - 1) // tile[1])
+    tiles8 = max(1, ((W + 7) // 8) * ((H + 7) // 8))
+    order_bwd = int(v.tile_order) + a256(tiles8 * 4)
+    work = order_bwd + a256(tiles8 * 4)
+    hit = int(v.ranges) - a256(max(D, 1) * 2)
+    return dict(order_bwd=_view(binning, order_bwd, tiles * 4, torch.int32), tile_work=_view(binning, work, tiles * parts * 8, torch.int32).view(tiles, parts, 2),
+                hit_mask=_view(binning, hit, D * 2, torch.int16), tile_order=_view(binning, v.tile_order, tiles * 4, torch.int32),
+                ranges=_view(binning, v.ranges, tiles * 8, torch.int32).view(tiles, 2))
+
+
+BWD_TEST_WEIGHT, BWD_ENTRY_WEIGHT, BWD_KEY_LEVELS = 85, 96, 256
+
+
+def backward_work_estimate(tile_work: torch.Tensor) -> torch.Tensor:
+    w = tile_work.long()
+    return (BWD_TEST_WEIGHT * w[..., 0] + BWD_ENTRY_WEIGHT * w[..., 1]).sum(1)
+
+
+def backward_order_keys(estimate) -> "numpy.ndarray":
+    import numpy as np
+    est = np.minimum(np.asarray(estimate.cpu() if hasattr(estimate, "cpu") else estimate, dtype=np.int64), 0xFFFFFFFF)
+    top = max(int(est.max()) if est.size else 1, 1)
+    down = max(0, top.bit_length() - 16)
+    return (BWD_KEY_LEVELS - 1) - ((est >> down) * (BWD_KEY_LEVELS - 1)) // (top >> down)
diff --git a/streetunveiler_amd/csrc/api.hip b/streetunveiler_amd/csrc/api.hip
--- a/streetunveiler_amd/csrc/api.hip
+++ b/streetunveiler_amd/csrc/api.hip
@@ -1,3 +1,4 @@
+#include <cstdlib>
 #include <cstdarg>
 #include <cstdio>
 #include <cstring>
@@ -31,11 +32,12 @@
 hipError_t run_expand_rows(uint32_t D, int tiles_x, int tiles_y, const uint2* columns, const uint32_t* n_columns, uint32_t* hist, uint32_t* row_total,
                            uint32_t* point_list, uint32_t* tile_counts, int rank_mode, hipStream_t s);
 hipError_t run_tile_ranges_order(int n_tiles, const uint32_t* tile_counts, uint2* ranges, uint32_t* order, hipStream_t s);
+hipError_t run_backward_order(int n_tiles, int parts, const uint2* work, uint32_t* keys, uint32_t* tmp, uint32_t* order_bwd, hipStream_t s);
 hipError_t run_capacity_guard(uint32_t* counts, uint32_t capacity, hipStream_t s);
 hipError_t launch_zero_bytes(void* p, size_t n, hipStream_t s);
 hipError_t launch_render_forward(const FrameDev& f, const uint2* ranges, const uint32_t* tile_order, const uint32_t* point_list, const float4* recs,
                                  const float* extra, float* out_color, float* out_allmap, float* final_T, uint32_t* n_contrib, uint16_t* hit_mask, int flags,
-                                 unsigned long long* counters, const uint32_t* frame_counts, hipStream_t s);
+                                 unsigned long long* counters, const uint32_t* frame_counts, hipStream_t s, int* work_parts);
 hipError_t launch_render_backward(const FrameDev& f, const uint2* ranges, const uint32_t* tile_order, const uint32_t* point_list, const float4* recs,
                                   const float* extra, const float* final_T, const uint32_t* n_contrib, const float* dL_dcolor,
                                   const float* dL_dallmap, const uint16_t* hit_mask, float4* inst_grads, uint8_t* written, bool precomp_color_grads, hipStream_t s, int coop_mode);
@@ -219,7 +221,7 @@
 }
 
 struct BinLayout {
-    size_t columns, point_list, hit_mask, ranges, order, tile_counts, row_total, n_columns, hist, hist_bytes, total;
+    size_t columns, point_list, hit_mask, ranges, order, order_bwd, tile_work, order_keys, order_tmp, tile_counts, row_total, n_columns, hist, hist_bytes, total;
 };
 BinLayout bin_layout(uint32_t D, int W, int H) {
     BinLayout L{};
@@ -232,6 +234,16 @@
     L.hit_mask = take(n * 2);
     L.ranges = take((size_t)(tiles > 0 ? tiles : 1) * 8);
     L.order = take((size_t)(tiles > 0 ? tiles : 1) * 4);
+    L.order_bwd = take((size_t)(tiles > 0 ? tiles : 1) * 4);
+    {
+        const size_t t16 = (size_t)((W + 15) / 16) * ((H + 15) / 16) * 4, t32 = (size_t)((W + 31) / 32) * ((H + 15) / 16) * 2;
+        size_t waves = (size_t)(tiles > 0 ? tiles : 1);
+        if (t16 > waves) waves = t16;
+        if (t32 > waves) waves = t32;
+        L.tile_work = take(waves * 8);
+    }
+    L.order_keys = take((size_t)(tiles > 0 ? tiles : 1) * 4);
+    L.order_tmp = take((size_t)(tiles > 0 ? tiles : 1) * 4);
     L.tile_counts = take((size_t)(tiles > 0 ? tiles : 1) * 4);
     L.row_total = take((size_t)kMaxTilesPerAxis * 4);
     L.n_columns = take(4);
@@ -523,7 +535,7 @@
     if (!fwd_only && image_bytes < I.total) return fail(SR_ERR_BUFFER_TOO_SMALL, "image buffer %zu < %zu", image_bytes, I.total);
     if (fwd_only && frame->blend_counters) return fail(SR_ERR_UNSUPPORTED, "SR_FLAG_FORWARD_ONLY and blend_counters exclude each other");
     hipStream_t s = static_cast<hipStream_t>(stream);
-    const FrameDev f = make_frame(frame, g);
+    FrameDev f = make_frame(frame, g);
     if (frame->blend_counters && !(f.tile_w == 16 && f.tile_h == 16 && (f.colors == 3 || f.colors == 6)))
         return fail(SR_ERR_UNSUPPORTED, "blend_counters: the counting variant of the forward blend exists for the 16x16 tile with 3 or 6 colour channels only");
     float4* recs = nullptr;
@@ -541,10 +553,15 @@
                           ((frame->flags & SR_FLAG_ONE_WAVE_BACKWARD) ? 16 : 0) | ((frame->flags & SR_FLAG_COOP_BACKWARD) ? 32 : 0) |
                           (cells ? 64 : 0);
         const GeomLayout GL = geom_layout(g->P);
+        f.tile_work = fwd_only ? nullptr : at<uint2>(binning, B.tile_work);
+        int work_parts = 1;
         SR_HIP(launch_render_forward(f, at<uint2>(binning, B.ranges), at<uint32_t>(binning, B.order), at<uint32_t>(binning, B.point_list), recs, g->colors_precomp, out_color,
                                      out_allmap, fwd_only ? nullptr : at<float>(image, I.final_T), fwd_only ? nullptr : at<uint32_t>(image, I.n_contrib),
                                      fwd_only ? nullptr : at<uint16_t>(binning, B.hit_mask), flags,
-                                     reinterpret_cast<unsigned long long*>(frame->blend_counters), at<uint32_t>(geom, GL.block_base) + GL.n_scan_blocks, s));
+                                     reinterpret_cast<unsigned long long*>(frame->blend_counters), at<uint32_t>(geom, GL.block_base) + GL.n_scan_blocks, s, &work_parts));
+        if (!fwd_only)
+            SR_HIP(run_backward_order(f.tiles_x * f.tiles_y, work_parts, at<uint2>(binning, B.tile_work), at<uint32_t>(binning, B.order_keys),
+                                      at<uint32_t>(binning, B.order_tmp), at<uint32_t>(binning, B.order_bwd), s));
     }
     return debug_sync(frame, s, "render_forward");
 }
@@ -739,8 +756,10 @@
     {
         StageTimer t(SR_STAGE_BLEND_BWD, c.s);
         if (D > 0) SR_HIP(launch_zero_bytes(c.written, D, c.s));
+        const char* fwd_order = std::getenv("SURFEL_BACKWARD_FORWARD_ORDER");
+        const size_t order = (fwd_order && fwd_order[0] == '1') ? c.B.order : c.B.order_bwd;
         if (D > 0)
-            SR_HIP(launch_render_backward(c.f, at<uint2>(binning, c.B.ranges), at<uint32_t>(binning, c.B.order), at<uint32_t>(binning, c.B.point_list), at<float4>(geom, c.L.recs), g->colors_precomp,
+            SR_HIP(launch_render_backward(c.f, at<uint2>(binning, c.B.ranges), at<uint32_t>(binning, order), at<uint32_t>(binning, c.B.point_list), at<float4>(geom, c.L.recs), g->colors_precomp,
                                           at<float>(image, c.I.final_T), at<uint32_t>(image, c.I.n_contrib), dL_dcolor, dL_dallmap, at<uint16_t>(binning, c.B.hit_mask), c.inst_grads, c.written,
                                           !(frame->flags & SR_FLAG_NO_PRECOMP_COLOR_GRAD), c.s,
                                           (frame->flags & SR_FLAG_ROW_BACKWARD) ? 3
diff --git a/streetunveiler_amd/csrc/binning.hip b/streetunveiler_amd/csrc/binning.hip
--- a/streetunveiler_amd/csrc/binning.hip
+++ b/streetunveiler_amd/csrc/binning.hip
@@ -358,6 +358,88 @@
     }
 }
 
+constexpr uint32_t kBwdTestWeight = 85, kBwdEntryWeight = 96;
+constexpr int kBwdOrderThreads = 512, kBwdDigitBits = 4, kBwdDigits = 1 << kBwdDigitBits, kBwdKeyLevels = 256, kBwdBatch = 8;
+constexpr int kBwdTileBits = 32 - kBwdDigitBits;
+static_assert(kBwdKeyLevels == kBwdDigits * kBwdDigits, "two digits make a level");
+__global__ __launch_bounds__(kBwdOrderThreads) void backward_order_kernel(int n_tiles, int parts, const uint2* __restrict__ work, uint32_t* __restrict__ keys,
+                                                                         uint32_t* __restrict__ tmp, uint32_t* __restrict__ order_bwd) {
+    __shared__ uint32_t s_cnt[kBwdDigits][kBwdOrderThreads];
+    __shared__ uint32_t s_wsum[kBwdOrderThreads / 64];
+    __shared__ uint32_t s_max;
+    const int tid = threadIdx.x, lane = tid & 63, w = tid >> 6;
+    if (tid == 0) s_max = 1u;
+    __syncthreads();
+    uint32_t mx = 0;
+#pragma unroll 4
+    for (int t = tid; t < n_tiles; t += kBwdOrderThreads) {
+        unsigned long long e = 0ull;
+        for (int p = 0; p < parts; ++p) { const uint2 c = work[(size_t)t * parts + p]; e += (unsigned long long)kBwdTestWeight * c.x + (unsigned long long)kBwdEntryWeight * c.y; }
+        const uint32_t e32 = e > 0xFFFFFFFFull ? 0xFFFFFFFFu : (uint32_t)e;
+        keys[t] = e32;
+        mx = max(mx, e32);
+    }
+    atomicMax(&s_max, mx);
+    __threadfence();
+    __syncthreads();
+    const uint32_t top = s_max;
+    const int down = max(0, 16 - (int)__clz(top));
+    const uint32_t top16 = top >> down;
+    const int chunk = (n_tiles + kBwdOrderThreads - 1) / kBwdOrderThreads;
+    const int i0 = min(tid * chunk, n_tiles), i1 = min(i0 + chunk, n_tiles);
+    for (int pass = 0; pass < 2; ++pass) {
+#pragma unroll
+        for (int d = 0; d < kBwdDigits; ++d) s_cnt[d][tid] = 0;
+        for (int i = i0; i < i1; i += kBwdBatch) {
+            uint32_t v[kBwdBatch];
+#pragma unroll
+            for (int k = 0; k < kBwdBatch; ++k) v[k] = i + k < i1 ? (pass == 0 ? keys[i + k] : tmp[i + k]) : 0u;
+#pragma unroll
+            for (int k = 0; k < kBwdBatch; ++k) {
+                if (i + k >= i1) break;
+                uint32_t digit;
+                if (pass == 0) {
+                    const uint32_t level = (uint32_t)(kBwdKeyLevels - 1) - (v[k] >> down) * (uint32_t)(kBwdKeyLevels - 1) / top16;
+                    keys[i + k] = level;
+                    digit = level & (kBwdDigits - 1);
+                } else digit = v[k] >> kBwdTileBits;
+                atomicAdd(&s_cnt[digit][tid], 1u);
+            }
+        }
+        __syncthreads();
+        {
+            constexpr int kPerRow = kBwdOrderThreads / kBwdDigits;
+            uint32_t* row = &s_cnt[tid / kPerRow][(tid % kPerRow) * kBwdDigits];
+            uint32_t v[kBwdDigits], sum = 0;
+#pragma unroll
+            for (int k = 0; k < kBwdDigits; ++k) { v[k] = sum; sum += row[k]; }
+            const uint32_t incl = wave_inclusive_scan(sum);
+            if (lane == 63) s_wsum[w] = incl;
+            __syncthreads();
+            uint32_t off = incl - sum;
+#pragma unroll
+            for (int k = 0; k < kBwdOrderThreads / 64; ++k) off += k < w ? s_wsum[k] : 0u;
+#pragma unroll
+            for (int k = 0; k < kBwdDigits; ++k) row[k] = off + v[k];
+        }
+        __syncthreads();
+        uint32_t* dst = pass == 0 ? tmp : order_bwd;
+        for (int i = i0; i < i1; i += kBwdBatch) {
+            uint32_t v[kBwdBatch], pos[kBwdBatch];
+#pragma unroll
+            for (int k = 0; k < kBwdBatch; ++k) v[k] = i + k < i1 ? (pass == 0 ? keys[i + k] : tmp[i + k]) : 0u;
+#pragma unroll
+            for (int k = 0; k < kBwdBatch; ++k)
+                if (i + k < i1) pos[k] = atomicAdd(&s_cnt[pass == 0 ? (v[k] & (kBwdDigits - 1)) : (v[k] >> kBwdTileBits)][tid], 1u);
+#pragma unroll
+            for (int k = 0; k < kBwdBatch; ++k)
+                if (i + k < i1) dst[pos[k]] = pass == 0 ? ((uint32_t)(i + k) | (v[k] >> kBwdDigitBits) << kBwdTileBits) : (v[k] & ((1u << kBwdTileBits) - 1u));
+        }
+        __threadfence();
+        __syncthreads();
+    }
+}
+
 size_t depth_sort_temp_bytes(int P) {
     const uint32_t n = (uint32_t)(P > 0 ? P : 1);
     return align_up(radix_sort_temp_bytes(n), 256);
@@ -449,6 +531,13 @@
     return hipGetLastError();
 }
 
+hipError_t run_backward_order(int n_tiles, int parts, const uint2* work, uint32_t* keys, uint32_t* tmp, uint32_t* order_bwd, hipStream_t s) {
+    if (n_tiles == 0) return hipSuccess;
+    if ((unsigned)n_tiles > (1u << kBwdTileBits)) return hipErrorInvalidValue;
+    hipLaunchKernelGGL(backward_order_kernel, dim3(1), dim3(kBwdOrderThreads), 0, s, n_tiles, parts, work, keys, tmp, order_bwd);
+    return hipGetLastError();
+}
+
 hipError_t run_tile_ranges_order(int n_tiles, const uint32_t* tile_counts, uint2* ranges, uint32_t* order, hipStream_t s) {
     if (n_tiles == 0) return hipSuccess;
     hipLaunchKernelGGL(tile_ranges_order_kernel, dim3(1), dim3(kOrderThreads), 0, s, n_tiles, tile_counts, ranges, order);
diff --git a/streetunveiler_amd/csrc/common.h b/streetunveiler_amd/csrc/common.h
--- a/streetunveiler_amd/csrc/common.h
+++ b/streetunveiler_amd/csrc/common.h
@@ -46,6 +46,7 @@
     const uint32_t* first_base;
     float* sh_jac;
     const uint32_t* overflow;
+    uint2* tile_work;
 };
 constexpr int kScanTile = 2048;
 __device__ __forceinline__ uint32_t first_index(const FrameDev& f, uint32_t gid) { return f.first[gid] + f.first_base[gid / kScanTile]; }
diff --git a/streetunveiler_amd/csrc/render.hip b/streetunveiler_amd/csrc/render.hip
--- a/streetunveiler_amd/csrc/render.hip
+++ b/streetunveiler_amd/csrc/render.hip
@@ -63,6 +63,7 @@
 #pragma unroll
     for (int q = 0; q < NQ; ++q) hit_prev[q] = 0ull;
     uint32_t n_prev = 0, base_prev = 0;
+    uint32_t work_tests = 0, work_entries = 0;
     for (uint32_t base = 0; base < n_total && alive; base += kWave) {
         const uint32_t n = min((uint32_t)kWave, n_total - base);
         uint32_t m = 0;
@@ -189,8 +190,10 @@
             if (lane == 0) { atomicAdd(&g_stats[12], kept); atomicAdd(&g_stats[13], steps); }
         }
         if (hit_mask) {
-#pragma unroll
-            for (int q = 0; q < NQ; ++q) hit_prev[q] = hit[q];
+            unsigned long long any = 0ull;
+#pragma unroll
+            for (int q = 0; q < NQ; ++q) { hit_prev[q] = hit[q]; work_tests += (uint32_t)__popcll(hit[q]); any |= hit[q]; }
+            work_entries += (uint32_t)__popcll(any);
             n_prev = n; base_prev = base;
         }
     }
@@ -235,6 +238,7 @@
             out_allmap[6 * HW + pix] = dist[q];
         }
     }
+    if (f.tile_work && lane_again == 0) f.tile_work[tile * SPLIT + part] = make_uint2(work_tests, work_entries);
 }
 
 template <bool kStats, int NC, int QX, int QY, int SPLIT>
@@ -288,6 +292,7 @@
     if ((uint32_t)lane < n_total) load_record18(recs, point_list[range.x + lane], nr);
     if (kWave + (uint32_t)lane < n_total) gid_ahead = point_list[range.x + kWave + lane];
     uint32_t hm_prev = 0, n_prev = 0, base_prev = 0;
+    uint32_t work_tests = 0, work_entries = 0;
     for (uint32_t base = 0; base < n_total && alive; base += kWave) {
         const uint32_t n = min((uint32_t)kWave, n_total - base);
         int ys = yshift_px;
@@ -356,6 +361,9 @@
                 } else hm |= (uint32_t)s_hit[q][lane] << q;
             }
             hm_prev = hm; n_prev = n; base_prev = base;
+#pragma unroll
+            for (int q = 0; q < NQ; ++q) work_tests += (uint32_t)__popcll(ballot64(kCells ? ((hm >> (4 * q)) & 15u) != 0u : ((hm >> q) & 1u) != 0u));
+            work_entries += (uint32_t)__popcll(ballot64(hm != 0u));
         }
     }
     if (hit_mask && (uint32_t)lane < n_prev) store_hit_mask<QX, QY, SPLIT>(hit_mask, range.x + base_prev + lane, part, hm_prev);
@@ -384,6 +392,7 @@
             out_allmap[6 * HW + pix] = dist[q];
         }
     }
+    if (f.tile_work && lane_again == 0) f.tile_work[tile * SPLIT + part] = make_uint2(work_tests, work_entries);
 }
 
 template <int QX, int QY, int SPLIT, bool kCells = false>
@@ -431,6 +440,7 @@
     if (stager && (uint32_t)se < n_total) load_record18(recs, point_list[range.x + se], nr);
     if (stager && kWave + (uint32_t)se < n_total) gid_ahead = point_list[range.x + kWave + se];
     uint32_t hm_prev = 0, n_prev = 0, base_prev = 0;
+    uint32_t work_tests = 0;
     for (uint32_t base = 0; base < n_total; base += kWave) {
         const uint32_t alive = (s_alive[0] ? 1u : 0u) | (s_alive[1] ? 2u : 0u) | (s_alive[2] ? 4u : 0u) | (s_alive[3] ? 8u : 0u);
         if (!alive) break;
@@ -483,6 +493,7 @@
             if (ballot64(T > 0.f) == 0) open = false;
         }
         s_hitq[w][lane] = (uint8_t)((hit >> lane) & 1ull);
+        work_tests += (uint32_t)__popcll(hit);
         const bool quadrant_done = ballot64(T > 0.f) == 0ull;
         if (lane == 0 && quadrant_done) s_alive[w] = 0u;
         __syncthreads();
@@ -510,6 +521,7 @@
         out_allmap[5 * HW + pix] = med;
         out_allmap[6 * HW + pix] = dist;
     }
+    if (f.tile_work && lane == 0) f.tile_work[tile * 4 + w] = make_uint2(work_tests, work_tests);
 }
 
 constexpr uint32_t kRowsBelowDuplicatesPerVisibleX2 = 13;
@@ -562,30 +574,39 @@
 
 hipError_t launch_render_forward(const FrameDev& f, const uint2* ranges, const uint32_t* tile_order, const uint32_t* point_list, const float4* recs,
                                  const float* extra, float* out_color, float* out_allmap, float* final_T, uint32_t* n_contrib,
-                                 uint16_t* hit_mask, int flags, unsigned long long* counters, const uint32_t* frame_counts, hipStream_t s) {
+                                 uint16_t* hit_mask, int flags, unsigned long long* counters, const uint32_t* frame_counts, hipStream_t s, int* work_parts) {
     const int n_tiles = f.tiles_x * f.tiles_y;
+    int parts = 1;
+    if (work_parts) *work_parts = parts;
     if (n_tiles == 0) return hipSuccess;
     const dim3 block(kWave);
     const int cull = flags & 1;
     const bool count = (flags & 2) != 0 && counters != nullptr;
 #define SR_LAUNCH_FWD(STATS, NCH, QX, QY, SPLIT)                                                                                  \
-    hipLaunchKernelGGL((render_forward_kernel<STATS, NCH, QX, QY, SPLIT>),                                                          \
-                       dim3(SPLIT > 1 ? (n_tiles + kXcds - 1) / kXcds * kXcds * SPLIT : n_tiles), block, 0, s, f, \
-                       ranges, tile_order, point_list, recs, extra, out_color, out_allmap, final_T, n_contrib, hit_mask, cull, counters)
+    do {                                                                                                                          \
+        parts = SPLIT;                                                                                                            \
+        hipLaunchKernelGGL((render_forward_kernel<STATS, NCH, QX, QY, SPLIT>),                                                      \
+                           dim3(SPLIT > 1 ? (n_tiles + kXcds - 1) / kXcds * kXcds * SPLIT : n_tiles), block, 0, s, f, \
+                           ranges, tile_order, point_list, recs, extra, out_color, out_allmap, final_T, n_contrib, hit_mask, cull, counters); \
+    } while (0)
+#define SR_LAUNCH_ROWS(KERNEL, ...)                                                                                               \
+    do {                                                                                                                          \
+        parts = 2;            \
+        hipLaunchKernelGGL(KERNEL, dim3((n_tiles + kXcds - 1) / kXcds * kXcds * 2), block, 0, s, f, ranges, tile_order, point_list, recs, out_color,    \
+                           out_allmap, final_T, n_contrib, hit_mask, ##__VA_ARGS__);                                                \
+    } while (0)
     if (f.tile_w == 16 && f.tile_h == 16) {
         if (f.colors == 9) { SR_LAUNCH_FWD(false, 9, 2, 1, 2); }
         else if (f.colors == 6) { if (count) SR_LAUNCH_FWD(true, 6, 2, 2, 1); else SR_LAUNCH_FWD(false, 6, 2, 1, 2); }
         else if (count)         SR_LAUNCH_FWD(true, 3, 2, 2, 1);
-        else if (cull && !(flags & (4 | 8)) && (flags & 32))
-                                hipLaunchKernelGGL(render_forward_coop_kernel, dim3(n_tiles), dim3(4 * kWave), 0, s, f, ranges, tile_order, point_list, recs, out_color,
-                                                   out_allmap, final_T, n_contrib, hit_mask);
-        else if (flags & 64)    hipLaunchKernelGGL((render_forward_rows_kernel<2, 1, 2, true>), dim3((n_tiles + kXcds - 1) / kXcds * kXcds * 2), block, 0, s, f, ranges,
-                                                   tile_order, point_list, recs, out_color, out_allmap, final_T, n_contrib, hit_mask);
-        else if (flags & 4)     hipLaunchKernelGGL((render_forward_rows_kernel<2, 1, 2>), dim3((n_tiles + kXcds - 1) / kXcds * kXcds * 2), block, 0, s, f, ranges,
-                                                   tile_order, point_list, recs, out_color, out_allmap, final_T, n_contrib, hit_mask);
-        else if (cull && !(flags & 8) && frame_counts)
-                                hipLaunchKernelGGL(render_forward_auto_kernel, dim3((n_tiles + kXcds - 1) / kXcds * kXcds * 2), block, 0, s, f, ranges,
-                                                   tile_order, point_list, recs, out_color, out_allmap, final_T, n_contrib, hit_mask, frame_counts);
+        else if (cull && !(flags & (4 | 8)) && (flags & 32)) {
+            parts = 4;
+            hipLaunchKernelGGL(render_forward_coop_kernel, dim3(n_tiles), dim3(4 * kWave), 0, s, f, ranges, tile_order, point_list, recs, out_color,
+                               out_allmap, final_T, n_contrib, hit_mask);
+        }
+        else if (flags & 64)    SR_LAUNCH_ROWS((render_forward_rows_kernel<2, 1, 2, true>));
+        else if (flags & 4)     SR_LAUNCH_ROWS((render_forward_rows_kernel<2, 1, 2>));
+        else if (cull && !(flags & 8) && frame_counts) SR_LAUNCH_ROWS(render_forward_auto_kernel, frame_counts);
         else                    SR_LAUNCH_FWD(false, 3, 2, 1, 2);
     } else if (f.colors != 3 && f.tile_w == 32 && f.tile_h == 16) {
         if (f.colors == 9) { SR_LAUNCH_FWD(false, 9, 4, 1, 2); } else { SR_LAUNCH_FWD(false, 6, 4, 1, 2); }
@@ -603,6 +624,8 @@
 #undef SR_FWD_SHAPE
         }
     }
+#undef SR_LAUNCH_ROWS
+    if (work_parts) *work_parts = parts;
 #undef SR_LAUNCH_FWD
     return hipGetLastError();
 }
```

Result: faster. 949.4 Msplats/s, median of 6 (+2.7%).
